# ilirlikalla/Smith-Waterman-FPGA-module

Hardware: AMD Instinct MI355X
Metric: GCUPS (higher is better)
Workload: dtype f16

## Files before the change

smith-waterman-fpga-module_amd/csrc/swbank_bank.h:

```cpp
#ifndef SWBANK_BANK_H
#define SWBANK_BANK_H

#include <dlfcn.h>
#include <hip/hip_runtime.h>
#include <rccl/rccl.h>

#include <algorithm>
#include <cmath>
#include <cstdarg>
#include <cstdio>
#include <cstdlib>
#include <cstring>
#include <atomic>
#include <condition_variable>
#include <functional>
#include <memory>
#include <mutex>
#include <numeric>
#include <thread>
#include <chrono>
#include <vector>
#if defined(__SSE2__)
#include <emmintrin.h>
#endif
#if defined(__x86_64__)
#include <immintrin.h>
#endif

#include "swbank.h"
#include "swbank_align.h"
#include "swbank_internal.h"
#include "swbank_pack.h"

extern "C" int swk_has_variant(int R, int RB, int col0, int prof, int gotoh, int f16);
extern "C" hipError_t swk_launch_wave(int K, int col0, int prof, int gotoh, int f16,
                                      const void* edge_in, void* edge_out, uint32_t ecols,
                                      int accum, const uint8_t* res,
                                      const uint64_t* offs, const uint32_t* lens, size_t n,
                                      const uint32_t* qtab, uint32_t nv, uint32_t S, uint32_t O,
                                      uint32_t E, uint32_t PS, uint32_t pad, int32_t* scores,
                                      int packed, const uint32_t* fb_qtab, uint32_t fb_nv,
                                      uint32_t fb_PS, int32_t fb_thresh,
                                      const SwkWaveSplit* split, uint32_t ulen,
                                      uint32_t ustride, int half, hipStream_t st);
extern "C" hipError_t swk_launch_score(int R, int RB, int col0, int prof, int gotoh, int f16,
                                       const uint8_t* res, const uint64_t* offs,
                                       const uint32_t* lens, size_t n, const uint32_t* qtab,
                                       uint32_t nv, uint32_t S, uint32_t O, uint32_t E,
                                       uint32_t PS, uint32_t pad, int W, int32_t* scores,
                                       const void* edge_in, void* edge_out, uint32_t ecols,
                                       int accum, int packed, const uint32_t* idx,
                                       const uint32_t* nidx, uint32_t idx_base,
                                       const uint32_t* ident, int pair, uint32_t pS1,
                                       uint32_t pS2, uint32_t ulen, uint32_t ustride, uint32_t nq,
                                       uint32_t qwords, size_t sstride, hipStream_t st);
extern "C" unsigned swk_bal_slots(int W, uint32_t PS, int trim);
extern "C" unsigned swk_wave_half_grid(int gotoh, uint32_t prof_bytes, int W);
extern "C" hipError_t swk_bal_plan_uniform(void* plan, uint32_t ntiles, uint32_t K, uint32_t G,
                                           hipStream_t st);
extern "C" hipError_t swk_launch_pair_bal(const uint8_t* res, const uint64_t* offs,
                                          const uint32_t* lens, size_t n, const uint32_t* qtab,
                                          uint32_t nv, uint32_t S, uint32_t O, uint32_t E,
                                          uint32_t PS, uint32_t pad, int W, int32_t* scores,
                                          uint32_t pS1, uint32_t pS2, uint32_t ulen,
                                          uint32_t ustride, uint32_t* flag, uint32_t* state,
                                          uint32_t gen, unsigned grid, const uint32_t* idx,
                                          const uint32_t* nidx, const uint32_t* ident,
                                          const void* plan, uint32_t* fault, uint32_t poll_limit,
                                          uint32_t stall, int trim, uint32_t packed,
                                          const uint32_t* sidx, hipStream_t st);
extern "C" hipError_t swk_best_hit(const int32_t* scores, const uint64_t* ids, size_t n,
                                   unsigned long long* key, uint64_t* out, uint64_t* out_index,
                                   hipStream_t st);
extern "C" hipError_t swk_best_part(const int32_t* scores, size_t n, size_t base,
                                    unsigned long long* key, hipStream_t st);
extern "C" hipError_t swk_best_finalize(const unsigned long long* key, const uint64_t* ids,
                                        uint64_t* out, uint64_t* out_index, hipStream_t st);
extern "C" hipError_t swk_sort_lens(const uint32_t* lens, size_t n, uint32_t max_len,
                                    uint32_t* perm, uint32_t* perm_n, uint32_t* ident,
                                    uint32_t* scratch, hipStream_t st, void* plan = nullptr,
                                    unsigned G = 0);
extern "C" size_t swk_sort_scratch_bytes(void);
extern "C" hipError_t swk_flag_high(const int32_t* scores, size_t n, int32_t thresh,
                                    uint32_t* idx, uint32_t* count, hipStream_t st);
extern "C" size_t swk_i32_waves(size_t n, uint32_t scols, size_t budget_bytes);
extern "C" hipError_t swk_launch_i32(int gotoh, const uint8_t* res, const uint64_t* offs,
                                     const uint32_t* lens, size_t n, int packed,
                                     const uint32_t* idx, const uint32_t* nidx, uint32_t idx_base,
                                     const void* prof, uint32_t nstrips, uint32_t qlen,
                                     uint32_t pad, uint32_t O, uint32_t E, int32_t* scores,
                                     void* scratch, uint32_t scols, size_t waves, hipStream_t st);

extern "C" size_t swk_top_state_words(void);
extern "C" hipError_t swk_top_hits(const int32_t* scores, const uint64_t* ids, size_t n, size_t nq,
                                   size_t k, int32_t min_score, unsigned long long* state,
                                   unsigned long long* keys, uint64_t* hits, int32_t* hit_scores,
                                   uint64_t* hit_ids, uint32_t* counts, hipStream_t st);

inline int env_int(const char* name, int dflt) {
  const char* v = std::getenv(name);
  return (v && *v) ? std::atoi(v) : dflt;
}

struct PhaseTrace {
  const char* path = std::getenv("SWBANK_TRACE_FILE");
  std::chrono::steady_clock::time_point t0 = std::chrono::steady_clock::now();
  std::vector<std::pair<const char*, double>> marks;
  std::mutex mu;
  void mark(const char* what) { mark_at(what, std::chrono::steady_clock::now()); }
  void mark_at(const char* what, std::chrono::steady_clock::time_point t) {
    if (!path) return;
    std::lock_guard<std::mutex> g(mu);
    marks.push_back({what, std::chrono::duration<double, std::micro>(t - t0).count()});
  }
  ~PhaseTrace() {
    if (!path || marks.empty()) return;
    if (FILE* f = std::fopen(path, "a")) {
      for (auto& m : marks) std::fprintf(f, "%s %.1f\n", m.first, m.second);
      std::fprintf(f, "--\n");
      std::fclose(f);
    }
  }
};
inline thread_local PhaseTrace* g_trace = nullptr;
inline void trace_mark(const char* what) {
  if (g_trace) g_trace->mark(what);
}

inline bool poison_buffers() {
  const char* v = std::getenv("SWBANK_POISON");
  return v && v[0] == '1';
}

template <typename T>
struct DevBuf {
  T* p = nullptr;
  size_t cap = 0;
  hipError_t reserve(size_t n) {
    if (n <= cap) return hipSuccess;
    if (p) (void)hipFree(p);
    p = nullptr;
    cap = 0;
    size_t want = std::max<size_t>(n, 64);
    hipError_t e = hipMalloc(reinterpret_cast<void**>(&p), want * sizeof(T));
    if (e == hipSuccess) cap = want;
    if (e == hipSuccess && poison_buffers()) {
      e = hipMemset(p, 0x3C, want * sizeof(T));
      if (e == hipSuccess) e = hipStreamSynchronize(nullptr);
    }
    return e;
  }
  void release() {
    if (p) (void)hipFree(p);
    p = nullptr;
    cap = 0;
  }
};

struct UcBuf {
  uint8_t* p = nullptr;
  size_t cap = 0;
  hipError_t reserve(size_t n) {
    if (n <= cap) return hipSuccess;
    if (p) (void)hipFree(p);
    p = nullptr;
    cap = 0;
    hipError_t e = hipExtMallocWithFlags(reinterpret_cast<void**>(&p), n, hipDeviceMallocUncached);
    if (e == hipSuccess) cap = n;
    return e;
  }
  void release() {
    if (p) (void)hipFree(p);
    p = nullptr;
    cap = 0;
  }
};

struct PinBuf {
  unsigned flags = hipHostMallocDefault;
  uint8_t* p = nullptr;
  size_t cap = 0;
  hipError_t reserve(size_t n) {
    if (n <= cap) return hipSuccess;
    if (p) (void)hipHostFree(p);
    p = nullptr;
    cap = 0;
    const size_t want = std::max<size_t>(n, 4096);
    hipError_t e = hipHostMalloc(reinterpret_cast<void**>(&p), want, flags);
    if (e == hipSuccess) cap = want;
    return e;
  }
  void release() {
    if (p) (void)hipHostFree(p);
    p = nullptr;
    cap = 0;
  }
};


class HostPool {
 public:
  explicit HostPool(unsigned n) : n_(std::max(1u, n)) {
    for (unsigned i = 1; i < n_; ++i) th_.emplace_back([this, i] { loop(i); });
  }
  ~HostPool() {
    {
      std::lock_guard<std::mutex> g(m_);
      stop_.store(true);
      gen_.fetch_add(1);
    }
    cv_.notify_all();
    for (auto& t : th_) t.join();
  }
  unsigned size() const { return n_; }
  void run(const std::function<void(unsigned)>& f) {
    if (n_ == 1) {
      f(0);
      return;
    }
    job_ = &f;
    pending_.store(n_ - 1, std::memory_order_relaxed);
    {
      std::lock_guard<std::mutex> g(m_);
      gen_.fetch_add(1, std::memory_order_release);
    }
    cv_.notify_all();
    f(0);
    for (unsigned it = 1; pending_.load(std::memory_order_acquire) != 0; ++it) relax(it);
    job_ = nullptr;
  }

 private:
  static void relax(unsigned) {
#if defined(__SSE2__)
    _mm_pause();
#endif
  }
  void loop(unsigned i) {
    uint64_t seen = 0;
    for (;;) {
      const auto t0 = std::chrono::steady_clock::now();
      for (unsigned it = 1; gen_.load(std::memory_order_acquire) == seen; ++it) {
        relax(it);
        if ((it & 255) == 0 &&
            std::chrono::steady_clock::now() - t0 > std::chrono::microseconds(200)) {
          std::unique_lock<std::mutex> l(m_);
          cv_.wait(l, [&] { return gen_.load() != seen; });
        }
      }
      seen = gen_.load(std::memory_order_acquire);
      if (stop_.load()) return;
      (*job_)(i);
      pending_.fetch_sub(1, std::memory_order_acq_rel);
    }
  }
  unsigned n_;
  std::vector<std::thread> th_;
  std::mutex m_;
  std::condition_variable cv_;
  const std::function<void(unsigned)>* job_ = nullptr;
  std::atomic<unsigned> pending_{0};
  std::atomic<uint64_t> gen_{0};
  std::atomic<bool> stop_{false};
};

class Launcher {
 public:
  explicit Launcher(int device) : th_([this, device] { loop(device); }) {}
  ~Launcher() {
    {
      std::lock_guard<std::mutex> g(m_);
      stop_ = true;
    }
    cv_.notify_one();
    th_.join();
  }
  void post(std::function<sw_status()> f) {
    {
      std::lock_guard<std::mutex> g(m_);
      q_.push_back(std::move(f));
      ++posted_;
    }
    cv_.notify_one();
  }
  sw_status wait(size_t k) {
    while (done_.load(std::memory_order_acquire) < k) {
#if defined(__SSE2__)
      _mm_pause();
#endif
    }
    return st_.load(std::memory_order_acquire);
  }
  sw_status wait_all() { return wait(posted_); }
  void reset() {
    wait_all();
    posted_ = 0;
    done_.store(0);
    st_.store(SW_OK);
  }

 private:
  void loop(int device) {
    (void)hipSetDevice(device);
    for (;;) {
      std::function<sw_status()> f;
      {
        std::unique_lock<std::mutex> l(m_);
        cv_.wait(l, [&] { return stop_ || !q_.empty(); });
        if (q_.empty()) return;
        f = std::move(q_.front());
        q_.erase(q_.begin());
      }
      if (st_.load(std::memory_order_relaxed) == SW_OK) {
        const sw_status s = f();
        if (s != SW_OK) st_.store(s, std::memory_order_release);
      }
      done_.fetch_add(1, std::memory_order_acq_rel);
    }
  }
  std::mutex m_;
  std::condition_variable cv_;
  std::vector<std::function<sw_status()>> q_;
  bool stop_ = false;
  size_t posted_ = 0;
  std::atomic<size_t> done_{0};
  std::atomic<sw_status> st_{SW_OK};
  std::thread th_;
};

struct sw_bank {
  sw_config cfg{};
  int device = 0;
  int cus = 0;
  hipStream_t stream = nullptr;
  char err[512] = {0};

  bool have_pen = false;
  int alpha = SW_DNA_ALPHA;
  std::vector<int8_t> matrix;
  int32_t gap_open = 0, gap_extend = 0;

  bool have_query = false;
  uint64_t qid = 0;
  std::vector<uint8_t> query;
  std::vector<std::vector<uint8_t>> qset;
  bool mq_ready = false;
  DevBuf<uint32_t> mqtab, mqtab16;
  size_t mq_words = 0;
  DevBuf<uint32_t> mqpair;
  size_t mq_pair_words = 0;
  int mq_pair_segs = 0, mq_pair_rows = 0;
  uint32_t mq_pS1 = 0, mq_pS2 = 0;

  bool dirty = true;
  int R = 32, RB = 4, W = 1, col0 = 0, prof = 0;
  uint32_t S = 0, O = 0, E = 0, nv = 0, PS = 0, pad = 4;
  int32_t smax = 0;
  DevBuf<uint32_t> qtab;
  bool f16 = false;
  uint32_t nv16 = 0, PS16 = 0;
  int32_t f16_neg = 0;
  DevBuf<uint32_t> qtab16;
  DevBuf<uint32_t> qpair;
  uint32_t pair_bytes = 0, pS1 = 0, pS2 = 0;
  DevBuf<uint32_t> fb_idx, fb_cnt;
  bool i32_ready = false;
  uint32_t i32_strips = 0;
  DevBuf<uint2> i32prof, i32scr;
  DevBuf<unsigned long long> best_key;
  bool al_ready = false;
  DevBuf<uint8_t> al_tab, al_res;
  DevBuf<uint2> al_scr;
  DevBuf<uint32_t> al_dirs, al_lens, al_cig, al_list;
  DevBuf<uint64_t> al_offs;
  DevBuf<sw_alignment> al_out;
  DevBuf<SwkAlignPlan> al_plan;
  DevBuf<unsigned long long> top_state, top_keys;
  DevBuf<int32_t> top_scores, top_hsc;
  DevBuf<uint64_t> top_hits;
  DevBuf<uint32_t> top_cnt;
  hipEvent_t ev_top = nullptr;
  struct Seg { int W; size_t off, off16; };
  std::vector<Seg> segs;
  DevBuf<uint2> edge[2];
  int wK = 0;
  int wsegs = 1;
  size_t wseg_words = 0, wseg_words16 = 0;
  uint32_t wPS = 0;
  DevBuf<uint32_t> wtab;
  DevBuf<uint32_t> wtab16;
  uint32_t wPS16 = 0;
  int sK[3] = {0, 0, 0};
  size_t sseg_words[3] = {0, 0, 0}, sseg_words16[3] = {0, 0, 0};
  uint32_t sPS[3] = {0, 0, 0}, sPS16[3] = {0, 0, 0};
  DevBuf<uint32_t> stab[3], stab16[3];
  DevBuf<uint2> sring;
  DevBuf<uint32_t> tprog;

  static constexpr int NSLOT = 3, NDSLOT = 6;
  hipStream_t copy_stream = nullptr;
  hipEvent_t h2d_done[NSLOT] = {}, kern_done[NDSLOT] = {};
  PinBuf hslot[NSLOT], hscores;
  std::vector<std::vector<uint32_t>> mlist;
  std::vector<std::vector<uint8_t>> mstage;
  std::vector<std::vector<uint32_t>> mbad;
  std::vector<hipEvent_t> out_ev;
  hipStream_t out_stream = nullptr;
  hipStream_t stream2 = nullptr;
  hipEvent_t ev_s2 = nullptr;
  double host_pack_ms = 0;
  int feed_dslots = NSLOT;
  DevBuf<uint8_t> dslot[NDSLOT];
  DevBuf<uint32_t> sortscr[NDSLOT];
  DevBuf<uint8_t> sbuf;
  UcBuf sflag;
  DevBuf<SwkStreamChunk> sdrec;
  DevBuf<uint32_t> sctr;
  hipStream_t kstream = nullptr;
  PinBuf srec, shflag{hipHostMallocCoherent};
  PinBuf shscores{hipHostMallocCoherent};
  std::vector<hipEvent_t> sev;
  std::unique_ptr<HostPool> pool;
  std::unique_ptr<Launcher> launcher;

  DevBuf<uint8_t> res;
  DevBuf<uint64_t> offs;
  DevBuf<uint32_t> lens;
  DevBuf<int32_t> scores;
  DevBuf<uint8_t> gres;
  DevBuf<uint64_t> goffs;
  DevBuf<uint32_t> glens;

  char last_kernel[160] = {0};

  int best_kind = 0;
  uint64_t best_id = 0, best_index = 0;
  int32_t best_score = 0;
  DevBuf<uint64_t> best_dev;
  hipEvent_t best_ev = nullptr;

  std::vector<sw_bank*> kids;
  std::unique_ptr<HostPool> dpool;
  std::vector<void*> comms;
  bool rccl_gather = false;
  unsigned pool_threads = 0;
  DevBuf<int32_t> grecv;
  PinBuf hrecv;
  DevBuf<uint32_t> bal_state, bal_flag;
  DevBuf<uint32_t> wbal_state, wbal_flag;
  uint32_t wbal_gen = 0;
  DevBuf<uint32_t> bal_plan;
  size_t bal_key[3] = {0, 0, 0};
  uint32_t bal_gen = 0;
  bool peer_ready = false;
  hipEvent_t ev_join = nullptr;
  std::vector<hipEvent_t> deal_ev;
  bool best_root = false;
  DevBuf<uint32_t> dperm, dsort;
  bool is_multi() const { return !kids.empty(); }
  bool gotoh() const { return cfg.gap_model == SW_GAP_GOTOH; }

  hipEvent_t ev_ready = nullptr, ev_used = nullptr;
  PinBuf stage;

  sw_counters ctr{};

  PinBuf faultw{hipHostMallocCoherent};
  bool host_call = false;
  bool no_handoff = false;

  bool timing = false;
  struct Ev { hipEvent_t a, b, c; };
  std::vector<Ev> events;
};

struct DevGuard {
  int prev = -1;
  DevGuard() {
    if (hipGetDevice(&prev) != hipSuccess) prev = -1;
  }
  explicit DevGuard(const sw_bank* b) : DevGuard() {
    if (b && b->device >= 0) (void)hipSetDevice(b->device);
  }
  ~DevGuard() {
    if (prev >= 0) (void)hipSetDevice(prev);
  }
  DevGuard(const DevGuard&) = delete;
  DevGuard& operator=(const DevGuard&) = delete;
};

inline uint16_t f16_score_bits(int v) {
  return __builtin_bit_cast(uint16_t, (_Float16)((float)v * (1.0f / 2048.0f)));
}


sw_status fail(sw_bank* b, sw_status st, const char* fmt, ...);

#define HIPOK(bank, expr)                                                                 \
  do {                                                                                    \
    hipError_t e_ = (expr);                                                               \
    if (e_ != hipSuccess)                                                                 \
      return fail((bank), SW_ERR_HIP, "%s: %s (%s:%d)", #expr, hipGetErrorString(e_),    \
                  __FILE__, __LINE__);                                                    \
  } while (0)

struct Timed {
  sw_bank* b;
  hipStream_t st;
  sw_bank::Ev ev{};
  sw_status begin() {
    if (!b->timing) return SW_OK;
    HIPOK(b, hipEventCreate(&ev.a));
    HIPOK(b, hipEventCreate(&ev.c));
    HIPOK(b, hipEventRecord(ev.a, st));
    ev.b = ev.a;
    return SW_OK;
  }
  sw_status end() {
    if (!b->timing) return SW_OK;
    HIPOK(b, hipEventRecord(ev.c, st));
    b->events.push_back(ev);
    return SW_OK;
  }
  void drop() {
    if (!b->timing) return;
    if (ev.a) (void)hipEventDestroy(ev.a);
    if (ev.c) (void)hipEventDestroy(ev.c);
    ev = {};
  }
};

struct Rccl {
  bool ok = false;
  char err[160] = {0};
  decltype(&ncclCommInitAll) commInitAll = nullptr;
  decltype(&ncclCommDestroy) commDestroy = nullptr;
  decltype(&ncclGather) gather = nullptr;
  decltype(&ncclGetErrorString) errorString = nullptr;
  decltype(&ncclCommAbort) commAbort = nullptr;
  decltype(&ncclCommGetAsyncError) asyncError = nullptr;
  decltype(&ncclGroupStart) groupStart = nullptr;
  decltype(&ncclGroupEnd) groupEnd = nullptr;
};
const Rccl& rccl();

template <class F>
sw_status each_kid(sw_bank* b, F&& f) {
  for (sw_bank* k : b->kids) {
    const sw_status st = f(k);
    if (st != SW_OK) return fail(b, st, "device %d: %s", k->device, k->err);
  }
  return SW_OK;
}

unsigned host_threads();

template <class F>
void parallel_for(HostPool& pool, size_t n, F&& f) {
  const unsigned T = pool.size();
  if (T <= 1 || n < 2048) {
    f((size_t)0, n);
    return;
  }
  const size_t step = (n + T - 1) / T;
  pool.run([&](unsigned p) {
    const size_t lo = std::min(n, p * step), hi = std::min(n, lo + step);
    if (lo < hi) f(lo, hi);
  });
}

inline size_t align16(size_t x) { return (x + 15) & ~(size_t)15; }
inline uint32_t record_len(const uint8_t* rec) {
  uint16_t l;
  std::memcpy(&l, rec + 4, 2);
  return l;
}

void copy_kernel_name(sw_bank* b, const char* gather);
uint32_t* fault_word(sw_bank* b);
sw_status take_fault(sw_bank* b, int which);
sw_status prepare(sw_bank* b);
sw_status prepare_multi(sw_bank* b);
sw_status prepare_i32(sw_bank* b);
void u16_gotoh_rows(const sw_bank* b, bool f16, int& R, int& W);
bool wave_preferred(const sw_bank* b, size_t n, uint32_t max_len, bool use_f16);
sw_status launch(sw_bank* b, const uint8_t* d_res, const uint64_t* d_offs,
                 const uint32_t* d_lens, size_t n, uint32_t max_len, int32_t* d_scores,
                 hipStream_t st, uint32_t packed = SWK_PACK_BYTES,
                 const uint32_t* perm = nullptr, const uint32_t* perm_n = nullptr,
                 bool dsort = false, bool wait_prev = true, uint32_t* sort_out = nullptr,
                 uint32_t* sort_scr = nullptr, uint32_t ulen = 0, uint32_t ustride = 0,
                 uint32_t min_len = 0);
bool chunk_perm(HostPool& pool, const uint32_t* len, size_t n, uint32_t* perm);
bool scratch_free(const sw_bank* b, uint32_t max_len);
struct MixedOrder {
  std::vector<uint32_t> pos;
  uint32_t hi = 0, shift = 0, nbin = 0;
};
bool mixed_pack(sw_bank* b, const uint8_t* residues, size_t nres, const uint64_t* offsets,
                const uint32_t* lens, size_t c0, size_t cnt, size_t step,
                const std::vector<uint64_t>& rbase, const std::vector<uint64_t>& rspan,
                const std::vector<size_t>& psz, const std::vector<size_t>& part4, uint32_t* so32,
                uint32_t* sl32, uint8_t* mcodes, uint32_t* order, MixedOrder* mo, size_t& end);
sw_status batch_feed(sw_bank* b, const uint8_t* residues, size_t nres, const uint64_t* offsets,
                     const uint32_t* lens, size_t n, int32_t* out);
sw_status records_feed(sw_bank* b, const uint8_t* recs, size_t n, int32_t* out);
sw_status stream_feed(sw_bank* b, const uint8_t* residues, size_t nres, const uint64_t* offsets,
                      size_t n, uint32_t L, int32_t* out, bool& used,
                      const uint8_t* recs = nullptr, const uint32_t* rlens = nullptr);
sw_status multi_batch(sw_bank* b, const uint8_t* residues, size_t nres, const uint64_t* offsets,
                      const uint32_t* lens, size_t n, int32_t* scores_out);
sw_status multi_records(sw_bank* b, const uint8_t* recs, size_t n, int32_t* scores_out);
sw_status multi_device(sw_bank* b, const uint8_t* d_res, const uint64_t* d_offs,
                       const uint32_t* d_lens, const uint64_t* d_ids, size_t n, uint32_t min_len,
                       uint32_t max_len, int32_t* d_scores, hipStream_t hs, bool records);
sw_status multi_resident(sw_bank* b, const sw_device_batch* per, int32_t* d_gathered,
                         hipStream_t hs);
sw_status launch_set(sw_bank* b, const uint8_t* d_res, const uint64_t* d_offs,
                     const uint32_t* d_lens, size_t n, uint32_t min_len, uint32_t max_len,
                     int32_t* d_scores, hipStream_t st, size_t sstride);
sw_status track_best_device(sw_bank* b, const int32_t* d_scores, const uint64_t* d_ids, size_t n,
                            hipStream_t st);

#endif
```

smith-waterman-fpga-module_amd/csrc/swbank_bank.hip:

```cpp
#include "swbank_bank.h"

sw_status fail(sw_bank* b, sw_status st, const char* fmt, ...) {
  if (b) {
    va_list ap;
    va_start(ap, fmt);
    vsnprintf(b->err, sizeof(b->err), fmt, ap);
    va_end(ap);
  }
  return st;
}

extern "C" int32_t sw_device_count(void) {
  int n = 0;
  if (hipGetDeviceCount(&n) != hipSuccess) return 0;
  return n;
}

static sw_status check_device(int dev) {
  int ndev = 0;
  if (hipGetDeviceCount(&ndev) != hipSuccess || ndev <= 0) return SW_ERR_NO_DEVICE;
  if (dev < 0 || dev >= ndev) return SW_ERR_NO_DEVICE;
  hipDeviceProp_t prop;
  if (hipGetDeviceProperties(&prop, dev) != hipSuccess) return SW_ERR_NO_DEVICE;
  if (std::strncmp(prop.gcnArchName, "gfx950", 6) != 0) return SW_ERR_NO_DEVICE;
  return SW_OK;
}


extern "C" sw_status sw_bank_create(sw_bank** out, const sw_config* cfg_in) {
  DevGuard dev_guard;
  if (!out) return SW_ERR_ARG;
  *out = nullptr;
  sw_config cfg;
  if (cfg_in)
    cfg = *cfg_in;
  else
    sw_config_default(&cfg);
  if (cfg.alphabet != SW_ALPHABET_DNA && cfg.alphabet != SW_ALPHABET_PROTEIN) return SW_ERR_ARG;
  if (cfg.gap_model != SW_GAP_MERGED && cfg.gap_model != SW_GAP_GOTOH) return SW_ERR_ARG;
  if (cfg.max_query_len > SWB_MAX_QUERY) return SW_ERR_UNSUPPORTED;
  if (cfg.n_devices < 0 || cfg.n_devices > SW_MAX_DEVICES) return SW_ERR_ARG;

  if (cfg.n_devices >= 1) {
    for (int d = 0; d < cfg.n_devices; ++d) {
      const sw_status st = check_device(cfg.devices[d]);
      if (st != SW_OK) return st;
    }
    sw_bank* b = new (std::nothrow) sw_bank();
    if (!b) return SW_ERR_NOMEM;
    b->cfg = cfg;
    b->device = cfg.devices[0];
    b->alpha = cfg.alphabet == SW_ALPHABET_DNA ? SW_DNA_ALPHA : SW_PROTEIN_ALPHA;
    for (int d = 0; d < cfg.n_devices; ++d) {
      sw_config kc = cfg;
      kc.n_devices = 0;
      kc.device = cfg.devices[d];
      sw_bank* k = nullptr;
      const sw_status st = sw_bank_create(&k, &kc);
      if (st != SW_OK) {
        sw_bank_destroy(b);
        return st;
      }
      k->pool_threads = std::max(2u, host_threads() / (unsigned)cfg.n_devices);
      b->kids.push_back(k);
    }
    b->dpool.reset(new (std::nothrow) HostPool((unsigned)cfg.n_devices));
    b->pool.reset(new (std::nothrow) HostPool(host_threads()));
    if (!b->dpool || !b->pool) {
      sw_bank_destroy(b);
      return SW_ERR_NOMEM;
    }
    const char* gm = std::getenv("SWBANK_GATHER");
    const bool force_copy = gm && std::strcmp(gm, "copy") == 0;
    const bool force_rccl = gm && std::strcmp(gm, "rccl") == 0;
    bool distinct = true;
    for (int i = 0; i < cfg.n_devices; ++i)
      for (int j = 0; j < i; ++j) distinct = distinct && cfg.devices[i] != cfg.devices[j];
    if (!force_copy && (distinct || force_rccl)) {
      const Rccl& r = rccl();
      ncclResult_t nr = ncclSuccess;
      if (r.ok) {
        std::vector<ncclComm_t> comms((size_t)cfg.n_devices);
        nr = r.commInitAll(comms.data(), cfg.n_devices, cfg.devices);
        if (nr == ncclSuccess) b->comms.assign(comms.begin(), comms.end());
      }
      b->rccl_gather = !b->comms.empty();
      if (b->comms.empty() && force_rccl) {
        sw_bank_destroy(b);
        return SW_ERR_UNSUPPORTED;
      }
      if (b->comms.empty())
        snprintf(b->err, sizeof(b->err), "RCCL unavailable (%s), gathering with device copies",
                 r.ok ? r.errorString(nr) : r.err);
    }
    (void)hipSetDevice(b->device);
    *out = b;
    return SW_OK;
  }

  int dev = cfg.device;
  if (dev < 0 && hipGetDevice(&dev) != hipSuccess) return SW_ERR_NO_DEVICE;
  const sw_status dst = check_device(dev);
  if (dst != SW_OK) return dst;

  sw_bank* b = new (std::nothrow) sw_bank();
  if (!b) return SW_ERR_NOMEM;
  b->cfg = cfg;
  b->device = dev;
  if (hipSetDevice(dev) != hipSuccess ||
      hipStreamCreateWithFlags(&b->stream, hipStreamNonBlocking) != hipSuccess ||
      hipStreamCreateWithFlags(&b->copy_stream, hipStreamNonBlocking) != hipSuccess ||
      hipStreamCreateWithFlags(&b->out_stream, hipStreamNonBlocking) != hipSuccess ||
      hipStreamCreateWithFlags(&b->stream2, hipStreamNonBlocking) != hipSuccess) {
    for (hipStream_t* x : {&b->stream, &b->copy_stream, &b->out_stream, &b->stream2})
      if (*x) (void)hipStreamDestroy(*x);
    delete b;
    return SW_ERR_HIP;
  }
  b->alpha = cfg.alphabet == SW_ALPHABET_DNA ? SW_DNA_ALPHA : SW_PROTEIN_ALPHA;
  if (hipDeviceGetAttribute(&b->cus, hipDeviceAttributeMultiprocessorCount, dev) != hipSuccess)
    b->cus = 0;
  if (cfg.alphabet == SW_ALPHABET_PROTEIN) {
    int8_t m[SW_PROTEIN_ALPHA * SW_PROTEIN_ALPHA];
    sw_fill_matrix(SW_ALPHABET_PROTEIN, 0, 0, m);
    b->matrix.assign(m, m + sizeof(m));
    b->gap_open = -11;
    b->gap_extend = -1;
    b->have_pen = true;
  }
  *out = b;
  return SW_OK;
}

extern "C" void sw_bank_destroy(sw_bank* b) {
  DevGuard dev_guard(b);
  if (!b) return;
  if (b->is_multi() || !b->comms.empty()) {
    const Rccl& r = rccl();
    for (void* c : b->comms) (void)r.commDestroy(static_cast<ncclComm_t>(c));
    (void)hipSetDevice(b->device);
    if (b->ev_used) (void)hipEventSynchronize(b->ev_used);
    if (b->ev_join) (void)hipEventDestroy(b->ev_join);
    if (b->ev_used) (void)hipEventDestroy(b->ev_used);
    for (sw_bank* k : b->kids) sw_bank_destroy(k);
    b->dpool.reset();
    b->pool.reset();
    (void)hipSetDevice(b->device);
    b->grecv.release();
    b->hrecv.release();
    b->res.release();
    b->offs.release();
    b->lens.release();
    b->dperm.release();
    b->dsort.release();
    delete b;
    return;
  }
  (void)hipSetDevice(b->device);
  if (b->stream) (void)hipStreamSynchronize(b->stream);
  if (b->ev_top) (void)hipEventSynchronize(b->ev_top);
  uint64_t nl;
  double pm, sm;
  (void)sw_bank_timing(b, &nl, &pm, &sm);
  b->faultw.release();
  b->qtab.release();
  b->qtab16.release();
  b->mqtab.release();
  b->mqtab16.release();
  b->mqpair.release();
  b->qpair.release();
  b->stage.release();
  if (b->ev_ready) (void)hipEventDestroy(b->ev_ready);
  if (b->ev_used) (void)hipEventDestroy(b->ev_used);
  if (b->best_ev) (void)hipEventDestroy(b->best_ev);
  if (b->ev_top) (void)hipEventDestroy(b->ev_top);
  if (b->ev_join) (void)hipEventDestroy(b->ev_join);
  for (hipEvent_t e : b->deal_ev) (void)hipEventDestroy(e);
  b->fb_idx.release();
  b->fb_cnt.release();
  b->best_key.release();
  b->best_dev.release();
  b->i32prof.release();
  b->i32scr.release();
  b->al_tab.release();
  b->al_res.release();
  b->al_scr.release();
  b->al_dirs.release();
  b->al_lens.release();
  b->al_cig.release();
  b->al_list.release();
  b->al_offs.release();
  b->al_out.release();
  b->al_plan.release();
  b->top_state.release();
  b->top_keys.release();
  b->top_scores.release();
  b->top_hsc.release();
  b->top_hits.release();
  b->top_cnt.release();
  b->dperm.release();
  b->dsort.release();
  b->bal_state.release();
  b->bal_flag.release();
  b->wbal_state.release();
  b->wbal_flag.release();
  b->bal_plan.release();
  b->wtab.release();
  b->wtab16.release();
  b->tprog.release();
  for (int i = 0; i < 3; ++i) {
    b->stab[i].release();
    b->stab16[i].release();
  }
  b->sring.release();
  b->edge[0].release();
  b->edge[1].release();
  if (b->copy_stream) (void)hipStreamSynchronize(b->copy_stream);
  if (b->out_stream) (void)hipStreamSynchronize(b->out_stream);
  if (b->stream2) (void)hipStreamSynchronize(b->stream2);
  for (hipEvent_t e : b->out_ev) (void)hipEventDestroy(e);
  for (int i = 0; i < sw_bank::NSLOT; ++i) b->hslot[i].release();
  for (int i = 0; i < sw_bank::NDSLOT; ++i) {
    b->dslot[i].release();
    b->sortscr[i].release();
  }
  b->sbuf.release();
  b->sflag.release();
  b->sdrec.release();
  b->sctr.release();
  b->srec.release();
  b->shflag.release();
  b->shscores.release();
  for (hipEvent_t e : b->sev) (void)hipEventDestroy(e);
  for (int i = 0; i < sw_bank::NSLOT; ++i)
    if (b->h2d_done[i]) (void)hipEventDestroy(b->h2d_done[i]);
  for (int i = 0; i < sw_bank::NDSLOT; ++i)
    if (b->kern_done[i]) (void)hipEventDestroy(b->kern_done[i]);
  b->hscores.release();
  b->launcher.reset();
  b->pool.reset();
  if (b->copy_stream) (void)hipStreamDestroy(b->copy_stream);
  if (b->out_stream) (void)hipStreamDestroy(b->out_stream);
  if (b->stream2) (void)hipStreamDestroy(b->stream2);
  if (b->kstream) (void)hipStreamDestroy(b->kstream);
  if (b->ev_s2) (void)hipEventDestroy(b->ev_s2);
  b->res.release();
  b->offs.release();
  b->lens.release();
  b->scores.release();
  b->gres.release();
  b->goffs.release();
  b->glens.release();
  if (b->stream) (void)hipStreamDestroy(b->stream);
  delete b;
}

extern "C" int32_t sw_bank_devices(const sw_bank* b, int32_t* devices, int32_t cap) {
  if (!b) return 0;
  const int32_t n = b->is_multi() ? (int32_t)b->kids.size() : 1;
  for (int32_t i = 0; devices && i < std::min(n, cap); ++i)
    devices[i] = b->is_multi() ? b->kids[(size_t)i]->device : b->device;
  return n;
}

extern "C" const char* sw_last_error(const sw_bank* b) { return b ? b->err : "null bank"; }

extern "C" const char* sw_last_kernel(const sw_bank* b) { return b ? b->last_kernel : ""; }

uint32_t* fault_word(sw_bank* b) {
  if (!b->faultw.p) {
    if (b->faultw.reserve(64) != hipSuccess) return nullptr;
    std::memset(b->faultw.p, 0, b->faultw.cap);
  }
  return reinterpret_cast<uint32_t*>(b->faultw.p);
}

sw_status take_fault(sw_bank* b, int which) {
  if (b->is_multi()) {
    sw_status st = SW_OK;
    for (sw_bank* k : b->kids) {
      const sw_status ks = take_fault(k, which);
      if (ks != SW_OK && st == SW_OK) st = fail(b, ks, "device %d: %s", k->device, k->err);
    }
    return st;
  }
  if (!b->faultw.p) return SW_OK;
  volatile uint32_t* w = reinterpret_cast<volatile uint32_t*>(b->faultw.p) + which * SWK_FAULT_WORDS;
  uint32_t f = 0;
  for (int i = 0; i < SWK_FAULT_WORDS; ++i) {
    f |= w[i];
    w[i] = 0;
  }
  if (f == 0) return SW_OK;
  if (f & SWK_FAULT_BAL) ++b->ctr.balanced_timeouts;
  if (f & SWK_FAULT_TAIL) ++b->ctr.tail_timeouts;
  if (f & SWK_FAULT_WBAL) ++b->ctr.wave_balanced_timeouts;
  char kinds[96] = "";
  const char* names[3] = {"balanced ranges", "protein tail", "wave balanced ranges"};
  for (int i = 0; i < 3; ++i)
    if (f & (1u << i)) {
      if (kinds[0]) strncat(kinds, ", ", sizeof(kinds) - strlen(kinds) - 1);
      strncat(kinds, names[i], sizeof(kinds) - strlen(kinds) - 1);
    }
  return fail(b, SW_ERR_TIMEOUT,
              "a cross-workgroup hand-off wait ran out (%s) in a %s call: its scores are invalid",
              kinds, which ? "host-buffer" : "device");
}

extern "C" sw_status sw_bank_sync(sw_bank* b) {
  DevGuard dev_guard(b);
  if (!b) return SW_ERR_ARG;
  if (b->is_multi()) {
    for (sw_bank* k : b->kids) {
      const sw_status st = sw_bank_sync(k);
      if (st != SW_OK) {
        (void)take_fault(b, 0);
        return fail(b, st, "device %d: %s", k->device, k->err);
      }
    }
    if (b->ev_used) {
      int cur = -1;
      HIPOK(b, hipGetDevice(&cur));
      hipError_t e = hipSetDevice(b->device);
      if (e == hipSuccess) e = hipEventSynchronize(b->ev_used);
      (void)hipSetDevice(cur);
      HIPOK(b, e);
    }
    return SW_OK;
  }
  int cur = -1;
  HIPOK(b, hipGetDevice(&cur));
  hipError_t e = hipSetDevice(b->device);
  if (e == hipSuccess && b->ev_used) e = hipEventSynchronize(b->ev_used);
  if (e == hipSuccess && b->ev_top) e = hipEventSynchronize(b->ev_top);
  if (e == hipSuccess) e = hipStreamSynchronize(b->stream);
  (void)hipSetDevice(cur);
  HIPOK(b, e);
  return take_fault(b, 0);
}

static void sum_counters(sw_counters& c, const sw_bank* b) {
  c.stream_calls += b->ctr.stream_calls;
  c.stream_reruns += b->ctr.stream_reruns;
  c.stream_declined += b->ctr.stream_declined;
  c.chunked_calls += b->ctr.chunked_calls;
  c.device_sorts += b->ctr.device_sorts;
  c.gather_timeouts += b->ctr.gather_timeouts;
  c.mixed_chunks += b->ctr.mixed_chunks;
  c.mixed_runs += b->ctr.mixed_runs;
  c.balanced_calls += b->ctr.balanced_calls;
  c.balanced_timeouts += b->ctr.balanced_timeouts;
  c.tail_timeouts += b->ctr.tail_timeouts;
  c.handoff_reruns += b->ctr.handoff_reruns;
  c.wave_balanced_timeouts += b->ctr.wave_balanced_timeouts;
  c.h2d_bytes += __atomic_load_n(&b->ctr.h2d_bytes, __ATOMIC_RELAXED);
}

extern "C" sw_status sw_bank_counters_ex(const sw_bank* b, sw_counters* out, size_t out_size) {
  if (!b || !out) return SW_ERR_ARG;
  if (out_size != 64 && out_size != 80 && out_size != 96 && out_size != sizeof(sw_counters))
    return SW_ERR_ARG;
  sw_counters c{};
  sum_counters(c, b);
  for (const sw_bank* k : b->kids) sum_counters(c, k);
  std::memcpy(out, &c, out_size);
  return SW_OK;
}

extern "C" sw_status sw_bank_counters(const sw_bank* b, sw_counters* out) {
  return sw_bank_counters_ex(b, out, 64);
}

void copy_kernel_name(sw_bank* b, const char* gather) {
  snprintf(b->last_kernel, sizeof(b->last_kernel), "multi[%zu] gather=%s: %s", b->kids.size(),
           gather, b->kids[0]->last_kernel);
}

static sw_status set_matrix_impl(sw_bank* b, const int8_t* m, int alpha, int32_t go,
                                 int32_t ge) {
  if (go > 0 || ge > 0 || go < -32767 || ge < -32767)
    return fail(b, SW_ERR_ARG, "gap penalties must be <= 0 (got open %d, extend %d)", go, ge);
  b->matrix.assign(m, m + (size_t)alpha * alpha);
  b->alpha = alpha;
  b->gap_open = go;
  b->gap_extend = ge;
  b->have_pen = true;
  b->dirty = true;
  return SW_OK;
}


extern "C" sw_status sw_set_penalties(sw_bank* b, int32_t match, int32_t mismatch,
                                      int32_t gap_open, int32_t gap_extend) {
  DevGuard dev_guard(b);
  if (!b) return SW_ERR_ARG;
  if (b->is_multi())
    return each_kid(b, [&](sw_bank* k) {
      return sw_set_penalties(k, match, mismatch, gap_open, gap_extend);
    });
  if (b->cfg.alphabet != SW_ALPHABET_DNA)
    return fail(b, SW_ERR_ARG, "sw_set_penalties needs a DNA bank; use sw_set_matrix");
  int8_t m[SW_DNA_ALPHA * SW_DNA_ALPHA];
  if (sw_fill_matrix(SW_ALPHABET_DNA, match, mismatch, m) != SW_OK)
    return fail(b, SW_ERR_ARG, "match/mismatch outside int8 (%d, %d)", match, mismatch);
  return set_matrix_impl(b, m, SW_DNA_ALPHA, gap_open, gap_extend);
}

extern "C" sw_status sw_set_matrix(sw_bank* b, const int8_t* m, int32_t alpha, int32_t gap_open,
                                   int32_t gap_extend) {
  DevGuard dev_guard(b);
  if (!b || !m) return SW_ERR_ARG;
  if (b->is_multi())
    return each_kid(b, [&](sw_bank* k) { return sw_set_matrix(k, m, alpha, gap_open, gap_extend); });
  const int want = b->cfg.alphabet == SW_ALPHABET_DNA ? SW_DNA_ALPHA : SW_PROTEIN_ALPHA;
  if (alpha != want) return fail(b, SW_ERR_ARG, "matrix alphabet %d, bank expects %d", alpha, want);
  return set_matrix_impl(b, m, alpha, gap_open, gap_extend);
}

extern "C" sw_status sw_load_query(sw_bank* b, uint64_t id, const uint8_t* codes, uint32_t len) {
  DevGuard dev_guard(b);
  if (!b || (!codes && len)) return SW_ERR_ARG;
  if (b->is_multi()) {
    const sw_status st = each_kid(b, [&](sw_bank* k) { return sw_load_query(k, id, codes, len); });
    b->qset.clear();
    b->have_query = st == SW_OK;
    return st;
  }
  const uint32_t cap = b->cfg.max_query_len ? b->cfg.max_query_len : SWB_MAX_QUERY;
  if (len > cap)
    return fail(b, SW_ERR_UNSUPPORTED, "query length %u exceeds the bank maximum %u", len, cap);
  for (uint32_t i = 0; i < len; ++i)
    if (codes[i] >= (uint32_t)b->alpha)
      return fail(b, SW_ERR_ARG, "query code %u at %u outside alphabet %d", codes[i], i, b->alpha);
  b->query.assign(codes, codes + len);
  b->qid = id;
  b->qset.clear();
  b->have_query = true;
  b->dirty = true;
  return SW_OK;
}

extern "C" sw_status sw_load_queries(sw_bank* b, size_t nq, const uint64_t* ids,
                                     const uint8_t* codes, const uint64_t* offsets,
                                     const uint32_t* lens) {
  DevGuard dev_guard(b);
  if (!b || nq == 0 || !offsets || !lens) return SW_ERR_ARG;
  if (b->is_multi()) {
    const sw_status st = each_kid(
        b, [&](sw_bank* k) { return sw_load_queries(k, nq, ids, codes, offsets, lens); });
    b->qset = b->kids[0]->qset;
    b->have_query = st == SW_OK;
    return st;
  }
  if (nq > 65536) return fail(b, SW_ERR_UNSUPPORTED, "more than 65536 queries in one set");
  if (nq == 1) return sw_load_query(b, ids ? ids[0] : 0, codes + offsets[0], lens[0]);
  const uint32_t cap = b->cfg.max_query_len ? b->cfg.max_query_len : SWB_MAX_QUERY;
  size_t longest = 0;
  for (size_t i = 0; i < nq; ++i) {
    if (lens[i] > cap)
      return fail(b, SW_ERR_UNSUPPORTED, "query %zu length %u exceeds the bank maximum %u", i,
                  lens[i], cap);
    if (lens[i] && !codes) return fail(b, SW_ERR_ARG, "null query codes");
    for (uint32_t j = 0; j < lens[i]; ++j)
      if (codes[offsets[i] + j] >= (uint32_t)b->alpha)
        return fail(b, SW_ERR_ARG, "query %zu code %u at %u outside alphabet %d", i,
                    codes[offsets[i] + j], j, b->alpha);
    if (lens[i] > lens[longest]) longest = i;
  }
  b->qset.assign(nq, {});
  for (size_t i = 0; i < nq; ++i)
    b->qset[i].assign(codes + offsets[i], codes + offsets[i] + lens[i]);
  b->query = b->qset[longest];
  b->qid = ids ? ids[longest] : 0;
  b->have_query = true;
  b->dirty = true;
  b->mq_ready = false;
  return SW_OK;
}

extern "C" size_t sw_query_count(const sw_bank* b) {
  return !b || !b->have_query ? 0 : b->qset.size() > 1 ? b->qset.size() : 1;
}

static void pair_strides(uint32_t NR, uint32_t& pS1, uint32_t& pS2) {
  const uint32_t B = 4 * NR;
  pS2 = (B + 15) / 16 * 16;
  while ((pS2 / 16) % 16 != 1) pS2 += 16;
  pS1 = (4 * pS2 + B + 15) / 16 * 16;
  while ((pS1 / 16) % 16 != 4) pS1 += 16;
}

static std::vector<uint32_t> pair_table(const uint8_t* q, int qlen, int r0, uint32_t NR,
                                        const int8_t* m, int A, uint32_t pS1, uint32_t pS2) {
  const uint32_t bytes = 16 + 4 * pS1 + 4 * pS2 + 4 * NR;
  std::vector<uint32_t> t(bytes / 4, 0xBC00BC00u);
  auto word = [&](int r, int x, int y) -> uint32_t {
    if (r0 + r >= qlen) return 0xBC00BC00u;
    const int c = q[r0 + r];
    return (uint32_t)f16_score_bits(m[c * A + x]) | (uint32_t)f16_score_bits(m[c * A + y]) << 16;
  };
  for (int x = 0; x < A; ++x)
    for (int y = 0; y < A; ++y) {
      const uint32_t base = (16 + x * pS1 + y * pS2) / 4;
      for (uint32_t k = 0; k + 1 < NR; ++k) t[base + k] = word((int)k + 1, x, y);
    }
  for (int x = 0; x < A; ++x)
    for (int y = 0; y < A; ++y) t[(16 + x * pS1 + y * pS2) / 4 - 1] = word(0, x, y);
  return t;
}

sw_status prepare(sw_bank* b) {
  if (!b->have_pen || !b->have_query)
    return fail(b, SW_ERR_STATE, "load penalties (ld_penalties) and a query (ld_sequence) first");
  if (!b->dirty) return SW_OK;
  const int A = b->alpha;
  const int8_t* m = b->matrix.data();
  int smax = -128, smin = 127;
  for (int i = 0; i < A * A; ++i) {
    smax = std::max<int>(smax, m[i]);
    smin = std::min<int>(smin, m[i]);
  }
  const int S = std::max(0, smax);
  if (S - smin > 254)
    return fail(b, SW_ERR_RANGE, "substitution range [%d, %d] exceeds 254", smin, smax);
  const int o = -b->gap_open, e = -b->gap_extend;
  const bool gotoh = b->cfg.gap_model == SW_GAP_GOTOH;
  if (gotoh && o + e + S > 65535) return fail(b, SW_ERR_RANGE, "gap penalties too large");

  bool lut = A == SW_DNA_ALPHA;
  const int sN = m[4];
  for (int i = 0; lut && i < A; ++i) lut = m[i * A + 4] == sN;
  lut = lut && sN <= 0;
  bool lut_f16 = true;
  for (int i = 0; i < A * A; ++i) {
    const uint16_t bits = f16_score_bits(m[i]);
    lut_f16 = lut_f16 && (bits & 0xFFu) == 0;
  }
  const bool f16_range = -(o + 2 * e + (std::max(0, smax) - smin)) >= -2048;
  const int prof =
      (env_int("SWBANK_PROFILE", 0) || !lut || (!lut_f16 && f16_range)) ? 1 : 0;

  const int qlen = (int)b->query.size();
  const int col0 = (!gotoh && smax > o + e) ? 1 : 0;
  const bool u16_only = gotoh && (!f16_range || env_int("SWBANK_F16", 1) == 0);
  int R = (qlen <= 16 || prof || col0 || u16_only) ? 16 : 32, RB = 4;
  R = env_int("SWBANK_R", R);
  RB = env_int("SWBANK_RB", RB);
  const int max_rows = (R >= 64 ? 8 : 16) * R;
  int seg_rows = qlen > max_rows ? env_int("SWBANK_SEG", max_rows)
                                 : std::max(qlen, 1);
  if (seg_rows % R != 0 && seg_rows < qlen)
    return fail(b, SW_ERR_ARG, "segment rows %d not a multiple of R=%d", seg_rows, R);
  if (!swk_has_variant(R, RB, col0, prof, gotoh ? 1 : 0, 0))
    return fail(b, SW_ERR_UNSUPPORTED, "no kernel variant R=%d RB=%d col0=%d prof=%d gotoh=%d", R,
                RB, col0, prof, (int)gotoh);
  const int Wseg = std::max(1, (seg_rows + R - 1) / R);
  if (Wseg * 64 > (R >= 64 ? 512 : 1024))
    return fail(b, SW_ERR_UNSUPPORTED, "segment of %d rows too tall for one workgroup", seg_rows);

  std::vector<uint32_t> tab;
  std::vector<sw_bank::Seg> segs;
  uint32_t PS = prof ? (uint32_t)((Wseg * R + 15) / 16 * 16) : 0;
  if (prof) PS += (16u + 256u - PS % 256u) % 256u;
  const uint32_t pad = prof ? (uint32_t)A : 4u;
  const uint32_t nv = prof ? 0u : (uint32_t)(uint8_t)(S - sN) * 0x01010101u;
  for (int r0 = 0; r0 < std::max(qlen, 1); r0 += seg_rows) {
    const int rows = std::min(seg_rows, std::max(qlen, 1) - r0);
    const int W = std::max(1, (rows + R - 1) / R);
    segs.push_back({W, tab.size(), 0});
    if (!prof) {
      const size_t base = tab.size();
      tab.resize(base + (size_t)W * R, 0xFFFFFFFFu);
      for (int i = 0; i < rows && r0 + i < qlen; ++i) {
        uint32_t w = 0;
        for (int c = 0; c < 4; ++c)
          w |= (uint32_t)(uint8_t)(S - m[b->query[r0 + i] * A + c]) << (8 * c);
        tab[base + i] = w;
      }
    } else {
      std::vector<uint8_t> qp((size_t)(A + 1) * PS, 0xFF);
      for (int c = 0; c < A; ++c)
        for (int i = 0; i < rows && r0 + i < qlen; ++i)
          qp[(size_t)c * PS + i] = (uint8_t)(S - m[b->query[r0 + i] * A + c]);
      const size_t base = tab.size();
      tab.resize(base + qp.size() / 4);
      std::memcpy(tab.data() + base, qp.data(), qp.size());
    }
  }
  auto f16_hi = [](int v, uint8_t* out) {
    const uint16_t bits = f16_score_bits(v);
    *out = (uint8_t)(bits >> 8);
    return (bits & 0xFFu) == 0 &&
           (int)((float)__builtin_bit_cast(_Float16, bits) * 2048.0f) == v;
  };
  bool f16 = swk_has_variant(R, RB, col0, prof, gotoh ? 1 : 0, 1) != 0;
  std::vector<uint32_t> tab16;
  uint8_t hN = 0;
  uint32_t PS16 = 0;
  if (!prof) {
    f16 = f16 && f16_hi(sN, &hN);
    for (int i = 0; f16 && i < A * A; ++i) {
      uint8_t h;
      f16 = f16_hi(m[i], &h);
    }
  }
  if (f16 && !prof) {
    tab16.assign(tab.size(), 0xBCBCBCBCu);
    for (sw_bank::Seg& sg : segs) {
      const int r0 = (int)(&sg - segs.data()) * seg_rows;
      sg.off16 = sg.off;
      for (int i = 0; i < sg.W * R && r0 + i < qlen && i < seg_rows; ++i) {
        uint32_t w = 0;
        for (int c = 0; c < 4; ++c) {
          uint8_t h;
          f16_hi(m[b->query[r0 + i] * A + c], &h);
          w |= (uint32_t)h << (8 * c);
        }
        tab16[sg.off + i] = w;
      }
    }
  } else if (f16) {
    PS16 = (uint32_t)((2 * Wseg * R + 15) / 16 * 16);
    PS16 += (16u + 256u - PS16 % 256u) % 256u;
    const uint16_t padv = 0xBC00u;
    for (sw_bank::Seg& sg : segs) {
      const int r0 = (int)(&sg - segs.data()) * seg_rows;
      std::vector<uint16_t> qp((size_t)(A + 1) * PS16 / 2, padv);
      for (int c = 0; c < A; ++c)
        for (int i = 0; i < sg.W * R && r0 + i < qlen && i < seg_rows; ++i)
          qp[(size_t)c * PS16 / 2 + i] =
              f16_score_bits(m[b->query[r0 + i] * A + c]);
      sg.off16 = tab16.size();
      tab16.resize(sg.off16 + qp.size() / 2);
      std::memcpy(tab16.data() + sg.off16, qp.data(), qp.size() * 2);
    }
  }
  std::vector<uint32_t> tpair;
  uint32_t pS1 = 0, pS2 = 0, pair_words = 0;
  if (f16 && !prof && !col0 && A == SW_DNA_ALPHA &&
      (gotoh ? R == 16 || R == 32 : R == 32 && segs.size() == 1 && segs[0].W <= 4)) {
    const uint32_t NR = (uint32_t)segs[0].W * R;
    pair_strides(NR, pS1, pS2);
    for (size_t sg = 0; sg < segs.size(); ++sg) {
      const std::vector<uint32_t> t =
          pair_table(b->query.data(), qlen, (int)sg * seg_rows, NR, m, A, pS1, pS2);
      pair_words = (uint32_t)t.size();
      tpair.insert(tpair.end(), t.begin(), t.end());
    }
  }
  const auto wave_tables = [&](int wrows, int nsegs, std::vector<uint32_t>& wt,
                               std::vector<uint32_t>& wt16) {
    for (int sg = 0; sg < nsegs; ++sg) {
      const int r0 = sg * wrows, nr = std::min(wrows, std::max(0, qlen - r0));
      if (!prof) {
        const size_t base = wt.size();
        wt.resize(base + wrows, 0xFFFFFFFFu);
        for (int i = 0; i < nr; ++i) {
          uint32_t w = 0;
          for (int c = 0; c < 4; ++c)
            w |= (uint32_t)(uint8_t)(S - m[b->query[r0 + i] * A + c]) << (8 * c);
          wt[base + i] = w;
        }
        if (f16) {
          const size_t b16 = wt16.size();
          wt16.resize(b16 + wrows, 0xBCBCBCBCu);
          for (int i = 0; i < nr; ++i) {
            uint32_t w = 0;
            for (int c = 0; c < 4; ++c) {
              uint8_t h;
              f16_hi(m[b->query[r0 + i] * A + c], &h);
              w |= (uint32_t)h << (8 * c);
            }
            wt16[b16 + i] = w;
          }
        }
      } else {
        std::vector<uint8_t> qp((size_t)(A + 1) * wrows, 0xFF);
        for (int c = 0; c < A; ++c)
          for (int i = 0; i < nr; ++i)
            qp[(size_t)c * wrows + i] = (uint8_t)(S - m[b->query[r0 + i] * A + c]);
        const size_t base = wt.size();
        wt.resize(base + qp.size() / 4);
        std::memcpy(wt.data() + base, qp.data(), qp.size());
        if (f16) {
          std::vector<uint16_t> q16((size_t)(A + 1) * wrows, 0xBC00u);
          for (int c = 0; c < A; ++c)
            for (int i = 0; i < nr; ++i)
              q16[(size_t)c * wrows + i] = f16_score_bits(m[b->query[r0 + i] * A + c]);
          const size_t b16 = wt16.size();
          wt16.resize(b16 + q16.size() / 2);
          std::memcpy(wt16.data() + b16, q16.data(), q16.size() * 2);
        }
      }
    }
  };
  std::vector<uint32_t> wt, wt16;
  const int wK = qlen <= 256 ? 4 : qlen <= 512 ? 8 : 16;
  const int wrows = 64 * wK;
  const int wsegs = std::max(1, (qlen + wrows - 1) / wrows);
  const uint32_t wPS = prof ? (uint32_t)wrows : 0, wPS16 = prof ? (uint32_t)wrows * 2 : 0;
  wave_tables(wrows, wsegs, wt, wt16);
  std::vector<uint32_t> st[3], st16[3];
  int sK[3] = {0, 0, 0};
  for (int i = 0; i < 3; ++i) {
    sK[i] = (wsegs == 1 && wK >= 8) ? wK / (2 << i) : 0;
    if (sK[i]) wave_tables(64 * sK[i], 2 << i, st[i], st16[i]);
  }
  HIPOK(b, hipSetDevice(b->device));
  if (!b->ev_ready) {
    HIPOK(b, hipEventCreateWithFlags(&b->ev_ready, hipEventDisableTiming));
    HIPOK(b, hipEventCreateWithFlags(&b->ev_used, hipEventDisableTiming));
    HIPOK(b, hipEventRecord(b->ev_ready, b->stream));
    HIPOK(b, hipEventRecord(b->ev_used, b->stream));
  }
  HIPOK(b, hipEventSynchronize(b->ev_ready));
  const size_t nbytes =
      (wt16.size() + wt.size() + st16[0].size() + st[0].size() + st16[1].size() +
       st[1].size() + st16[2].size() + st[2].size() + tab.size() + tab16.size() + tpair.size()) *
      4;
  HIPOK(b, b->stage.reserve(nbytes));
  HIPOK(b, hipStreamWaitEvent(b->stream, b->ev_used, 0));
  size_t at = 0;
  auto upload = [&](DevBuf<uint32_t>& dst, const std::vector<uint32_t>& src) -> hipError_t {
    hipError_t e = dst.reserve(src.size());
    if (e != hipSuccess || src.empty()) return e;
    std::memcpy(b->stage.p + at, src.data(), src.size() * 4);
    e = hipMemcpyAsync(dst.p, b->stage.p + at, src.size() * 4, hipMemcpyHostToDevice, b->stream);
    at += src.size() * 4;
    return e;
  };
  if (!wt16.empty()) HIPOK(b, upload(b->wtab16, wt16));
  HIPOK(b, upload(b->wtab, wt));
  b->wPS16 = wPS16;
  b->wK = wK;
  b->wPS = wPS;
  b->wsegs = wsegs;
  b->wseg_words = wt.size() / wsegs;
  b->wseg_words16 = wt16.empty() ? 0 : wt16.size() / wsegs;
  for (int i = 0; i < 3; ++i) {
    if (!st16[i].empty()) HIPOK(b, upload(b->stab16[i], st16[i]));
    HIPOK(b, upload(b->stab[i], st[i]));
    b->sK[i] = sK[i];
    b->sseg_words[i] = st[i].size() / (2 << i);
    b->sseg_words16[i] = st16[i].size() / (2 << i);
    b->sPS[i] = prof ? (uint32_t)(64 * sK[i]) : 0;
    b->sPS16[i] = prof ? (uint32_t)(128 * sK[i]) : 0;
  }
  HIPOK(b, upload(b->qtab, tab));
  if (f16) HIPOK(b, upload(b->qtab16, tab16));
  if (!tpair.empty()) HIPOK(b, upload(b->qpair, tpair));
  b->pair_bytes = pair_words * 4;
  b->pS1 = pS1;
  b->pS2 = pS2;
  HIPOK(b, hipEventRecord(b->ev_ready, b->stream));
  b->f16 = f16;
  b->nv16 = (uint32_t)hN * 0x01010101u;
  b->PS16 = PS16;
  b->f16_neg = -(o + 2 * e + (S - smin));
  b->R = R;
  b->RB = RB;
  b->W = segs[0].W;
  b->segs = segs;
  b->S = (uint32_t)S;
  b->O = (uint32_t)o;
  b->E = (uint32_t)e;
  b->nv = nv;
  b->PS = PS;
  b->pad = pad;
  b->prof = prof;
  b->smax = smax;
  b->col0 = col0;
  b->i32_ready = false;
  b->al_ready = false;
  b->mq_ready = false;
  b->dirty = false;
  return SW_OK;
}

sw_status prepare_multi(sw_bank* b) {
  if (b->mq_ready) return SW_OK;
  const int A = b->alpha;
  const int8_t* m = b->matrix.data();
  const int R = b->R, S = (int)b->S;
  const size_t words = b->segs.back().off + (size_t)b->segs.back().W * R;
  const int seg_rows = b->segs[0].W * R;
  const size_t nq = b->qset.size();
  std::vector<uint32_t> t16, t8(nq * words, 0xFFFFFFFFu);
  if (b->f16) t16.assign(nq * words, 0xBCBCBCBCu);
  for (size_t i = 0; i < nq; ++i) {
    const std::vector<uint8_t>& qi = b->qset[i];
    for (size_t sg = 0; sg < b->segs.size(); ++sg) {
      const size_t base = i * words + b->segs[sg].off;
      const int r0 = (int)sg * seg_rows;
      for (int j = 0; j < b->segs[sg].W * R && r0 + j < (int)qi.size(); ++j) {
        uint32_t w = 0, h = 0;
        for (int c = 0; c < 4; ++c) {
          const int v = m[qi[r0 + j] * A + c];
          w |= (uint32_t)(uint8_t)(S - v) << (8 * c);
          h |= (uint32_t)(f16_score_bits(v) >> 8) << (8 * c);
        }
        t8[base + j] = w;
        if (b->f16) t16[base + j] = h;
      }
    }
  }
  std::vector<uint32_t> tp;
  b->mq_pair_segs = 0;
  if (b->f16 && !b->prof && !b->gotoh() && !b->col0 && A == SW_DNA_ALPHA &&
      env_int("SWBANK_MQ_PAIR", 1) != 0) {
    const int want = env_int("SWBANK_MQ_PAIR_ROWS", 128);
    const uint32_t NR = want == 128 ? 128 : want == 256 ? 256 : 512;
    b->mq_pair_rows = (int)NR;
    pair_strides(NR, b->mq_pS1, b->mq_pS2);
    const int qmax = (int)b->query.size();
    b->mq_pair_segs = std::max(1, (qmax + (int)NR - 1) / (int)NR);
    for (int sg = 0; sg < b->mq_pair_segs; ++sg)
      for (size_t i = 0; i < nq; ++i) {
        const std::vector<uint32_t> t = pair_table(b->qset[i].data(), (int)b->qset[i].size(),
                                                   sg * (int)NR, NR, m, A, b->mq_pS1, b->mq_pS2);
        b->mq_pair_words = t.size();
        tp.insert(tp.end(), t.begin(), t.end());
      }
  }
  HIPOK(b, hipSetDevice(b->device));
  HIPOK(b, hipEventSynchronize(b->ev_ready));
  HIPOK(b, b->stage.reserve((t8.size() + t16.size() + tp.size()) * 4));
  HIPOK(b, b->mqtab.reserve(t8.size()));
  if (!t16.empty()) HIPOK(b, b->mqtab16.reserve(t16.size()));
  HIPOK(b, hipStreamWaitEvent(b->stream, b->ev_used, 0));
  std::memcpy(b->stage.p, t8.data(), t8.size() * 4);
  HIPOK(b, hipMemcpyAsync(b->mqtab.p, b->stage.p, t8.size() * 4, hipMemcpyHostToDevice,
                          b->stream));
  if (!t16.empty()) {
    std::memcpy(b->stage.p + t8.size() * 4, t16.data(), t16.size() * 4);
    HIPOK(b, hipMemcpyAsync(b->mqtab16.p, b->stage.p + t8.size() * 4, t16.size() * 4,
                            hipMemcpyHostToDevice, b->stream));
  }
  if (!tp.empty()) {
    const size_t at = (t8.size() + t16.size()) * 4;
    HIPOK(b, b->mqpair.reserve(tp.size()));
    std::memcpy(b->stage.p + at, tp.data(), tp.size() * 4);
    HIPOK(b, hipMemcpyAsync(b->mqpair.p, b->stage.p + at, tp.size() * 4, hipMemcpyHostToDevice,
                            b->stream));
  }
  HIPOK(b, hipEventRecord(b->ev_ready, b->stream));
  b->mq_words = words;
  b->mq_ready = true;
  return SW_OK;
}

sw_status prepare_i32(sw_bank* b) {
  if (b->i32_ready) return SW_OK;
  const int A = b->alpha;
  const int8_t* m = b->matrix.data();
  const uint32_t qlen = (uint32_t)b->query.size();
  const uint32_t strips = std::max(1u, (qlen + 255) / 256), pad = b->pad;
  if (pad + 1 > 25) return fail(b, SW_ERR_UNSUPPORTED, "int32 kernel: alphabet %d too large", A);
  std::vector<int16_t> h((size_t)strips * (pad + 1) * 64 * 4, 0);
  for (uint32_t s = 0; s < strips; ++s)
    for (uint32_t c = 0; c <= pad; ++c)
      for (uint32_t l = 0; l < 64; ++l)
        for (uint32_t k = 0; k < 4; ++k) {
          const uint32_t r = s * 256 + 4 * l + k;
          int v = 0;
          if (r < qlen) v = c < (uint32_t)A ? m[b->query[r] * A + c] : (int)b->S - 255;
          h[(((size_t)s * (pad + 1) + c) * 64 + l) * 4 + k] = (int16_t)v;
        }
  HIPOK(b, hipSetDevice(b->device));
  HIPOK(b, hipEventSynchronize(b->ev_ready));
  HIPOK(b, b->stage.reserve(h.size() * 2));
  HIPOK(b, b->i32prof.reserve(h.size() / 4));
  HIPOK(b, hipStreamWaitEvent(b->stream, b->ev_used, 0));
  std::memcpy(b->stage.p, h.data(), h.size() * 2);
  HIPOK(b, hipMemcpyAsync(b->i32prof.p, b->stage.p, h.size() * 2, hipMemcpyHostToDevice,
                          b->stream));
  HIPOK(b, hipEventRecord(b->ev_ready, b->stream));
  b->i32_strips = strips;
  b->i32_ready = true;
  return SW_OK;
}

extern "C" sw_status sw_bank_set_timing(sw_bank* b, int32_t enable) {
  DevGuard dev_guard(b);
  if (!b) return SW_ERR_ARG;
  if (b->is_multi()) return each_kid(b, [&](sw_bank* k) { return sw_bank_set_timing(k, enable); });
  b->timing = enable != 0;
  return SW_OK;
}

extern "C" sw_status sw_bank_timing(sw_bank* b, uint64_t* launches, double* pack_ms,
                                    double* score_ms) {
  DevGuard dev_guard(b);
  if (!b) return SW_ERR_ARG;
  double p = 0, s = 0;
  uint64_t n = 0;
  sw_status st = SW_OK;
  if (b->is_multi()) {
    for (sw_bank* k : b->kids) {
      uint64_t kn = 0;
      double kp = 0, ks = 0;
      if ((st = sw_bank_timing(k, &kn, &kp, &ks)) != SW_OK)
        return fail(b, st, "device %d: %s", k->device, k->err);
      n += kn;
      p += kp;
      s += ks;
    }
    if (launches) *launches = n;
    if (pack_ms) *pack_ms = p;
    if (score_ms) *score_ms = s;
    return SW_OK;
  }
  for (auto& ev : b->events) {
    float t1 = 0, t2 = 0;
    if (st == SW_OK && hipEventSynchronize(ev.c) == hipSuccess &&
        (ev.b == ev.a || hipEventElapsedTime(&t1, ev.a, ev.b) == hipSuccess) &&
        hipEventElapsedTime(&t2, ev.b, ev.c) == hipSuccess) {
      p += t1;
      s += t2;
      ++n;
    } else {
      st = fail(b, SW_ERR_HIP, "event timing failed");
    }
    (void)hipEventDestroy(ev.a);
    if (ev.b != ev.a) (void)hipEventDestroy(ev.b);
    (void)hipEventDestroy(ev.c);
  }
  b->events.clear();
  p += b->host_pack_ms;
  b->host_pack_ms = 0;
  if (launches) *launches = n;
  if (pack_ms) *pack_ms = p;
  if (score_ms) *score_ms = s;
  if (st == SW_OK && n > 0) st = take_fault(b, 0);
  return st;
}

extern "C" sw_status sw_best_hit_device(sw_bank* b, const int32_t* d_scores, const uint64_t* d_ids,
                                        size_t n, uint64_t* d_out, void* stream) {
  DevGuard dev_guard(b);
  if (!b) return SW_ERR_ARG;
  if (b->is_multi())
    return sw_best_hit_device(b->kids[0], d_scores, d_ids, n, d_out,
                              stream ? stream : b->kids[0]->stream);
  if (!d_scores || !d_out || n == 0 || n > 0xFFFFFFFFull)
    return fail(b, SW_ERR_ARG, "sw_best_hit_device: empty, null or > 2^32 scores");
  HIPOK(b, hipSetDevice(b->device));
  HIPOK(b, b->best_key.reserve(1));
  HIPOK(b, swk_best_hit(d_scores, d_ids, n, b->best_key.p, d_out, nullptr,
                        stream ? reinterpret_cast<hipStream_t>(stream) : b->stream));
  return SW_OK;
}

extern "C" sw_status sw_best_hit(sw_bank* b, const int32_t* scores, const uint64_t* ids, size_t n,
                                 uint64_t* best_id, int32_t* best_score) {
  DevGuard dev_guard(b);
  if (!scores || !best_id || !best_score || n == 0)
    return b ? fail(b, SW_ERR_ARG, "sw_best_hit: empty or null input") : SW_ERR_ARG;
  size_t bi = 0;
  for (size_t k = 1; k < n; ++k)
    if (scores[k] > scores[bi]) bi = k;
  *best_id = ids ? ids[bi] : (uint64_t)bi;
  *best_score = scores[bi];
  return SW_OK;
}
```

smith-waterman-fpga-module_amd/csrc/swbank_kcommon.h:

```cpp
#ifndef SWBANK_KCOMMON_H
#define SWBANK_KCOMMON_H
#include <hip/hip_runtime.h>
#include <stdint.h>

#include <algorithm>
#include <cstdlib>
#include <mutex>
#include <type_traits>
#include <vector>

#include "swbank_internal.h"

#ifndef SWK_TAIL_TOP
#define SWK_TAIL_TOP 1
#endif
#ifndef SWK_PRIO_ROT
#define SWK_PRIO_ROT 1
#endif
#ifndef SWK_PRIO_SHIFT
#define SWK_PRIO_SHIFT 18
#endif

#ifndef SWK_PRIO_END
#define SWK_PRIO_END 3
#endif
#ifndef SWK_PRIO_END_FRAC
#define SWK_PRIO_END_FRAC 4
#endif

#ifndef SWK_STAMPS
#define SWK_STAMPS 0
#endif

namespace swk {

#if SWK_PRIO_ROT
__device__ __forceinline__ void prio_rotate(uint32_t q, uint32_t& prio, uint32_t shift) {
  const uint32_t pr = ((uint32_t)(__builtin_amdgcn_s_memtime() >> shift) + q) & 3u;
  if (pr != prio) {
    prio = pr;
    if (pr == 0) __builtin_amdgcn_s_setprio(0);
    else if (pr == 1) __builtin_amdgcn_s_setprio(1);
    else if (pr == 2) __builtin_amdgcn_s_setprio(2);
    else __builtin_amdgcn_s_setprio(3);
  }
}
#endif

#if SWK_STAMPS
inline uint64_t* g_stamps_host = nullptr;
#endif
typedef unsigned short u16x2 __attribute__((ext_vector_type(2)));

__device__ __forceinline__ u16x2 as_u16x2(uint32_t x) { return __builtin_bit_cast(u16x2, x); }
__device__ __forceinline__ uint32_t as_u32(u16x2 x) { return __builtin_bit_cast(uint32_t, x); }
__device__ __forceinline__ u16x2 vmax(u16x2 a, u16x2 b) { return __builtin_elementwise_max(a, b); }
__device__ __forceinline__ u16x2 vsubs(u16x2 a, u16x2 b) {
  return __builtin_elementwise_sub_sat(a, b);
}



template <int R>
struct LutLookup {
  const uint32_t (&tab)[R];
  uint32_t nv, selw;
  __device__ __forceinline__ u16x2 operator()(int r) const {
    return as_u16x2(__builtin_amdgcn_perm(nv, tab[r], selw));
  }
};
template <int R>
struct ProfLookup {
  uint32_t lo[R / 4], hi[R / 4];
  __device__ __forceinline__ u16x2 operator()(int r) const {
    const uint32_t sel = (uint32_t)(r & 3) | ((uint32_t)(4 + (r & 3)) << 16) | 0x0C000C00u;
    return as_u16x2(__builtin_amdgcn_perm(hi[r >> 2], lo[r >> 2], sel));
  }
};

template <int R>
struct ProfLookup16 {
  uint32_t lo[R / 2], hi[R / 2];
  __device__ __forceinline__ u16x2 operator()(int r) const {
    const uint32_t k = (uint32_t)(r & 1) * 2;
    const uint32_t sel = k | ((k + 1) << 8) | ((k + 4) << 16) | ((k + 5) << 24);
    return as_u16x2(__builtin_amdgcn_perm(hi[r >> 1], lo[r >> 1], sel));
  }
};

template <int R, int RB, bool ZDOWN, class LK>
__device__ __forceinline__ void column_merged(const LK& lk, u16x2& diag, u16x2& upG,
                                              u16x2 (&Hl)[R], u16x2 (&Gl)[R], u16x2& best,
                                              u16x2 S2, u16x2 O2, u16x2 E2) {
#pragma unroll
  for (int r = 0; r < R; ++r) {
    const u16x2 p = lk(r);
    const u16x2 M = vsubs(diag, p);
    const u16x2 I = vsubs(vmax(upG, Gl[r]), E2);
    const u16x2 Hn = vmax(M, I) + S2;
    const u16x2 Gn = vmax(vsubs(M, O2), I);
    best = vmax(best, M);
    diag = Hl[r];
    Hl[r] = Hn;
    Gl[r] = Gn;
    upG = ZDOWN ? (u16x2){0, 0} : Gn;
    if ((r % RB) == RB - 1) __builtin_amdgcn_sched_barrier(0);
  }
}

typedef _Float16 f16x2 __attribute__((ext_vector_type(2)));
__device__ __forceinline__ f16x2 as_f16x2(u16x2 x) { return __builtin_bit_cast(f16x2, x); }
__device__ __forceinline__ u16x2 as_u16x2(f16x2 x) { return __builtin_bit_cast(u16x2, x); }
__device__ __forceinline__ f16x2 fmax2(f16x2 a, f16x2 b) {
  return __builtin_elementwise_maximum(a, b);
}
__host__ __device__ inline uint32_t f16_pair(int x) {
  const uint16_t h = __builtin_bit_cast(uint16_t, (_Float16)((float)x * (1.0f / 2048.0f)));
  return (uint32_t)h * 0x10001u;
}
__device__ __forceinline__ int32_t f16_unscore(uint32_t bits) {
  return (int32_t)((float)__builtin_bit_cast(_Float16, (unsigned short)bits) * 2048.0f);
}
template <int R, int RB, bool ZDOWN, class LK>
__device__ __forceinline__ void column_merged_f16(const LK& lk, u16x2& diag_, u16x2& upT_,
                                                  u16x2 (&Hl)[R], u16x2 (&Tl)[R], u16x2& best_,
                                                  f16x2 NOE2, f16x2 NE2) {
  f16x2 diag = as_f16x2(diag_), upT = as_f16x2(upT_), best = as_f16x2(best_);
  const f16x2 Z = {(_Float16)0, (_Float16)0};
#pragma unroll
  for (int r = 0; r < R; ++r) {
    const f16x2 sc = as_f16x2(lk(r));
    const f16x2 D = diag + sc;
    const f16x2 I = fmax2(upT, as_f16x2(Tl[r]));
    const f16x2 H = fmax2(fmax2(D, Z), I);
    const f16x2 T = fmax2(fmax2(D + NOE2, NOE2), I + NE2);
    best = fmax2(best, H);
    diag = as_f16x2(Hl[r]);
    Hl[r] = as_u16x2(H);
    Tl[r] = as_u16x2(T);
    upT = ZDOWN ? NOE2 : T;
    if ((r % RB) == RB - 1) __builtin_amdgcn_sched_barrier(0);
  }
  diag_ = as_u16x2(diag);
  upT_ = as_u16x2(upT);
  best_ = as_u16x2(best);
}

template <int R, int RB, class LK>
__device__ __forceinline__ void column_gotoh_f16(const LK& lk, u16x2& diag_, u16x2& upF_,
                                                 u16x2 (&Hl)[R], u16x2 (&El)[R], u16x2& best_,
                                                 f16x2 NOE2, f16x2 NE2) {
  f16x2 diag = as_f16x2(diag_), F = as_f16x2(upF_), best = as_f16x2(best_);
  const f16x2 Z = {(_Float16)0, (_Float16)0};
#pragma unroll
  for (int r = 0; r < R; ++r) {
    const f16x2 D = diag + as_f16x2(lk(r));
    const f16x2 E = as_f16x2(El[r]);
    const f16x2 H = fmax2(fmax2(D, E), F);
    const f16x2 HN = H + NOE2;
    best = fmax2(best, H);
    diag = as_f16x2(Hl[r]);
    Hl[r] = as_u16x2(H);
    El[r] = as_u16x2(fmax2(fmax2(HN, Z), E + NE2));
    F = fmax2(fmax2(HN, Z), F + NE2);
    if ((r % RB) == RB - 1) __builtin_amdgcn_sched_barrier(0);
  }
  upF_ = as_u16x2(F);
  best_ = as_u16x2(best);
}

#ifndef SWK_F16_ASM
#define SWK_F16_ASM 1
#endif
#ifndef SWK_F16_COLBLOCK
#define SWK_F16_COLBLOCK 1
#endif
#include "swbank_f16_rows.inc"
#define SWK_F16_HT(B)                                                                         \
  [h0] "+v"(Hl[B]), [h1] "+v"(Hl[B + 1]), [h2] "+v"(Hl[B + 2]), [h3] "+v"(Hl[B + 3]),          \
      [h4] "+v"(Hl[B + 4]), [h5] "+v"(Hl[B + 5]), [h6] "+v"(Hl[B + 6]), [h7] "+v"(Hl[B + 7]),  \
      [t0] "+v"(Xl[B]), [t1] "+v"(Xl[B + 1]), [t2] "+v"(Xl[B + 2]), [t3] "+v"(Xl[B + 3]),      \
      [t4] "+v"(Xl[B + 4]), [t5] "+v"(Xl[B + 5]), [t6] "+v"(Xl[B + 6]), [t7] "+v"(Xl[B + 7]),  \
      [Da] "+v"(Da), [Db] "=&v"(Db), [S1] "=&v"(S1), [best] "+v"(best)
#define SWK_F16_OUT_M(B) SWK_F16_HT(B), [X] "=&v"(X), [DN] "=&v"(DN), [IN] "=&v"(IN)
#define SWK_F16_OUT_G(B) SWK_F16_HT(B), [EN] "=&v"(X), [HN] "=&v"(DN), [FN] "=&v"(IN), [F] "+v"(up)
#define SWK_F16_IN_L(B)                                                                       \
  [nv] "v"(lk.nv), [sel] "v"(lk.selw), [noe] "s"(noe), [ne] "s"(ne), [no] "s"(no), [up] "v"(up),            \
      [tb0] "s"(lk.tab[B + 1]), [tb1] "s"(lk.tab[B + 2]), [tb2] "s"(lk.tab[B + 3]),           \
      [tb3] "s"(lk.tab[B + 4]), [tb4] "s"(lk.tab[B + 5]), [tb5] "s"(lk.tab[B + 6]),           \
      [tb6] "s"(lk.tab[B + 7]), [tb7] "s"(lk.tab[(B + 8) < R ? B + 8 : R - 1])
#define SWK_F16_IN_P(B)                                                                       \
  [noe] "s"(noe), [ne] "s"(ne), [no] "s"(no), [up] "v"(up), [selA] "s"(0x05040100u), [selB] "s"(0x07060302u), \
      [lo0] "v"(lk.lo[B / 2]), [lo1] "v"(lk.lo[B / 2 + 1]), [lo2] "v"(lk.lo[B / 2 + 2]),       \
      [lo3] "v"(lk.lo[B / 2 + 3]), [lo4] "v"(lk.lo[(B + 8) < R ? B / 2 + 4 : B / 2 + 3]),      \
      [hi0] "v"(lk.hi[B / 2]), [hi1] "v"(lk.hi[B / 2 + 1]), [hi2] "v"(lk.hi[B / 2 + 2]),       \
      [hi3] "v"(lk.hi[B / 2 + 3]), [hi4] "v"(lk.hi[(B + 8) < R ? B / 2 + 4 : B / 2 + 3])
#define SWK_F16_IN_LG(B)                                                                      \
  [nv] "v"(lk.nv), [sel] "v"(lk.selw), [noe] "s"(noe), [ne] "s"(ne),                          \
      [tb0] "s"(lk.tab[B + 1]), [tb1] "s"(lk.tab[B + 2]), [tb2] "s"(lk.tab[B + 3]),           \
      [tb3] "s"(lk.tab[B + 4]), [tb4] "s"(lk.tab[B + 5]), [tb5] "s"(lk.tab[B + 6]),           \
      [tb6] "s"(lk.tab[B + 7]), [tb7] "s"(lk.tab[(B + 8) < R ? B + 8 : R - 1])
#define SWK_F16_IN_PG(B)                                                                      \
  [noe] "s"(noe), [ne] "s"(ne), [selA] "s"(0x05040100u), [selB] "s"(0x07060302u),            \
      [lo0] "v"(lk.lo[B / 2]), [lo1] "v"(lk.lo[B / 2 + 1]), [lo2] "v"(lk.lo[B / 2 + 2]),       \
      [lo3] "v"(lk.lo[B / 2 + 3]), [lo4] "v"(lk.lo[(B + 8) < R ? B / 2 + 4 : B / 2 + 3]),      \
      [hi0] "v"(lk.hi[B / 2]), [hi1] "v"(lk.hi[B / 2 + 1]), [hi2] "v"(lk.hi[B / 2 + 2]),       \
      [hi3] "v"(lk.hi[B / 2 + 3]), [hi4] "v"(lk.hi[(B + 8) < R ? B / 2 + 4 : B / 2 + 3])

template <int R, bool GOTOH, bool ZDOWN, class LK>
__device__ __forceinline__ void column_f16_asm(const LK& lk, u16x2& diag_, u16x2& upX_,
                                               u16x2 (&Hl)[R], u16x2 (&Xl)[R], u16x2& best_,
                                               uint32_t noe, uint32_t ne, uint32_t no) {
  static_assert(R % 8 == 0, "rows come in blocks of 8");
  constexpr bool PROF = !std::is_same<LK, LutLookup<R>>::value;
  uint32_t Da, Db, S1, X, DN, IN;
  u16x2 best = best_, up = upX_;
#if SWK_F16_COLBLOCK
  if constexpr ((R == 32 || R == 16) && !GOTOH && !PROF && !ZDOWN) {
#define SWK_F16_COLASM(RR)                                                                    \
    asm volatile(                                                                             \
        "v_perm_b32 %[Da], %[nv], %[tz], %[sel]\n\t"                                          \
        "v_pk_add_f16 %[Da], %[dg], %[Da] clamp\n\t" SWK_F16M_L_Z0_COL##RR                          \
        : SWK_F16_COL##RR##_HT, [Da] "=&v"(Da), [Db] "=&v"(Db), [S1] "=&v"(S1), [X] "=&v"(X), \
          [DN] "=&v"(DN), [IN] "=&v"(IN), [best] "+v"(best)                                  \
        : [nv] "v"(lk.nv), [sel] "v"(lk.selw), [noe] "s"(noe), [ne] "s"(ne), [no] "s"(no), [up] "v"(up),     \
          [tz] "s"(lk.tab[0]), [dg] "v"(diag_), SWK_F16_COL##RR##_TB)
    if constexpr (R == 32) SWK_F16_COLASM(32);
    else SWK_F16_COLASM(16);
#undef SWK_F16_COLASM
    (void)Db; (void)S1; (void)X; (void)DN; (void)IN;
    upX_ = Xl[R - 1];
    best_ = best;
    return;
  }
#endif
  if constexpr (PROF)
    asm volatile(
        "v_perm_b32 %[Da], %[h0], %[l0], %[sA]\n\t"
        "v_pk_add_f16 %[Da], %[dg], %[Da] clamp"
        : [Da] "=&v"(Da)
        : [h0] "v"(lk.hi[0]), [l0] "v"(lk.lo[0]), [sA] "s"(0x05040100u), [dg] "v"(diag_));
  else
    asm volatile(
        "v_perm_b32 %[Da], %[nv], %[t0], %[sel]\n\t"
        "v_pk_add_f16 %[Da], %[dg], %[Da] clamp"
        : [Da] "=&v"(Da)
        : [nv] "v"(lk.nv), [t0] "s"(lk.tab[0]), [sel] "v"(lk.selw), [dg] "v"(diag_));
#pragma unroll
  for (int b = 0; b < R; b += 8) {
    const bool last = b + 8 >= R;
    if constexpr (GOTOH) {
      if constexpr (PROF) {
        if (last) asm volatile(SWK_F16G_P_L1 : SWK_F16_OUT_G(b) : SWK_F16_IN_PG(b));
        else      asm volatile(SWK_F16G_P_L0 : SWK_F16_OUT_G(b) : SWK_F16_IN_PG(b));
      } else {
        if (last) asm volatile(SWK_F16G_L_L1 : SWK_F16_OUT_G(b) : SWK_F16_IN_LG(b));
        else      asm volatile(SWK_F16G_L_L0 : SWK_F16_OUT_G(b) : SWK_F16_IN_LG(b));
      }
    } else {
      if constexpr (PROF) {
        if constexpr (ZDOWN) {
          if (last) asm volatile(SWK_F16M_P_Z1_L1 : SWK_F16_OUT_M(b) : SWK_F16_IN_P(b));
          else      asm volatile(SWK_F16M_P_Z1_L0 : SWK_F16_OUT_M(b) : SWK_F16_IN_P(b));
        } else {
          if (last) asm volatile(SWK_F16M_P_Z0_L1 : SWK_F16_OUT_M(b) : SWK_F16_IN_P(b));
          else      asm volatile(SWK_F16M_P_Z0_L0 : SWK_F16_OUT_M(b) : SWK_F16_IN_P(b));
        }
      } else {
        if constexpr (ZDOWN) {
          if (last) asm volatile(SWK_F16M_L_Z1_L1 : SWK_F16_OUT_M(b) : SWK_F16_IN_L(b));
          else      asm volatile(SWK_F16M_L_Z1_L0 : SWK_F16_OUT_M(b) : SWK_F16_IN_L(b));
        } else {
          if (last) asm volatile(SWK_F16M_L_Z0_L1 : SWK_F16_OUT_M(b) : SWK_F16_IN_L(b));
          else      asm volatile(SWK_F16M_L_Z0_L0 : SWK_F16_OUT_M(b) : SWK_F16_IN_L(b));
        }
      }
      up = ZDOWN ? as_u16x2(noe) : Xl[b + 7];
    }
  }
  (void)Db; (void)S1; (void)X; (void)DN; (void)IN;
  upX_ = up;
  best_ = best;
}

template <int R, int RB, bool GOTOH, bool ZDOWN, class LK>
__device__ __forceinline__ void column_f16(const LK& lk, u16x2& diag, u16x2& upX,
                                           u16x2 (&Hl)[R], u16x2 (&Xl)[R], u16x2& best,
                                           f16x2 NOE2, f16x2 NE2, f16x2 NO2) {
#if SWK_F16_ASM
  column_f16_asm<R, GOTOH, ZDOWN>(lk, diag, upX, Hl, Xl, best, as_u32(as_u16x2(NOE2)),
                                  as_u32(as_u16x2(NE2)), as_u32(as_u16x2(NO2)));
#else
  (void)NO2;
  if constexpr (GOTOH)
    column_gotoh_f16<R, RB>(lk, diag, upX, Hl, Xl, best, NOE2, NE2);
  else
    column_merged_f16<R, RB, ZDOWN>(lk, diag, upX, Hl, Xl, best, NOE2, NE2);
#endif
}

template <int R, int RB, class LK>
__device__ __forceinline__ void column_gotoh(const LK& lk, u16x2& diag, u16x2& upH, u16x2& upF,
                                             u16x2 (&Hl)[R], u16x2 (&El)[R], u16x2& best,
                                             u16x2 S2, u16x2 OES2, u16x2 E2) {
#pragma unroll
  for (int r = 0; r < R; ++r) {
    const u16x2 p = lk(r);
    const u16x2 M = vsubs(diag, p);
    const u16x2 Ei = vmax(vsubs(Hl[r], OES2), vsubs(El[r], E2));
    const u16x2 Fi = vmax(vsubs(upH, OES2), vsubs(upF, E2));
    const u16x2 Hn = vmax(vmax(M, Ei), Fi) + S2;
    best = vmax(best, M);
    diag = Hl[r];
    Hl[r] = Hn;
    El[r] = Ei;
    upH = Hn;
    upF = Fi;
    if ((r % RB) == RB - 1) __builtin_amdgcn_sched_barrier(0);
  }
}

struct Lane2 {
  const uint8_t* plo;
  const uint8_t* phi;
  uint32_t llo, lhi;
};

__device__ __forceinline__ uint2 unpack8(uint32_t b) {
  return make_uint2((b & 3u) | ((b << 6) & 0x300u) | ((b << 12) & 0x30000u) |
                        ((b << 18) & 0x3000000u),
                    ((b >> 8) & 3u) | ((b >> 2) & 0x300u) | ((b << 4) & 0x30000u) |
                        ((b << 10) & 0x3000000u));
}
__device__ __forceinline__ uint2 unpack8n(uint32_t x) {
  const uint32_t lo = x & 0x0F0F0F0Fu, hi = (x >> 4) & 0x0F0F0F0Fu;
  return make_uint2(__builtin_amdgcn_perm(hi, lo, 0x05010400u),
                    __builtin_amdgcn_perm(hi, lo, 0x07030602u));
}
__device__ __forceinline__ uint2 pad_tail(uint2 w, uint32_t j0, uint32_t len, uint32_t pad) {
  const uint32_t n = len > j0 ? min(len - j0, 8u) : 0u;
  const uint64_t keep = n >= 8 ? ~0ull : ((1ull << (8 * n)) - 1);
  const uint64_t v = ((uint64_t)w.y << 32 | w.x) & keep;
  const uint64_t p = (pad * 0x0101010101010101ull) & ~keep;
  return make_uint2((uint32_t)(v | p), (uint32_t)((v | p) >> 32));
}

template <class T>
__device__ __forceinline__ T load_u(const uint8_t* p) {
  T v;
  __builtin_memcpy(&v, p, sizeof(T));
  return v;
}
__device__ __forceinline__ uint32_t record_len(const uint8_t* rec) {
  return min((uint32_t)load_u<uint16_t>(rec + 4), SWB_RECORD_MAX);
}

constexpr uint64_t SWK_MIX_NIB = 1ull << 63;
constexpr uint64_t SWK_MIX_ADDR = (1ull << 61) - 1;
__device__ __forceinline__ const uint8_t* mixed_ptr(const uint8_t* res, uint32_t o) {
  const uint64_t p = reinterpret_cast<uint64_t>(res);
  return reinterpret_cast<const uint8_t*>(
      (o & 1u) ? (p + (o >> 1)) | SWK_MIX_NIB : (p + (o >> 3)) | (uint64_t)((o >> 1) & 3u) << 61);
}
template <int C>
__device__ __forceinline__ uint32_t mixed_word(const uint8_t* tp, uint32_t cl, bool& nib) {
  const uint64_t v = reinterpret_cast<uint64_t>(tp);
  nib = (v & SWK_MIX_NIB) != 0;
  const uint8_t* p = reinterpret_cast<const uint8_t*>(v & SWK_MIX_ADDR);
  if (nib) return C == 4 ? (uint32_t)load_u<uint16_t>(p + 2 * cl) : load_u<uint32_t>(p + 4 * cl);
  const uint32_t w = C == 4 ? (uint32_t)load_u<uint16_t>(p + cl) : load_u<uint32_t>(p + 2 * cl);
  return w >> (2u * (uint32_t)(v >> 61 & 3u));
}

__device__ __forceinline__ uint32_t pad_tail4(uint32_t w, uint32_t j0, uint32_t len, uint32_t pad) {
  const uint32_t n = len > j0 ? min(len - j0, 4u) : 0u;
  const uint32_t keep = n >= 4 ? ~0u : ((1u << (8 * n)) - 1);
  return (w & keep) | ((pad * 0x01010101u) & ~keep);
}

template <int C = 8, bool MIX = true>
__device__ __forceinline__ void load_raw(const Lane2& t, int c, bool full, uint32_t pad,
                                         uint32_t packed, uint2& lo, uint2& hi) {
  static_assert(C == 8 || C == 4, "chunks of 8 or 4 columns");
  if constexpr (C == 4) {
    const uint32_t j0 = (uint32_t)c * 4;
    uint32_t x, y;
    if (packed == SWK_PACK_NIBBLE) {
      const uint32_t cl = min((uint32_t)c, max((t.llo + 3) / 4, 1u) - 1);
      const uint32_t ch = min((uint32_t)c, max((t.lhi + 3) / 4, 1u) - 1);
      x = unpack8n(load_u<uint16_t>(t.plo + 2 * cl)).x;
      y = unpack8n(load_u<uint16_t>(t.phi + 2 * ch)).x;
    } else if (MIX && packed == SWK_PACK_MIXED) {
      const uint32_t cl = min((uint32_t)c, max((t.llo + 3) / 4, 1u) - 1);
      const uint32_t ch = min((uint32_t)c, max((t.lhi + 3) / 4, 1u) - 1);
      bool nl, nh;
      const uint32_t wl = mixed_word<4>(t.plo, cl, nl);
      const uint32_t wh = mixed_word<4>(t.phi, ch, nh);
      x = nl ? unpack8n(wl).x : unpack8(wl).x;
      y = nh ? unpack8n(wh).x : unpack8(wh).x;
    } else if (packed) {
      uint32_t cl = (uint32_t)c, ch = (uint32_t)c;
      if (packed == SWK_PACK_STREAM) {
        cl = min(cl, max((t.llo + 3) / 4, 1u) - 1);
        ch = min(ch, max((t.lhi + 3) / 4, 1u) - 1);
      }
      x = unpack8(t.plo[cl]).x;
      y = unpack8(t.phi[ch]).x;
    } else if (full) {
      x = load_u<uint32_t>(t.plo + j0);
      y = load_u<uint32_t>(t.phi + j0);
    } else {
      uint32_t b[2][4];
#pragma unroll
      for (int k = 0; k < 4; ++k) {
        const uint32_t j = j0 + k;
        const uint32_t av = t.plo[j < t.llo ? j : 0];
        const uint32_t hv = t.phi[j < t.lhi ? j : 0];
        b[0][k] = j < t.llo ? av : pad;
        b[1][k] = j < t.lhi ? hv : pad;
      }
      x = b[0][0] | b[0][1] << 8 | b[0][2] << 16 | b[0][3] << 24;
      y = b[1][0] | b[1][1] << 8 | b[1][2] << 16 | b[1][3] << 24;
    }
    if (packed && !full) {
      x = pad_tail4(x, j0, t.llo, pad);
      y = pad_tail4(y, j0, t.lhi, pad);
    }
    lo = make_uint2(x, 0u);
    hi = make_uint2(y, 0u);
    return;
  }
  const uint32_t j0 = (uint32_t)c * 8;
  if (MIX && packed == SWK_PACK_MIXED) {
    const uint32_t cl = min((uint32_t)c, max((t.llo + 7) / 8, 1u) - 1);
    const uint32_t ch = min((uint32_t)c, max((t.lhi + 7) / 8, 1u) - 1);
    bool nl, nh;
    const uint32_t wl = mixed_word<8>(t.plo, cl, nl);
    const uint32_t wh = mixed_word<8>(t.phi, ch, nh);
    lo = nl ? unpack8n(wl) : unpack8(wl);
    hi = nh ? unpack8n(wh) : unpack8(wh);
    if (!full) {
      lo = pad_tail(lo, j0, t.llo, pad);
      hi = pad_tail(hi, j0, t.lhi, pad);
    }
  } else if (packed == SWK_PACK_NIBBLE) {
    const uint32_t cl = min((uint32_t)c, max((t.llo + 7) / 8, 1u) - 1);
    const uint32_t ch = min((uint32_t)c, max((t.lhi + 7) / 8, 1u) - 1);
    lo = unpack8n(load_u<uint32_t>(t.plo + 4 * cl));
    hi = unpack8n(load_u<uint32_t>(t.phi + 4 * ch));
    if (!full) {
      lo = pad_tail(lo, j0, t.llo, pad);
      hi = pad_tail(hi, j0, t.lhi, pad);
    }
  } else if (packed) {
    uint32_t cl = (uint32_t)c, ch = (uint32_t)c;
    if (packed == SWK_PACK_STREAM) {
      cl = min(cl, max((t.llo + 7) / 8, 1u) - 1);
      ch = min(ch, max((t.lhi + 7) / 8, 1u) - 1);
    }
    const uint32_t x = load_u<uint16_t>(t.plo + 2 * cl);
    const uint32_t y = load_u<uint16_t>(t.phi + 2 * ch);
    lo = unpack8(x);
    hi = unpack8(y);
    if (!full) {
      lo = pad_tail(lo, j0, t.llo, pad);
      hi = pad_tail(hi, j0, t.lhi, pad);
    }
  } else if (full) {
    lo = load_u<uint2>(t.plo + j0);
    hi = load_u<uint2>(t.phi + j0);
  } else {
    uint32_t b[2][8];
#pragma unroll
    for (int k = 0; k < 8; ++k) {
      const uint32_t j = j0 + k;
      const uint32_t a = t.plo[j < t.llo ? j : 0];
      const uint32_t h = t.phi[j < t.lhi ? j : 0];
      b[0][k] = j < t.llo ? a : pad;
      b[1][k] = j < t.lhi ? h : pad;
    }
    lo.x = b[0][0] | b[0][1] << 8 | b[0][2] << 16 | b[0][3] << 24;
    lo.y = b[0][4] | b[0][5] << 8 | b[0][6] << 16 | b[0][7] << 24;
    hi.x = b[1][0] | b[1][1] << 8 | b[1][2] << 16 | b[1][3] << 24;
    hi.y = b[1][4] | b[1][5] << 8 | b[1][6] << 16 | b[1][7] << 24;
  }
}

template <bool MIX = true>
__device__ __forceinline__ Lane2 lane_targets(const uint8_t* res, const uint64_t* offs,
                                              const uint32_t* lens, size_t n, int tile, int lane,
                                              uint32_t packed, const uint32_t* idx,
                                              uint32_t ulen, uint32_t ustride) {
  Lane2 t;
  size_t a = (size_t)tile * SWB_TILE + lane, b = a + 64;
  const bool va = a < n, vb = b < n;
  const size_t p0 = (size_t)tile * SWB_TILE;
  if (p0 >= n) {
    t.llo = t.lhi = 0u;
    t.plo = t.phi = packed == SWK_PACK_RECORDS || ustride ? res + (packed ? 6 : 0)
                                                          : reinterpret_cast<const uint8_t*>(lens);
    return t;
  }
  if (!va) a = p0;
  if (!vb) b = p0;
  if (idx) {
    a = idx[a];
    b = idx[b];
  }
  if (packed == SWK_PACK_RECORDS) {
    t.llo = va ? record_len(res + a * SWB_RECORD) : 0u;
    t.lhi = vb ? record_len(res + b * SWB_RECORD) : 0u;
    t.plo = res + a * SWB_RECORD + 6;
    t.phi = res + b * SWB_RECORD + 6;
    return t;
  }
  if (ustride) {
    t.llo = va ? ulen : 0u;
    t.lhi = vb ? ulen : 0u;
    t.plo = res + a * ustride;
    t.phi = res + b * ustride;
    return t;
  }
  const uint32_t la = lens[a], lb = lens[b];
  t.llo = va ? la : 0u;
  t.lhi = vb ? lb : 0u;
  if constexpr (MIX) {
    if (packed == SWK_PACK_MIXED) {
      const uint32_t* o32 = reinterpret_cast<const uint32_t*>(offs);
      t.plo = la ? mixed_ptr(res, o32[a]) : reinterpret_cast<const uint8_t*>(lens);
      t.phi = lb ? mixed_ptr(res, o32[b]) : reinterpret_cast<const uint8_t*>(lens);
      return t;
    }
  }
  t.plo = la ? res + offs[a] : reinterpret_cast<const uint8_t*>(lens);
  t.phi = lb ? res + offs[b] : reinterpret_cast<const uint8_t*>(lens);
  return t;
}

template <int C = 8>
__device__ __forceinline__ void tile_chunks(const Lane2& t, size_t tlo, size_t thi, size_t n,
                                            int& nch, int& nfull, int& ncl) {
  uint32_t Lmax = max(t.llo, t.lhi);
  uint32_t Lmin = min(tlo < n ? t.llo : ~0u, thi < n ? t.lhi : ~0u);
#pragma unroll
  for (int off = 32; off >= 1; off >>= 1) {
    Lmax = max(Lmax, (uint32_t)__shfl_xor((int)Lmax, off));
    Lmin = min(Lmin, (uint32_t)__shfl_xor((int)Lmin, off));
  }
  const int lx = (int)__builtin_amdgcn_readfirstlane(Lmax);
  nch = max(1, (lx + C - 1) / C);
  ncl = lx == 0 ? C : lx - C * (nch - 1);
  const uint32_t lm = __builtin_amdgcn_readfirstlane(Lmin);
  nfull = lm == ~0u ? 0 : (int)(lm / C);
}

struct ScoreArgs {
  const uint8_t* res;
  const uint64_t* offs;
  const uint32_t* lens;
  size_t n;
  const uint32_t* qtab;
  uint32_t nv;
  uint32_t S, O, E;
  uint32_t PS;
  uint32_t pad;
  int32_t* scores;
  const uint2* edge_in;
  uint2* edge_out;
  uint32_t ecols;
  uint32_t accum;
  uint32_t packed;
  const uint32_t* idx;
  const uint32_t* nidx;
  uint32_t idx_base;
  const uint32_t* ident;
  uint32_t pS1, pS2;
  uint32_t f16_noe, f16_ne, f16_no;
  const uint32_t* fb_qtab;
  uint32_t fb_nv, fb_PS;
  int32_t fb_thresh;
  uint32_t split_blocks;
  uint32_t split_P;
  uint32_t main_pairs;
  const uint32_t* split_qtab;
  const uint32_t* split_fb_qtab;
  uint32_t split_words, split_fb_words, split_PS, split_fb_PS;
  uint2* split_ring;
  uint32_t ulen, ustride;
  uint32_t nq, qwords;
  size_t sstride;
  const SwkStreamChunk* sc;
  const uint32_t* hflag;
  uint32_t* dflag;
  uint32_t* tctr;
  uint32_t nsc;
  uint32_t* bal_flag;
  uint32_t* bal_state;
  const uint4* bal_plan;
  uint32_t bal_gen;
  uint32_t* tail_prog;
  uint32_t tail_pairs, tail_cols;
  uint32_t* fault;
  uint32_t poll_limit, stall;
  uint32_t wbal_blocks, wbal_grid;
  const uint32_t* sidx;
};
static_assert(sizeof(ScoreArgs) == 376, "ScoreArgs layout (kernel argument block) changed");

__device__ __forceinline__ void report_fault(uint32_t* fault, uint32_t bit) {
  if (fault) __hip_atomic_store(fault + __builtin_ctz(bit), bit, __ATOMIC_RELAXED,
                                __HIP_MEMORY_SCOPE_SYSTEM);
}

typedef __attribute__((address_space(3))) void* lds_void_ptr;
typedef __attribute__((address_space(1))) void* glob_void_ptr;

#define SWK_RING_ROW 65

template <int C = 8>
__device__ __forceinline__ void dma_edge_chunk(const uint2* src, uint2* dst, int lane) {
  const uint32_t* s = reinterpret_cast<const uint32_t*>(src) + lane;
#pragma unroll
  for (int q = 0; q < 2 * C; ++q)
    __builtin_amdgcn_global_load_lds(
        (glob_void_ptr)(s + q * 64),
        (lds_void_ptr)(reinterpret_cast<uint32_t*>(dst + (q >> 1) * SWK_RING_ROW) + (q & 1) * 64),
        4, 0, 0);
}

template <int C = 8>
__device__ __forceinline__ int tile_nch(const uint8_t* res, const uint32_t* lens, size_t n,
                                        int tile, int lane, uint32_t packed, const uint32_t* idx,
                                        uint32_t ulen, uint32_t ustride) {
  const size_t a = (size_t)tile * SWB_TILE + lane, b = a + 64;
  auto len = [&](size_t k) -> uint32_t {
    if (k >= n) return 0u;
    if (ustride) return ulen;
    if (idx) k = idx[k];
    return packed == SWK_PACK_RECORDS ? record_len(res + k * SWB_RECORD) : lens[k];
  };
  uint32_t L = max(len(a), len(b));
#pragma unroll
  for (int off = 32; off >= 1; off >>= 1) L = max(L, (uint32_t)__shfl_xor((int)L, off));
  return max(1, (int)((__builtin_amdgcn_readfirstlane(L) + C - 1) / C));
}

#ifndef SWK_STREAM_POLL
#define SWK_STREAM_POLL 64
#endif
#ifndef SWK_STREAM_POLL_ALL
#define SWK_STREAM_POLL_ALL 0
#endif
__device__ __forceinline__ uint32_t stream_mode(const uint32_t* hflag, uint32_t* dflag, int c,
                                                int nsc, int lane) {
  for (int it = 0; it < (1 << 20); ++it) {
    uint32_t v = __builtin_amdgcn_readfirstlane(
        __hip_atomic_load(dflag + c, __ATOMIC_ACQUIRE, __HIP_MEMORY_SCOPE_AGENT));
    if (v) {
      __builtin_amdgcn_fence(__ATOMIC_ACQUIRE, "");
      return v;
    }
    if ((SWK_STREAM_POLL_ALL || threadIdx.x < 64) &&
        (it == 0 || ((it + (int)blockIdx.x) % SWK_STREAM_POLL) == 0)) {
      v = __builtin_amdgcn_readfirstlane(
          __hip_atomic_load(hflag + c, __ATOMIC_ACQUIRE, __HIP_MEMORY_SCOPE_SYSTEM));
      if (v) {
        if (lane == 0) __hip_atomic_store(dflag + c, v, __ATOMIC_RELEASE, __HIP_MEMORY_SCOPE_AGENT);
        return v;
      }
    }
    __builtin_amdgcn_s_sleep(16);
  }
  if (lane == 0) {
    __hip_atomic_store(dflag + c, SWK_STREAM_ABORT, __ATOMIC_RELAXED, __HIP_MEMORY_SCOPE_AGENT);
    __hip_atomic_store(const_cast<uint32_t*>(hflag) + nsc + c, SWK_STREAM_ABORT,
                       __ATOMIC_RELAXED, __HIP_MEMORY_SCOPE_SYSTEM);
  }
  return SWK_STREAM_ABORT;
}


inline int cached_occupancy(const void* fn, int threads, size_t lds, int dev, int* cus) {
  struct Entry { const void* fn; int threads; size_t lds; int dev, occ, cus; };
  static std::mutex m;
  static std::vector<Entry> cache;
  std::lock_guard<std::mutex> g(m);
  for (const Entry& e : cache)
    if (e.fn == fn && e.threads == threads && e.lds == lds && e.dev == dev) {
      *cus = e.cus;
      return e.occ;
    }
  int occ = 0, c = 0;
  if (hipDeviceGetAttribute(&c, hipDeviceAttributeMultiprocessorCount, dev) != hipSuccess ||
      hipOccupancyMaxActiveBlocksPerMultiprocessor(&occ, fn, threads, lds) != hipSuccess)
    return 0;
  cache.push_back({fn, threads, lds, dev, occ, c});
  *cus = c;
  return occ;
}

inline unsigned persistent_grid(const void* fn, size_t ntiles, int threads, size_t lds) {
  int dev = 0, cus = 0;
  if (hipGetDevice(&dev) != hipSuccess) return (unsigned)ntiles;
  const int occ = cached_occupancy(fn, threads, lds, dev, &cus);
  if (cus <= 0 || occ <= 0) return (unsigned)ntiles;
  const size_t slots = (size_t)cus * occ;
  const size_t rounds = (ntiles + slots - 1) / slots;
  return (unsigned)((ntiles + rounds - 1) / rounds);
}

}
#endif
```

smith-waterman-fpga-module_amd/csrc/swbank_ktile.hip:

```cpp
#include "swbank_kcommon.h"

namespace swk {

#ifndef SWK_TRIM_BREAK
#define SWK_TRIM_BREAK 1
#endif
template <int R, int RB, bool COL0, bool PROF, bool GOTOH, bool F16, bool PAIR = false,
          bool MQ = false, bool STREAM = false, int C = 8, bool BAL = false, bool TRIM = false>
__global__ void __launch_bounds__(R >= 64 ? 512 : 1024) score_kernel(const ScoreArgs a) {
  static_assert(!BAL || (!MQ && !STREAM && !COL0), "balanced ranges: one query, resident batch");
  static_assert(!TRIM || (BAL && PAIR), "trimmed last chunks: the balanced pair kernel");
  static_assert(!MQ || !PROF, "several queries: row-LUT or pair-table variants");
  static_assert(!STREAM || (!MQ && !PROF), "streamed batches: single-query LUT / pair variants");
  static_assert(C == 8 || (C == 4 && PAIR && !STREAM), "4-column chunks: pair tables only");
  static_assert(!PAIR || ((R == 32 || (R == 16 && GOTOH)) && F16 && !PROF && !COL0 &&
                          (!GOTOH || !MQ)),
                "PAIR: f16, merged R = 32 or Gotoh R = 16 / 32 (one query)");
  extern __shared__ __attribute__((aligned(16))) uint32_t smem[];
  const int lane = threadIdx.x & 63;
  const int wave = __builtin_amdgcn_readfirstlane(threadIdx.x >> 6);
  const int W = __builtin_amdgcn_readfirstlane(blockDim.x >> 6);
  const bool seg_in = a.edge_in != nullptr, seg_out = a.edge_out != nullptr;
  uint32_t* bestsh = smem + (PAIR ? a.PS / 4 : 0);
  constexpr int RS = SWK_RING_ROW;
  uint2* ein = reinterpret_cast<uint2*>(bestsh + W * SWB_TILE);
  uint2* ring = ein + (seg_in ? 2 * C * RS : 0);
  uint8_t* prof = reinterpret_cast<uint8_t*>(ring + (size_t)(W > 1 ? 2 * (W - 1) : 1) * C * RS);

  size_t n = a.n;
  const uint32_t* idx = a.idx;
  if (idx && a.ident && __builtin_amdgcn_readfirstlane(*a.ident)) idx = nullptr;
  const uint32_t* sidx = TRIM ? a.sidx : nullptr;
  if (TRIM && sidx && a.ident && __builtin_amdgcn_readfirstlane(*a.ident)) sidx = nullptr;
  if (idx) {
    const uint32_t cnt = __builtin_amdgcn_readfirstlane(*a.nidx);
    n = cnt > a.idx_base ? min(a.n, (size_t)(cnt - a.idx_base)) : 0;
  }
  const int ntiles = (int)((n + SWB_TILE - 1) / SWB_TILE);
  const int G = (int)gridDim.x;
  const int nunits = MQ ? ntiles * (int)a.nq : ntiles;
  int total = 0;
  uint32_t packed = a.packed;
  int* sq = reinterpret_cast<int*>(prof);
  int bs = 0, bo = 0, be = 0, bf = 0;
  if constexpr (BAL) {
    const uint4 p0 = a.bal_plan[blockIdx.x], p1 = a.bal_plan[blockIdx.x + 1];
    bs = (int)__builtin_amdgcn_readfirstlane(p0.x), bo = (int)__builtin_amdgcn_readfirstlane(p0.y);
    be = (int)__builtin_amdgcn_readfirstlane(p1.x), bf = (int)__builtin_amdgcn_readfirstlane(p1.y);
    total = (int)__builtin_amdgcn_readfirstlane(p1.z - p0.z);
  }
  const auto bal_visit = [&](int v, int& t, int& c0, int& c1) {
    const int bK = -1;
    const int bfirst = bo ? bs + 1 : bs;
    const int hh = bf > 0 ? 1 : 0;
    if (v < hh) {
      t = be, c0 = 0, c1 = bf;
    } else if (v - hh < be - bfirst) {
      t = bfirst + v - hh, c0 = 0, c1 = bK;
    } else if (v - hh == be - bfirst && bo > 0) {
      t = bs, c0 = bo, c1 = bK;
    } else {
      t = nunits, c0 = 0, c1 = 1;
    }
    t = __builtin_amdgcn_readfirstlane(t);
    c0 = __builtin_amdgcn_readfirstlane(c0);
    c1 = __builtin_amdgcn_readfirstlane(c1);
  };
  if constexpr (BAL) {
  } else if constexpr (STREAM) {
    total = (int)blockIdx.x < ntiles ? (1 << 30) : 0;
  } else {
    for (int u = blockIdx.x; u < nunits; u += G)
      total += tile_nch<C>(a.res, a.lens, n, !MQ ? u : PAIR ? u / (int)a.nq : u % ntiles, lane,
                        packed, idx, a.ulen, a.ustride);
  }
  const SwkStreamChunk* const ssc = a.sc;
  const int snc = (int)a.nsc;
  int scur = -1, st0 = 0;
  uint32_t scn = 0, sro_lo = 0, sro_hi = 0, smode = SWK_PACK_STREAM;
  const uint32_t* cperm = nullptr;
  const uint32_t* wperm = nullptr;
  int wst0 = 0;
  const auto stream_tile = [&](int t, uint32_t& pk) -> Lane2 {
    if (t >= ntiles) {
      pk = SWK_PACK_STREAM;
      Lane2 e;
      e.llo = e.lhi = 0u;
      e.plo = e.phi = a.res;
      return e;
    }
    int c = scur < 0 ? 0 : scur;
    while (c + 1 < snc && t >= (int)ssc[c + 1].tile0) ++c;
    if (c != scur) {
      scur = __builtin_amdgcn_readfirstlane(c);
      st0 = __builtin_amdgcn_readfirstlane((int)ssc[c].tile0);
      scn = __builtin_amdgcn_readfirstlane(
          (uint32_t)((c + 1 < snc ? (size_t)ssc[c + 1].tile0 * SWB_TILE : n) -
                     (size_t)st0 * SWB_TILE));
      sro_lo = __builtin_amdgcn_readfirstlane(ssc[c].res_off_lo);
      sro_hi = __builtin_amdgcn_readfirstlane(ssc[c].res_off_hi);
      const uint32_t md = stream_mode(a.hflag, a.dflag, c, snc, lane);
      smode = a.ulen == 0 ? SWK_PACK_MIXED
                          : md == SWK_PACK_NIBBLE ? SWK_PACK_NIBBLE : SWK_PACK_STREAM;
      if (md == SWK_STREAM_ABORT && a.ulen == 0) {
        const uint64_t z = (uint64_t)__builtin_amdgcn_readfirstlane(ssc[c].zero_off256) * 256u;
        sro_lo = (uint32_t)z;
        sro_hi = (uint32_t)(z >> 32);
      }
    }
    pk = smode;
    const uint8_t* base = a.res + ((size_t)sro_hi << 32 | sro_lo);
    if (a.ulen == 0) {
      const uint32_t* co = reinterpret_cast<const uint32_t*>(base);
      const uint32_t* cl = co + scn;
      cperm = cl + scn;
      return lane_targets<true>(base + (((size_t)scn * 12 + 15) & ~(size_t)15),
                                reinterpret_cast<const uint64_t*>(co), cl, scn, t - st0, lane, pk,
                                cperm, 0u, 0u);
    }
    return lane_targets<true>(base, nullptr, nullptr, scn, t - st0, lane, pk, nullptr, a.ulen,
                               pk == SWK_PACK_NIBBLE ? (a.ulen + 1) / 2 : (a.ulen + 3) / 4);
  };

  int unit = blockIdx.x, q = 0;
  int tile = unit;
  int vc0 = 0, vend = 0;
  if constexpr (BAL) {
    bal_visit(0, tile, vc0, vend);
    unit = tile;
  }
  if constexpr (MQ) {
    if (unit < nunits) {
      q = PAIR ? unit % (int)a.nq : unit / ntiles;
      tile = PAIR ? unit / (int)a.nq : unit - q * ntiles;
    }
  }
  Lane2 cur;
  if constexpr (STREAM) {
    cur = stream_tile(tile, packed);
    wperm = cperm;
    wst0 = st0;
  } else {
    cur = lane_targets<!MQ>(a.res, a.offs, a.lens, n, tile, lane, packed, idx, a.ulen,
                            a.ustride);
  }
  int nch, nfull, ncl;
  tile_chunks<C>(cur, (size_t)tile * SWB_TILE + lane, (size_t)tile * SWB_TILE + lane + 64, n, nch,
              nfull, ncl);
  (void)ncl;
  if constexpr (BAL) {
    if (vend >= 0 && vend < nch) ncl = C;
    nch = vend < 0 ? nch : vend;
  }
  const uint32_t S = a.S;

  for (int i = threadIdx.x; i < W * SWB_TILE; i += blockDim.x) bestsh[i] = 0;
  const f16x2 NOE2 = as_f16x2(as_u16x2(a.f16_noe)), NE2 = as_f16x2(as_u16x2(a.f16_ne)),
              NO2 = as_f16x2(as_u16x2(a.f16_no));
  if (wave == 0) {
    if (lane < C)
      ring[lane * RS + 64] = F16 ? make_uint2(0u, GOTOH ? 0u : as_u32(as_u16x2(NOE2)))
                                 : make_uint2(S | (S << 16), 0u);
    if (seg_in)
      dma_edge_chunk<C>(a.edge_in + (size_t)(MQ ? unit : tile) * a.ecols * 64, ein, lane);
  }
  uint32_t nv = a.nv;
  uint32_t tab[PROF || PAIR ? 1 : R];
  if constexpr (PAIR) {
    const uint4* src = reinterpret_cast<const uint4*>(a.qtab + (MQ ? (size_t)q * a.qwords : 0));
    for (uint32_t i = threadIdx.x; i < a.PS / 16; i += blockDim.x)
      reinterpret_cast<uint4*>(smem)[i] = src[i];
  } else if constexpr (PROF) {
    const uint32_t words = (a.pad + 1) * a.PS / 16;
    const uint4* src = reinterpret_cast<const uint4*>(a.qtab);
    for (uint32_t i = threadIdx.x; i < words; i += blockDim.x)
      reinterpret_cast<uint4*>(prof)[i] = src[i];
  } else {
    asm volatile("" : "+v"(nv));
#pragma unroll
    for (int r = 0; r < R; ++r)
      tab[r] = __builtin_amdgcn_readfirstlane(a.qtab[(MQ ? (size_t)q * a.qwords : 0) + wave * R + r]);
  }
  const u16x2 S2 = {(unsigned short)S, (unsigned short)S};
  const u16x2 O2 = {(unsigned short)a.O, (unsigned short)a.O};
  const u16x2 E2 = {(unsigned short)a.E, (unsigned short)a.E};
  const uint32_t oes = a.O + a.E + S;
  const u16x2 OES2 = {(unsigned short)oes, (unsigned short)oes};
  const u16x2 H0 = F16 ? (u16x2){0, 0} : S2;
  const u16x2 X0 = (F16 && !GOTOH) ? as_u16x2(NOE2) : (u16x2){0, 0};

  u16x2 Hl[R], Xl[R];
#pragma unroll
  for (int r = 0; r < R; ++r) {
    Hl[r] = H0;
    Xl[r] = X0;
  }
  u16x2 best = {0, 0};
  u16x2 prevUpH = H0;
  uint2 rlo, rhi;
  load_raw<C, !MQ>(cur, vc0, vc0 < nfull, a.pad, packed, rlo, rhi);
  if (STREAM && threadIdx.x == 0) sq[W] = total;
  __syncthreads();

  typedef unsigned int u32x4 __attribute__((ext_vector_type(4)));
  typedef __attribute__((address_space(3))) const u32x4 lds_u4;
  typedef __attribute__((address_space(3))) const uint32_t lds_u32;
  const auto ld4 = [](uint32_t addr) { return __builtin_bit_cast(uint4, *(lds_u4*)(size_t)addr); };
  const auto ld1 = [](uint32_t addr) {
    return __atomic_load_n((lds_u32*)(size_t)addr, __ATOMIC_RELAXED);
  };
  const uint32_t wofs = (uint32_t)wave * R * 4 + (uint32_t)(size_t)(lds_void_ptr)smem;
  const u16x2 pS12 = {(unsigned short)a.pS1, (unsigned short)a.pS2};
  const auto pair_addr = [&](uint32_t wl, uint32_t wh, int sh) {
    const uint32_t sel = (uint32_t)(sh >> 3) | 0x0C00u | ((uint32_t)(4 + (sh >> 3)) << 16) |
                         0x0C000000u;
    const u16x2 ab = __builtin_elementwise_min(as_u16x2(__builtin_amdgcn_perm(wh, wl, sel)),
                                               (u16x2){4, 4});
    return __builtin_amdgcn_udot2(ab, pS12, wofs, false);
  };
  uint32_t acur = 0, pw = 0;
  uint4 pA0 = {0, 0, 0, 0}, pA1 = {0, 0, 0, 0};
  if constexpr (PAIR) {
    acur = pair_addr(rlo.x, rhi.x, 0);
    pA0 = ld4(acur + 16);
    pA1 = ld4(acur + 32);
    pw = ld1(acur + 12);
  }
  (void)pA0; (void)pA1; (void)pw; (void)acur; (void)wofs;

  const uint32_t pbase = (uint32_t)wave * R;
  const uint32_t padc = a.pad;
  int bal_pend = 0;
  const auto bal_store = [&](int g_to) {
    uint32_t ol = (uint32_t)lane;
    asm volatile("" : "+v"(ol));
    uint32_t* sp = a.bal_state + ((size_t)g_to * W + wave) * (2 * R + 2) * 64 + ol;
#pragma unroll
    for (int r = 0; r < R; ++r) {
      __hip_atomic_store(sp + r * 64, as_u32(Hl[r]), __ATOMIC_RELAXED, __HIP_MEMORY_SCOPE_AGENT);
      __hip_atomic_store(sp + (R + r) * 64, as_u32(Xl[r]), __ATOMIC_RELAXED,
                         __HIP_MEMORY_SCOPE_AGENT);
    }
    __hip_atomic_store(sp + 2 * R * 64, as_u32(prevUpH), __ATOMIC_RELAXED, __HIP_MEMORY_SCOPE_AGENT);
    __hip_atomic_store(sp + (2 * R + 1) * 64, as_u32(best), __ATOMIC_RELAXED,
                       __HIP_MEMORY_SCOPE_AGENT);
    bal_pend = 2;
  };
  const auto bal_flag_out = [&]() {
    asm volatile("s_waitcnt vmcnt(0)" ::: "memory");
    if (lane == 0 && blockIdx.x + 1 != a.stall)
      __hip_atomic_store(a.bal_flag + ((size_t)blockIdx.x + 1) * W + wave, a.bal_gen,
                         __ATOMIC_RELAXED, __HIP_MEMORY_SCOPE_AGENT);
  };
#if SWK_STAMPS
  uint64_t st_bload = 0;
#endif
  const auto bal_load = [&]() {
#if SWK_STAMPS
    const uint64_t sb0 = __builtin_amdgcn_s_memtime();
#endif
    const uint32_t* fl = a.bal_flag + (size_t)blockIdx.x * W + wave;
    uint32_t it = 0;
    for (; it < a.poll_limit; ++it) {
      if (__builtin_amdgcn_readfirstlane(
              __hip_atomic_load(fl, __ATOMIC_RELAXED, __HIP_MEMORY_SCOPE_AGENT)) == a.bal_gen)
        break;
      __builtin_amdgcn_s_sleep(8);
    }
    if (it == a.poll_limit && lane == 0) report_fault(a.fault, SWK_FAULT_BAL);
    asm volatile("s_waitcnt vmcnt(0)" ::: "memory");
    uint32_t ol = (uint32_t)lane;
    asm volatile("" : "+v"(ol));
    const uint32_t* sp = a.bal_state + ((size_t)blockIdx.x * W + wave) * (2 * R + 2) * 64 + ol;
#pragma unroll
    for (int r = 0; r < R; ++r) {
      Hl[r] = as_u16x2(__hip_atomic_load(sp + r * 64, __ATOMIC_RELAXED, __HIP_MEMORY_SCOPE_AGENT));
      Xl[r] = as_u16x2(
          __hip_atomic_load(sp + (R + r) * 64, __ATOMIC_RELAXED, __HIP_MEMORY_SCOPE_AGENT));
    }
    prevUpH = as_u16x2(
        __hip_atomic_load(sp + 2 * R * 64, __ATOMIC_RELAXED, __HIP_MEMORY_SCOPE_AGENT));
    best = as_u16x2(
        __hip_atomic_load(sp + (2 * R + 1) * 64, __ATOMIC_RELAXED, __HIP_MEMORY_SCOPE_AGENT));
#if SWK_STAMPS
    asm volatile("s_waitcnt vmcnt(0)" ::: "memory");
    st_bload += __builtin_amdgcn_s_memtime() - sb0;
#endif
  };
  (void)bal_store; (void)bal_load; (void)bal_flag_out;
  int c = vc0, k = 0;
  int nch_n = 1, nfull_n = 0, ncl_n = C;
  uint32_t packed_n = packed;
#if SWK_PRIO_ROT
  const uint32_t prq = (uint32_t)((blockIdx.x * 4ull) / gridDim.x);
  uint32_t prio = 4;
#endif
#if SWK_STAMPS
  uint64_t st_t0 = __builtin_amdgcn_s_memtime(), st_act = 0, st_idle = 0, st_bar = 0;
  uint64_t st_p = st_t0;
#endif
  for (int ph = 0;; ++ph) {
    if constexpr (STREAM) total = __builtin_amdgcn_readfirstlane(sq[W]);
    if (ph >= total + W - 1) break;
#if SWK_PRIO_ROT
    if (W <= 8)
      prio_rotate(prq, prio,
                  SWK_PRIO_END && ph >= total - (total >> SWK_PRIO_END_FRAC)
                      ? SWK_PRIO_SHIFT - SWK_PRIO_END : SWK_PRIO_SHIFT);

#endif
    const int g = ph - wave;
    if (g >= 0 && g < total) {
      const uint2 clo = rlo, chi = rhi;
      const bool last = c + 1 == nch;
      int nunit = (MQ ? unit : tile) + G;
      int nc0 = 0, nvend = 0;
      if constexpr (BAL) {
        if (last) bal_visit(k + 1, nunit, nc0, nvend);
      }
      if constexpr (STREAM) {
        if (last) {
          if (wave == 0) {
            int nt = 0;
            if (lane == 0) nt = G + (int)atomicAdd(a.tctr, 1u);
            nt = min(__builtin_amdgcn_readfirstlane(nt), ntiles);
            if (lane == 0) {
              sq[(k + 1) % W] = nt;
              if (nt >= ntiles) sq[W] = g + 1;
            }
            nunit = nt;
          } else {
            nunit = __builtin_amdgcn_readfirstlane(sq[(k + 1) % W]);
          }
        }
      }
      int ntile = nunit, nqq = q;
      if constexpr (MQ) {
        if (nunit < nunits) {
          if constexpr (PAIR) {
            ntile = nunit / (int)a.nq;
          } else {
            ntile = tile + G;
            while (ntile >= ntiles) {
              ntile -= ntiles;
              ++nqq;
            }
          }
        }
      }
      if (!last) {
        load_raw<C, !MQ>(cur, c + 1, c + 1 < nfull, a.pad, packed, rlo, rhi);
      } else if (nunit < nunits) {
        if constexpr (STREAM) cur = stream_tile(ntile, packed_n);
        else
          cur = lane_targets<!MQ>(a.res, a.offs, a.lens, n, ntile, lane, packed, idx, a.ulen,
                                  a.ustride);
        tile_chunks<C>(cur, (size_t)ntile * SWB_TILE + lane, (size_t)ntile * SWB_TILE + lane + 64,
                    n, nch_n, nfull_n, ncl_n);
        if (BAL && nvend >= 0 && nvend < nch_n) ncl_n = C;
        if (BAL && nvend < 0) nvend = nch_n;
        load_raw<C, !MQ>(cur, nc0, nc0 < nfull_n, a.pad, STREAM ? packed_n : packed, rlo, rhi);
      }
      const int slot = g & 1;
      if (seg_in && wave == 0 && (last ? nunit < nunits : (MQ ? unit : tile) < nunits))
        dma_edge_chunk<C>(a.edge_in + ((size_t)(last ? nunit : MQ ? unit : tile) * a.ecols +
                                    (size_t)(last ? 0 : c + 1) * C) * 64,
                       ein + (size_t)((g + 1) & 1) * C * RS, lane);
      uint2* rin = wave > 0 ? ring + ((size_t)((wave - 1) * 2 + slot) * C) * RS + lane
                   : seg_in ? ein + (size_t)slot * C * RS + lane
                            : ring + 64;
      uint2* rout = wave < W - 1 ? ring + ((size_t)(wave * 2 + slot) * C) * RS + lane
                    : W > 1      ? rin
                                 : ring + lane;
      uint2 rv = rin[0];
      ProfLookup16<PROF && F16 ? R : 2> lkq;
      (void)lkq;
      const int ncols = TRIM && c + 1 == nch ? ncl : C;
      bool trimmed = false;
      (void)ncols;
#pragma unroll
      for (int jj = 0; jj < C; ++jj) {
        if (TRIM && jj > 0 && __builtin_expect(jj >= ncols, 0)) {
          trimmed = true;
#if SWK_TRIM_BREAK
          break;
#else
          continue;
#endif
        }
        const u16x2 upH = as_u16x2(rv.x);
        u16x2 upX = as_u16x2(rv.y);
        if (jj + 1 < C) rv = rin[(jj + 1) * RS];
        u16x2 diag = prevUpH;
        prevUpH = upH;
        const uint32_t wlo = jj < 4 ? clo.x : clo.y, whi = jj < 4 ? chi.x : chi.y;
        if constexpr (PROF && F16) {
          const auto load16 = [&](int j, ProfLookup16<R>& out) {
            const uint32_t wl = j < 4 ? clo.x : clo.y, wh = j < 4 ? chi.x : chi.y;
            const uint32_t blo = min((wl >> (8 * (j & 3))) & 0xFFu, padc);
            const uint32_t bhi = min((wh >> (8 * (j & 3))) & 0xFFu, padc);
            const uint4* plo = reinterpret_cast<const uint4*>(prof + __umul24(blo, a.PS) + 2 * pbase);
            const uint4* phi = reinterpret_cast<const uint4*>(prof + __umul24(bhi, a.PS) + 2 * pbase);
#pragma unroll
            for (int q = 0; q < R / 8; ++q) {
              const uint4 x = plo[q], y = phi[q];
              out.lo[4 * q] = x.x; out.lo[4 * q + 1] = x.y; out.lo[4 * q + 2] = x.z;
              out.lo[4 * q + 3] = x.w;
              out.hi[4 * q] = y.x; out.hi[4 * q + 1] = y.y; out.hi[4 * q + 2] = y.z;
              out.hi[4 * q + 3] = y.w;
            }
          };
          ProfLookup16<R> lk;
          if (jj == 0) load16(0, lk);
          else lk = lkq;
          if (jj + 1 < C) load16(jj + 1, lkq);
          __builtin_amdgcn_sched_barrier(0);
          if (COL0 && jj == 0 && c == 0)
            column_f16<R, RB, GOTOH, true>(lk, diag, upX, Hl, Xl, best, NOE2, NE2, NO2);
          else
            column_f16<R, RB, GOTOH, false>(lk, diag, upX, Hl, Xl, best, NOE2, NE2, NO2);
        } else if constexpr (PROF) {
          ProfLookup<R> lk;
          const uint32_t blo = min((wlo >> (8 * (jj & 3))) & 0xFFu, padc);
          const uint32_t bhi = min((whi >> (8 * (jj & 3))) & 0xFFu, padc);
          const uint4* plo = reinterpret_cast<const uint4*>(prof + __umul24(blo, a.PS) + pbase);
          const uint4* phi = reinterpret_cast<const uint4*>(prof + __umul24(bhi, a.PS) + pbase);
#pragma unroll
          for (int q = 0; q < R / 16; ++q) {
            const uint4 x = plo[q], y = phi[q];
            lk.lo[4 * q] = x.x; lk.lo[4 * q + 1] = x.y; lk.lo[4 * q + 2] = x.z;
            lk.lo[4 * q + 3] = x.w;
            lk.hi[4 * q] = y.x; lk.hi[4 * q + 1] = y.y; lk.hi[4 * q + 2] = y.z;
            lk.hi[4 * q + 3] = y.w;
          }
          __builtin_amdgcn_sched_barrier(0);
          if constexpr (GOTOH) {
            u16x2 uH = upH;
            column_gotoh<R, RB>(lk, diag, uH, upX, Hl, Xl, best, S2, OES2, E2);
          } else if (COL0 && jj == 0 && c == 0) {
            column_merged<R, RB, true>(lk, diag, upX, Hl, Xl, best, S2, O2, E2);
          } else {
            column_merged<R, RB, false>(lk, diag, upX, Hl, Xl, best, S2, O2, E2);
          }
        } else if constexpr (PAIR) {
          const uint32_t nwl = jj + 1 < C ? (jj + 1 < 4 ? clo.x : clo.y) : rlo.x;
          const uint32_t nwh = jj + 1 < C ? (jj + 1 < 4 ? chi.x : chi.y) : rhi.x;
          const int nsh = jj + 1 < C ? 8 * ((jj + 1) & 3) : 0;
          uint32_t Da, Db, X, DN, IN;
          const uint32_t noe = as_u32(as_u16x2(NOE2)), ne = as_u32(as_u16x2(NE2)),
                 no = as_u32(as_u16x2(NO2));
          u16x2 bst = best;
          u16x2 F = upX;
#define SWK_PAIR_HT(B)                                                                        \
  [h0] "+v"(Hl[B]), [h1] "+v"(Hl[B + 1]), [h2] "+v"(Hl[B + 2]), [h3] "+v"(Hl[B + 3]),          \
      [h4] "+v"(Hl[B + 4]), [h5] "+v"(Hl[B + 5]), [h6] "+v"(Hl[B + 6]), [h7] "+v"(Hl[B + 7]),  \
      [t0] "+v"(Xl[B]), [t1] "+v"(Xl[B + 1]), [t2] "+v"(Xl[B + 2]), [t3] "+v"(Xl[B + 3]),      \
      [t4] "+v"(Xl[B + 4]), [t5] "+v"(Xl[B + 5]), [t6] "+v"(Xl[B + 6]), [t7] "+v"(Xl[B + 7]),  \
      [Db] "=&v"(Db), [best] "+v"(bst)
#define SWK_PAIR_OUT(B, DA) SWK_PAIR_HT(B), [Da] DA(Da), [X] "=&v"(X), [DN] "=&v"(DN), [IN] "=&v"(IN)
#define SWK_PAIR_OUTG(B, DA)                                                                  \
  SWK_PAIR_HT(B), [Da] DA(Da), [EN] "=&v"(X), [HN] "=&v"(DN), [FN] "=&v"(IN), [F] "+v"(F)
#define SWK_PAIR_IN(P0, P1)                                                                   \
  [p0] "v"(P0.x), [p1] "v"(P0.y), [p2] "v"(P0.z), [p3] "v"(P0.w), [p4] "v"(P1.x),             \
      [p5] "v"(P1.y), [p6] "v"(P1.z), [p7] "v"(P1.w), [noe] "s"(noe), [ne] "s"(ne), [no] "s"(no)
#define SWK_PAIR_BLOCK(KIND, B, P0, P1)                                                       \
  if constexpr (GOTOH) {                                                                      \
    if constexpr (KIND == 0)                                                                  \
      asm volatile(SWK_F16PAIRG_F : SWK_PAIR_OUTG(B, "=&v")                                   \
                   : SWK_PAIR_IN(P0, P1), [dg] "v"(diag), [pw] "v"(pw));                   \
    else if constexpr (KIND == 1)                                                             \
      asm volatile(SWK_F16PAIRG_M : SWK_PAIR_OUTG(B, "+v") : SWK_PAIR_IN(P0, P1));         \
    else                                                                                      \
      asm volatile(SWK_F16PAIRG_L : SWK_PAIR_OUTG(B, "+v") : SWK_PAIR_IN(P0, P1));         \
  } else {                                                                                    \
    if constexpr (KIND == 0)                                                                  \
      asm volatile(SWK_F16PAIR_F : SWK_PAIR_OUT(B, "=&v")                                     \
                   : SWK_PAIR_IN(P0, P1), [up] "v"(upX), [dg] "v"(diag), [pw] "v"(pw));                 \
    else if constexpr (KIND == 1)                                                             \
      asm volatile(SWK_F16PAIR_M : SWK_PAIR_OUT(B, "+v") : SWK_PAIR_IN(P0, P1), [up] "v"(Xl[B - 1]));   \
    else                                                                                      \
      asm volatile(SWK_F16PAIR_L : SWK_PAIR_OUT(B, "+v") : SWK_PAIR_IN(P0, P1), [up] "v"(Xl[B - 1]));   \
  }
          uint4 pB0 = ld4(acur + 48), pB1 = ld4(acur + 64);
          __builtin_amdgcn_sched_barrier(0);
          SWK_PAIR_BLOCK(0, 0, pA0, pA1)
          if constexpr (R == 32) {
            pA0 = ld4(acur + 80);
            pA1 = ld4(acur + 96);
            __builtin_amdgcn_sched_barrier(0);
            SWK_PAIR_BLOCK(1, 8, pB0, pB1)
            pB0 = ld4(acur + 112);
            pB1 = ld4(acur + 128);
            __builtin_amdgcn_sched_barrier(0);
            SWK_PAIR_BLOCK(1, 16, pA0, pA1)
          }
          acur = pair_addr(nwl, nwh, nsh);
          pA0 = ld4(acur + 16);
          pA1 = ld4(acur + 32);
          pw = ld1(acur + 12);
          __builtin_amdgcn_sched_barrier(0);
          SWK_PAIR_BLOCK(2, R - 8, pB0, pB1)
#undef SWK_PAIR_BLOCK
#undef SWK_PAIR_HT
#undef SWK_PAIR_OUT
#undef SWK_PAIR_OUTG
#undef SWK_PAIR_IN
          (void)Db; (void)X; (void)DN; (void)IN;
          best = bst;
          upX = GOTOH ? F : Xl[R - 1];
        } else if constexpr (F16) {
          const uint32_t sel16 = 0x0Cu | ((uint32_t)(jj & 3) << 8) | (0x0Cu << 16) |
                                 ((uint32_t)(4 + (jj & 3)) << 24);
          const LutLookup<R> lk{tab, nv, __builtin_amdgcn_perm(whi, wlo, sel16) | 0x000C000Cu};
          __builtin_amdgcn_sched_barrier(0);
          if (COL0 && jj == 0 && c == 0)
            column_f16<R, RB, GOTOH, true>(lk, diag, upX, Hl, Xl, best, NOE2, NE2, NO2);
          else
            column_f16<R, RB, GOTOH, false>(lk, diag, upX, Hl, Xl, best, NOE2, NE2, NO2);
        } else {
          const uint32_t sel =
              (uint32_t)(jj & 3) | ((uint32_t)(4 + (jj & 3)) << 16) | 0x0C000C00u;
          const LutLookup<R> lk{tab, nv, __builtin_amdgcn_perm(whi, wlo, sel) | 0x0C000C00u};
          __builtin_amdgcn_sched_barrier(0);
          if constexpr (GOTOH) {
            u16x2 uH = upH;
            column_gotoh<R, RB>(lk, diag, uH, upX, Hl, Xl, best, S2, OES2, E2);
          } else if (COL0 && jj == 0 && c == 0) {
            column_merged<R, RB, true>(lk, diag, upX, Hl, Xl, best, S2, O2, E2);
          } else {
            column_merged<R, RB, false>(lk, diag, upX, Hl, Xl, best, S2, O2, E2);
          }
        }
        asm volatile("" : "+v"(best));
        rout[jj * RS] = make_uint2(as_u32(Hl[R - 1]), as_u32(upX));
      }
      if constexpr (PAIR && TRIM) {
        if (trimmed) {
          acur = pair_addr(rlo.x, rhi.x, 0);
          pA0 = ld4(acur + 16);
          pA1 = ld4(acur + 32);
          pw = ld1(acur + 12);
        }
      }
      (void)trimmed;
      if (seg_out && wave == W - 1) {
        uint2* dst = a.edge_out + ((size_t)(MQ ? unit : tile) * a.ecols + (size_t)c * C) * 64 + lane;
#pragma unroll
        for (int jj = 0; jj < C; ++jj) dst[jj * 64] = rout[jj * RS];
      }
      if (last) {
        if (BAL && k == 0 && bf > 0) {
          bal_store((int)blockIdx.x + 1);
        } else {
        uint32_t* bs = bestsh + (k % W) * SWB_TILE;
        atomicMax(&bs[lane], (uint32_t)best.x);
        atomicMax(&bs[lane + 64], (uint32_t)best.y);
        if (wave == W - 1) {
          const size_t tlo = (size_t)tile * SWB_TILE + lane, thi = tlo + 64;
          int32_t blo = (int32_t)bs[lane], bhi = (int32_t)bs[lane + 64];
          bs[lane] = 0;
          bs[lane + 64] = 0;
          if constexpr (F16) {
            blo = f16_unscore((uint32_t)blo);
            bhi = f16_unscore((uint32_t)bhi);
          }
          const uint32_t* sx = TRIM && sidx ? sidx : idx;
          size_t slo = sx && tlo < n ? sx[tlo] : tlo;
          size_t shi = sx && thi < n ? sx[thi] : thi;
          if constexpr (STREAM) {
            if (wperm) {
              const size_t b0 = (size_t)wst0 * SWB_TILE;
              if (tlo < n) slo = b0 + wperm[tlo - b0];
              if (thi < n) shi = b0 + wperm[thi - b0];
            }
          }
          int32_t* qsc = MQ ? a.scores + (size_t)q * a.sstride : a.scores;
          if (a.accum) {
            if (tlo < n) blo = max(blo, qsc[slo]);
            if (thi < n) bhi = max(bhi, qsc[shi]);
          }
          if (tlo < n) qsc[slo] = blo;
          if (thi < n) qsc[shi] = bhi;
        }
        }
#pragma unroll
        for (int r = 0; r < R; ++r) {
          Hl[r] = H0;
          Xl[r] = X0;
        }
        best = (u16x2){0, 0};
        prevUpH = H0;
        tile = ntile;
        if constexpr (STREAM) {
          packed = packed_n;
          wperm = cperm;
          wst0 = st0;
        }
        if constexpr (MQ && PAIR) unit = nunit;
        if constexpr (MQ && !PAIR) {
          unit = nunit;
          if (nqq != q) {
            q = nqq;
#pragma unroll
            for (int r = 0; r < R; ++r)
              tab[r] = __builtin_amdgcn_readfirstlane(a.qtab[(size_t)q * a.qwords + wave * R + r]);
          }
        }
        nch = nch_n;
        nfull = nfull_n;
        ncl = ncl_n;
        c = 0;
        if constexpr (BAL) {
          c = nc0;
          nch = nvend;
          if (nc0 > 0) bal_load();
        }
        ++k;
      } else {
        ++c;
      }
    }
    if constexpr (BAL) {
      if (bal_pend > 0 && --bal_pend == 0) bal_flag_out();
    }
#if SWK_STAMPS
    const bool st_own = g >= 0 && g < total;
    const uint64_t st_b = __builtin_amdgcn_s_memtime();
    (st_own ? st_act : st_idle) += st_b - st_p;
#endif
    __syncthreads();
#if SWK_STAMPS
    st_p = __builtin_amdgcn_s_memtime();
    (st_own ? st_bar : st_idle) += st_p - st_b;
#endif
  }
  if constexpr (BAL) {
    if (bal_pend > 0) bal_flag_out();
  }
#if SWK_STAMPS
  uint64_t* const g_stamps = STREAM ? nullptr : reinterpret_cast<uint64_t*>(a.tctr);
  if (lane == 0 && g_stamps) {
    uint64_t* o = g_stamps + ((size_t)blockIdx.x * 16 + wave) * 16;
    unsigned hw = 0;
    asm volatile("s_getreg_b32 %0, hwreg(HW_REG_HW_ID)" : "=s"(hw));
    o[0] = st_t0;
    o[1] = __builtin_amdgcn_s_memtime();
    o[2] = st_act;
    o[3] = st_idle;
    o[4] = st_bar;
    o[5] = hw;
    unsigned xcc = 0;
    asm volatile("s_getreg_b32 %0, hwreg(HW_REG_XCC_ID)" : "=s"(xcc));
    o[6] = (uint64_t)total;
    o[7] = (uint64_t)(xcc & 15);
    o[8] = st_bload;
  }
#endif
}

static size_t tile_ring_entries(int W, int C, bool seg_in) {
  return (size_t)((W > 1 ? 2 * (W - 1) : 1) + (seg_in ? 2 : 0)) * C * SWK_RING_ROW;
}

template <int R, int RB, bool COL0, bool PROF, bool GOTOH, bool F16, bool PAIR = false,
          bool MQ = false, bool STREAM = false, int C = 8, bool BAL = false, bool TRIM = false>
static hipError_t launch_score(const ScoreArgs& a, int W, uint32_t prof_bytes, hipStream_t st,
                               unsigned bal_grid = 0) {
  const size_t ntiles = (a.n + SWB_TILE - 1) / SWB_TILE * (MQ ? a.nq : 1);
  const size_t lds = (size_t)W * SWB_TILE * 4 + tile_ring_entries(W, C, a.edge_in != nullptr) * 8 +
                     (PROF ? prof_bytes : 0) + (PAIR ? a.PS : 0) + (STREAM ? 256 : 0);
  auto fn = &score_kernel<R, RB, COL0, PROF, GOTOH, F16, PAIR, MQ, STREAM, C, BAL, TRIM>;
  static bool attr_set = false;
  if (!attr_set) {
    hipError_t e = hipFuncSetAttribute(reinterpret_cast<const void*>(fn),
                                       hipFuncAttributeMaxDynamicSharedMemorySize, 160 * 1024);
    if (e != hipSuccess) return e;
    attr_set = true;
  }
  if (lds > 160 * 1024) return hipErrorInvalidConfiguration;
  unsigned grid = BAL ? bal_grid
                      : persistent_grid(reinterpret_cast<const void*>(fn), ntiles, 64 * W, lds);
#if SWK_STAMPS
  if (!STREAM && g_stamps_host) {
    ScoreArgs b = a;
    b.tctr = reinterpret_cast<uint32_t*>(g_stamps_host);
    hipLaunchKernelGGL(fn, dim3(grid), dim3(64 * W), (unsigned)lds, st, b);
    return hipGetLastError();
  }
#endif
  if (MQ && PAIR) grid = std::max(a.nq, grid / a.nq * a.nq);
  if (BAL && (grid == 0 || ntiles < 2 * (size_t)grid)) return hipErrorInvalidConfiguration;
  hipLaunchKernelGGL(fn, dim3(grid), dim3(64 * W), (unsigned)lds, st, a);
  return hipGetLastError();
}

}

#define SWK_VARIANTS(X)                                                                       \
  X(16, 4, 0, 0, 0, 0) X(16, 4, 1, 0, 0, 0) X(32, 4, 0, 0, 0, 0) X(32, 4, 1, 0, 0, 0)         \
  X(32, 8, 0, 0, 0, 0) X(64, 4, 0, 0, 0, 0) X(64, 4, 1, 0, 0, 0)                              \
  X(16, 4, 0, 0, 1, 0) X(32, 4, 0, 0, 1, 0) X(64, 4, 0, 0, 1, 0)                              \
  X(16, 4, 0, 1, 0, 0) X(16, 4, 1, 1, 0, 0) X(32, 4, 0, 1, 0, 0) X(32, 4, 1, 1, 0, 0)         \
  X(64, 4, 0, 1, 0, 0) X(64, 4, 1, 1, 0, 0)                                                   \
  X(16, 4, 0, 1, 1, 0) X(32, 4, 0, 1, 1, 0) X(64, 4, 0, 1, 1, 0)                              \
  X(16, 4, 0, 0, 0, 1) X(16, 4, 1, 0, 0, 1) X(32, 4, 0, 0, 0, 1) X(64, 4, 0, 0, 0, 1)         \
  X(16, 4, 0, 0, 1, 1)                                                                        \
  X(16, 4, 0, 1, 0, 1) X(16, 4, 1, 1, 0, 1) X(16, 4, 0, 1, 1, 1) X(32, 4, 0, 0, 1, 1)


extern "C" int swk_has_variant(int R, int RB, int col0, int prof, int gotoh, int f16) {
#define SWK_HAS(RR, BB, C0, PF, GT, FH) \
  if (R == RR && RB == BB && col0 == C0 && prof == PF && gotoh == GT && f16 == FH) return 1;
  SWK_VARIANTS(SWK_HAS)
#undef SWK_HAS
  return 0;
}

extern "C" hipError_t swk_launch_score(int R, int RB, int col0, int prof, int gotoh, int f16,
                                       const uint8_t* res, const uint64_t* offs,
                                       const uint32_t* lens, size_t n, const uint32_t* qtab,
                                       uint32_t nv, uint32_t S, uint32_t O, uint32_t E,
                                       uint32_t PS, uint32_t pad, int W, int32_t* scores,
                                       const void* edge_in, void* edge_out, uint32_t ecols,
                                       int accum, int packed, const uint32_t* idx,
                                       const uint32_t* nidx, uint32_t idx_base,
                                       const uint32_t* ident, int pair, uint32_t pS1,
                                       uint32_t pS2, uint32_t ulen, uint32_t ustride,
                                       uint32_t nq, uint32_t qwords, size_t sstride,
                                       hipStream_t st) {
  if (n == 0) return hipSuccess;
  swk::ScoreArgs a{res,  offs, lens, n,  qtab, nv, S,
                   O,    E,    PS,   pad, scores, static_cast<const uint2*>(edge_in),
                   static_cast<uint2*>(edge_out), ecols, (uint32_t)accum, (uint32_t)packed,
                   idx, nidx, idx_base, ident, pS1, pS2,
                   swk::f16_pair(-(int)(O + E)), swk::f16_pair(-(int)E),
                   swk::f16_pair(-(int)O), nullptr, 0u, 0u, 0};
  a.ulen = ulen;
  a.ustride = ustride;
  a.nq = nq;
  a.qwords = qwords;
  a.sstride = sstride;
  const uint32_t prof_bytes = (pad + 1) * PS;
  if (nq > 1 && pair) {
    if (R == 32 && f16 && !prof && !gotoh && !col0 && (W > 4 || a.edge_in || a.edge_out))
      return swk::launch_score<32, 4, false, false, false, true, true, true, false, 4>(a, W, 0, st);
    if (R == 32 && f16 && !prof && !gotoh && !col0)
      return swk::launch_score<32, 4, false, false, false, true, true, true>(a, W, 0, st);
    return hipErrorInvalidValue;
  }
  if (nq > 1) {
#define SWK_MQ_CASE(RR, GT, FH)                                                                  \
  if (R == RR && RB == 4 && !col0 && !prof && !pair && gotoh == GT && f16 == FH)                 \
    return swk::launch_score<RR, 4, false, false, (GT != 0), (FH != 0), false, true>(a, W, 0, st);
    SWK_MQ_CASE(32, 0, 1) SWK_MQ_CASE(32, 0, 0) SWK_MQ_CASE(16, 0, 1) SWK_MQ_CASE(16, 0, 0)
    SWK_MQ_CASE(16, 1, 1) SWK_MQ_CASE(16, 1, 0) SWK_MQ_CASE(32, 1, 1) SWK_MQ_CASE(32, 1, 0)
#undef SWK_MQ_CASE
    return hipErrorInvalidValue;
  }
  if (pair) {
    if (R == 32 && f16 && !prof && !gotoh && !col0)
      return swk::launch_score<32, 4, false, false, false, true, true>(a, W, 0, st);
#define SWK_GPAIR(RR)                                                                         \
    if (R == RR && f16 && !prof && gotoh && !col0) {                                          \
      const hipError_t e = a.edge_in || a.edge_out                                            \
          ? hipErrorInvalidConfiguration                                                      \
          : swk::launch_score<RR, 4, false, false, true, true, true>(a, W, 0, st);            \
      if (e != hipErrorInvalidConfiguration) return e;                                        \
      return swk::launch_score<RR, 4, false, false, true, true, true, false, false, 4>(a, W, 0, \
                                                                                         st); \
    }
    SWK_GPAIR(32) SWK_GPAIR(16)
#undef SWK_GPAIR
    return hipErrorInvalidValue;
  }
#define SWK_CASE(RR, BB, C0, PF, GT, FH)                                                      \
  if (R == RR && RB == BB && col0 == C0 && prof == PF && gotoh == GT && f16 == FH)            \
    return swk::launch_score<RR, BB, (C0 != 0), (PF != 0), (GT != 0), (FH != 0)>(a, W,        \
                                                                               prof_bytes, st);
  SWK_VARIANTS(SWK_CASE)
#undef SWK_CASE
  return hipErrorInvalidValue;
}

#if SWK_STAMPS
extern "C" void swk_set_stamps(void* p) { swk::g_stamps_host = static_cast<uint64_t*>(p); }
#endif

namespace swk {
__global__ void __launch_bounds__(256) bal_plan_uniform(uint4* plan, uint32_t ntiles, uint32_t K,
                                                        uint32_t G) {
  for (uint32_t g = threadIdx.x; g <= G; g += blockDim.x) {
    const uint64_t A = (uint64_t)ntiles * K * g / G;
    plan[g] = make_uint4((uint32_t)(A / K), (uint32_t)(A % K), (uint32_t)A, 0u);
  }
}
}

extern "C" hipError_t swk_bal_plan_uniform(void* plan, uint32_t ntiles, uint32_t K, uint32_t G,
                                           hipStream_t st) {
  if (!plan || K == 0 || G == 0 || (uint64_t)ntiles * K >= (1ull << 31)) return hipErrorInvalidValue;
  hipLaunchKernelGGL(swk::bal_plan_uniform, dim3(1), dim3(256), 0, st, static_cast<uint4*>(plan),
                     ntiles, K, G);
  return hipGetLastError();
}

extern "C" unsigned swk_bal_slots(int W, uint32_t PS, int trim) {
  const void* fn =
      trim ? reinterpret_cast<const void*>(
                 &swk::score_kernel<32, 4, false, false, false, true, true, false, false, 8, true,
                                    true>)
           : reinterpret_cast<const void*>(
                 &swk::score_kernel<32, 4, false, false, false, true, true, false, false, 8, true>);
  if (hipFuncSetAttribute(fn, hipFuncAttributeMaxDynamicSharedMemorySize, 160 * 1024) !=
      hipSuccess)
    return 0;
  const size_t lds = (size_t)W * SWB_TILE * 4 + swk::tile_ring_entries(W, 8, false) * 8 + PS;
  int dev = 0, cus = 0;
  if (hipGetDevice(&dev) != hipSuccess) return 0;
  const int occ = swk::cached_occupancy(fn, 64 * W, lds, dev, &cus);
  return occ > 0 && cus > 0 ? (unsigned)(occ * cus) : 0u;
}

extern "C" hipError_t swk_launch_pair_bal(const uint8_t* res, const uint64_t* offs,
                                          const uint32_t* lens, size_t n, const uint32_t* qtab,
                                          uint32_t nv, uint32_t S, uint32_t O, uint32_t E,
                                          uint32_t PS, uint32_t pad, int W, int32_t* scores,
                                          uint32_t pS1, uint32_t pS2, uint32_t ulen,
                                          uint32_t ustride, uint32_t* flag, uint32_t* state,
                                          uint32_t gen, unsigned grid, const uint32_t* idx,
                                          const uint32_t* nidx, const uint32_t* ident,
                                          const void* plan, uint32_t* fault, uint32_t poll_limit,
                                          uint32_t stall, int trim, uint32_t packed,
                                          const uint32_t* sidx, hipStream_t st) {
  if (n == 0) return hipSuccess;
  if (W > 4 || !flag || !state || !plan || !fault || poll_limit == 0 || (idx && !nidx) ||
      (packed != SWK_PACK_BYTES && packed != SWK_PACK_NIBBLE) || (sidx && (!trim || idx)))
    return hipErrorInvalidValue;
  swk::ScoreArgs a{res,  offs, lens, n,  qtab, nv, S,
                   O,    E,    PS,   pad, scores, nullptr, nullptr, 0u, 0u, packed,
                   idx, nidx, 0u, ident, pS1, pS2,
                   swk::f16_pair(-(int)(O + E)), swk::f16_pair(-(int)E),
                   swk::f16_pair(-(int)O), nullptr, 0u, 0u, 0};
  a.ulen = ulen;
  a.ustride = ustride;
  a.nq = 1;
  a.bal_flag = flag;
  a.bal_state = state;
  a.bal_gen = gen;
  a.bal_plan = static_cast<const uint4*>(plan);
  a.fault = fault;
  a.poll_limit = poll_limit;
  a.stall = stall;
  a.sidx = sidx;
  if (trim)
    return swk::launch_score<32, 4, false, false, false, true, true, false, false, 8, true, true>(
        a, W, 0, st, grid);
  return swk::launch_score<32, 4, false, false, false, true, true, false, false, 8, true>(
      a, W, 0, st, grid);
}

extern "C" hipError_t swk_launch_stream(int R, int gotoh, int f16, int pair, const uint8_t* res,
                                        size_t n, uint32_t ulen, const SwkStreamChunk* sc,
                                        const uint32_t* hflag, uint32_t* dflag, uint32_t nsc,
                                        uint32_t* tctr, const uint32_t* qtab, uint32_t nv,
                                        uint32_t S, uint32_t O, uint32_t E, uint32_t PS,
                                        uint32_t pad, int W, int32_t* scores, uint32_t pS1,
                                        uint32_t pS2, hipStream_t st) {
  if (n == 0) return hipSuccess;
  if (!sc || !hflag || !dflag || !tctr || nsc == 0) return hipErrorInvalidValue;
  swk::ScoreArgs a{res,  nullptr, nullptr, n, qtab, nv, S, O, E, PS, pad, scores, nullptr, nullptr,
                   0u, 0u, (uint32_t)SWK_PACK_STREAM, nullptr, nullptr, 0u, nullptr, pS1, pS2,
                   swk::f16_pair(-(int)(O + E)), swk::f16_pair(-(int)E),
                   swk::f16_pair(-(int)O), nullptr, 0u, 0u, 0};
  a.ulen = ulen;
  a.sc = sc;
  a.hflag = hflag;
  a.dflag = dflag;
  a.tctr = tctr;
  a.nsc = nsc;
  if (pair) {
    if (R == 32 && f16 && !gotoh)
      return swk::launch_score<32, 4, false, false, false, true, true, false, true>(a, W, 0, st);
    if (R == 32 && f16 && gotoh)
      return swk::launch_score<32, 4, false, false, true, true, true, false, true>(a, W, 0, st);
    if (R == 16 && f16 && gotoh)
      return swk::launch_score<16, 4, false, false, true, true, true, false, true>(a, W, 0, st);
    return hipErrorInvalidValue;
  }
#define SWK_ST_CASE(RR, GT, FH)                                                                  \
  if (R == RR && gotoh == GT && f16 == FH)                                                       \
    return swk::launch_score<RR, 4, false, false, (GT != 0), (FH != 0), false, false, true>(     \
        a, W, 0, st);
  SWK_ST_CASE(32, 0, 1) SWK_ST_CASE(32, 0, 0) SWK_ST_CASE(16, 0, 1) SWK_ST_CASE(16, 0, 0)
  SWK_ST_CASE(16, 1, 1) SWK_ST_CASE(16, 1, 0) SWK_ST_CASE(32, 1, 1) SWK_ST_CASE(32, 1, 0)
#undef SWK_ST_CASE
  return hipErrorInvalidValue;
}
```

smith-waterman-fpga-module_amd/csrc/swbank_launch.hip:

```cpp
#include "swbank_bank.h"

static bool one_len_bin(uint32_t min_len, uint32_t max_len) {
  if (min_len > max_len) return false;
  uint32_t shift = 0;
  while ((max_len >> shift) >= 2048u) ++shift;
  return ((max_len - min_len) >> shift) == 0;
}

void u16_gotoh_rows(const sw_bank* b, bool f16, int& R, int& W) {
  if (f16 || !b->gotoh() || b->prof || R != 32 || b->segs.size() != 1 || b->query.size() > 256)
    return;
  R = 16;
  W = std::max(1, (int)((b->query.size() + 15) / 16));
}

bool wave_preferred(const sw_bank* b, size_t n, uint32_t max_len, bool use_f16) {
  const size_t nseg = b->segs.size();
  const size_t ntiles = (n + SWB_TILE - 1) / SWB_TILE;
  const bool gotoh = b->cfg.gap_model == SW_GAP_GOTOH;
  const double tiles = (double)ntiles, W = b->segs[0].W;
  const double cu_frac = std::min(1.0, tiles / 256.0);
  const double wps = std::min(4.0, std::max(1.0, std::ceil(tiles / 256.0)) * W / 4.0);
  const bool pair_tab = use_f16 && b->pair_bytes != 0 && env_int("SWBANK_PAIR", 1) != 0;
  const double tile_base = use_f16 ? (gotoh ? (b->prof ? 7100 : pair_tab ? 8500 : 7500)
                                            : (b->prof ? 8000 : 9000))
                                   : (gotoh ? (b->prof ? 5600 : 5800) : (b->prof ? 6500 : 7400));
  const double tile_est = tile_base * cu_frac * std::min(1.0, 0.45 + 0.15 * wps) *
                          (nseg > 1 ? 0.85 : 1.0);
  double wave_est = 0;
  if (b->wK > 0) {
    const double rowfill = (double)b->query.size() / (64.0 * b->wK * b->wsegs);
    const double colfill = max_len / (max_len + 63.0);
    const double wave_base = use_f16 ? (gotoh ? (b->prof ? 6800 : 7800) : (b->prof ? 7700 : 8600))
                                     : (gotoh ? (b->prof ? 5200 : 6100) : (b->prof ? 6600 : 7600));
    wave_est = wave_base * rowfill * colfill *
               (b->wsegs > 1 ? 0.9 : 1.0);
  }
  const char* kforce = std::getenv("SWBANK_KERNEL");
  bool use_wave = b->wK > 0 && wave_est > tile_est;
  if (kforce && std::strcmp(kforce, "tile") == 0) use_wave = false;
  if (kforce && std::strcmp(kforce, "wave") == 0 && b->wK > 0) use_wave = true;
  return use_wave;
}

static uint32_t poll_limit(uint32_t dflt) {
  const int v = env_int("SWBANK_POLL_LIMIT", 0);
  return v > 0 ? (uint32_t)v : dflt;
}

static int ragged_trim() { return env_int("SWBANK_TRIM", 1) != 0 ? 1 : 0; }

sw_status launch(sw_bank* b, const uint8_t* d_res, const uint64_t* d_offs,
                 const uint32_t* d_lens, size_t n, uint32_t max_len, int32_t* d_scores,
                 hipStream_t st, uint32_t packed, const uint32_t* perm, const uint32_t* perm_n,
                 bool dsort, bool wait_prev, uint32_t* sort_out, uint32_t* sort_scr, uint32_t ulen,
                 uint32_t ustride, uint32_t min_len) {
  const uint64_t bound = std::min<uint64_t>(b->query.size(), max_len) *
                             (uint64_t)std::max(0, b->smax) + (uint64_t)std::max(0, b->smax);
  const bool need32 = bound > 65535u || env_int("SWBANK_I32", 0) != 0;
  if (need32 && ustride) return fail(b, SW_ERR_ARG, "uniform batch past the 16-bit bound");
  if (need32) {
    if (n > 0xFFFFFFFFull)
      return fail(b, SW_ERR_RANGE, "batches past the 16-bit score bound hold < 2^32 targets");
    const sw_status ps = prepare_i32(b);
    if (ps != SW_OK) return ps;
  }
  sw_bank::Ev ev{};
  if (b->timing) {
    HIPOK(b, hipEventCreate(&ev.a));
    HIPOK(b, hipEventCreate(&ev.c));
    HIPOK(b, hipEventRecord(ev.a, st));
    ev.b = ev.a;
  }
  HIPOK(b, hipStreamWaitEvent(st, b->ev_ready, 0));
  if (wait_prev) HIPOK(b, hipStreamWaitEvent(st, b->ev_used, 0));
  const size_t nseg = b->segs.size();
  const bool rec = packed == SWK_PACK_RECORDS;
  const uint32_t ecols = (max_len + 7) / 8 * 8;
  const size_t ntiles = (n + SWB_TILE - 1) / SWB_TILE;
  const bool gotoh = b->cfg.gap_model == SW_GAP_GOTOH;
  const uint64_t top = std::min<uint64_t>(b->query.size(), max_len) * (uint64_t)std::max(0, b->smax) +
                       (uint64_t)std::max(0, b->smax);
  const bool f16_ok = b->f16 && b->f16_neg >= -2048 && env_int("SWBANK_F16", 1) != 0;
  const bool exact16 = f16_ok && top <= 2048u;
  const bool opt16 = f16_ok && !exact16 && n <= 0xFFFFFFFFull;
  const bool use_f16 = exact16 || opt16;
  bool use_wave = wave_preferred(b, n, max_len, use_f16);
  if (packed == SWK_PACK_MIXED) use_wave = false;
  if (use_f16 && b->prof && (size_t)(b->alpha + 1) * b->wPS16 > 65536) use_wave = false;
  const char* arith = opt16 ? "f16+u16-rescore" : use_f16 ? "f16" : "u16";
  const bool use_pair = use_f16 && b->pair_bytes != 0 && env_int("SWBANK_PAIR", 1) != 0;
  bool wave_fb = false;
  if (use_wave) {
    const bool half = use_f16 && b->prof && !b->col0 && b->wK == 8 && b->wsegs == 1 &&
                      env_int("SWBANK_WAVE_HALF", 1) != 0;
    snprintf(b->last_kernel, sizeof(b->last_kernel), "wave %s%s K=%d segs=%d%s", arith,
             b->prof ? "-profile" : "", b->wK, b->wsegs, half ? " pairs/wave=2" : "");
    size_t wspan = n;
    if (b->wsegs > 1) {
      const size_t budget = (size_t)std::max(1, env_int("SWBANK_EDGE_MB", 2048)) << 20;
      wspan = std::min(n, std::max<size_t>(1, budget / ((size_t)ecols * sizeof(uint2))) * 2);
      const size_t words = std::max<size_t>(1, (wspan + 1) / 2 * ecols);
      HIPOK(b, b->edge[0].reserve(words));
      HIPOK(b, b->edge[1].reserve(words));
    }
    wave_fb = opt16 && b->wsegs == 1;
    SwkWaveSplit sp{};
    const size_t pairs = (n + 1) / 2;
    const int sforce = env_int("SWBANK_WAVE_SPLIT", -1);
    bool wbal = false;
    if (half && b->wsegs == 1 && n == wspan && !b->no_handoff && (ustride || min_len == max_len) &&
        sforce < 0 && pairs <= 0xFFFFFFFFull && env_int("SWBANK_WAVE_BAL", 1) != 0) {
      const size_t U = (pairs + 1) / 2, B = (max_len + 31 + 31) / 32;
      const int wforce = env_int("SWBANK_WAVE_W", 0);
      int W = wforce == 4 ? 4 : 8;
      unsigned grid = swk_wave_half_grid(gotoh ? 1 : 0, (b->pad + 1) * b->wPS16, W);
      bool ok = W == 8 && swk_wbal_admissible(U, B, 8, grid) &&
                (wforce == 8 || U >= (size_t)8 * grid);
      if (!ok) {
        W = 4;
        grid = swk_wave_half_grid(gotoh ? 1 : 0, (b->pad + 1) * b->wPS16, W);
        const size_t G4 = (size_t)4 * grid;
        ok = swk_wbal_admissible(U, B, 4, grid) && U >= G4 && U % G4;
      }
      const size_t G = (size_t)W * grid;
      uint32_t* fw = ok ? fault_word(b) : nullptr;
      if (ok && fw) {
        const size_t sw = (G + 1) * 36 * 64;
        HIPOK(b, b->wbal_state.reserve(sw));
        if (b->wbal_flag.cap < G + 1) {
          HIPOK(b, b->wbal_flag.reserve(G + 1));
          HIPOK(b, hipMemsetAsync(b->wbal_flag.p, 0, b->wbal_flag.cap * 4, st));
        }
        sp.wbal_blocks = (uint32_t)B;
        sp.wbal_grid = grid;
        sp.wbal_waves = (unsigned)W;
        sp.wbal_gen = ++b->wbal_gen;
        sp.wbal_flag = b->wbal_flag.p;
        sp.wbal_state = b->wbal_state.p;
        sp.fault = fw + (b->host_call ? SWK_FAULT_WORDS : 0);
        sp.poll_limit = poll_limit(1u << 23);
        sp.stall = (unsigned)std::max(0, env_int("SWBANK_STALL", 0));
        wbal = true;
        const size_t L = strlen(b->last_kernel);
        snprintf(b->last_kernel + L, sizeof(b->last_kernel) - L, " balanced grid=%ux%d", grid, W);
      }
    }
    if (!wbal && b->sK[0] && b->wsegs == 1 && n == wspan && pairs <= 0xFFFFFFFFull) {
      const size_t simds = 4 * (size_t)std::max(b->cus, 1);
      const size_t units = half ? 2 * simds : simds;
      size_t T = 0;
      if (sforce >= 0) T = std::min(pairs, (size_t)sforce);
      else if (pairs >= units && pairs % units <= units / 2) T = pairs % units;
      const int pforce = env_int("SWBANK_WAVE_SPLIT_P", 0);
      const bool seg8 = half && b->sK[2] == 1 && T && !b->no_handoff &&
                        (pforce == 8 || (!pforce && 8 * T <= simds));
      const int i = pforce == 2 ? 0 : pforce == 4 ? 1 : (4 * T <= simds ? 1 : 0);
      uint32_t* fw = seg8 ? fault_word(b) : nullptr;
      if (seg8 && !fw) return fail(b, SW_ERR_NOMEM, "fault word allocation failed");
      if (seg8) {
        HIPOK(b, b->sring.reserve(std::max<size_t>(1, T * 7 * (size_t)ecols)));
        const size_t pw = T * 8 * 3;
        HIPOK(b, b->tprog.reserve(pw));
        HIPOK(b, hipMemsetAsync(b->tprog.p, 0, pw * 4, st));
        sp.pairs = (unsigned)T;
        sp.P = 8;
        sp.qtab = b->stab16[2].p;
        sp.words = (unsigned)b->sseg_words16[2];
        sp.PS = b->sPS16[2];
        sp.ring = b->sring.p;
        sp.cols = ecols;
        sp.prog = b->tprog.p;
        sp.fault = fw + (b->host_call ? SWK_FAULT_WORDS : 0);
        sp.poll_limit = poll_limit(1u << 24);
        sp.stall = (unsigned)std::max(0, env_int("SWBANK_STALL", 0));
        const size_t L = strlen(b->last_kernel);
        snprintf(b->last_kernel + L, sizeof(b->last_kernel) - L, " tail=%zu/8", T);
      } else if (T && b->sK[i]) {
        const unsigned P = 2u << i;
        HIPOK(b, b->sring.reserve((T + 4 / P - 1) / (4 / P) * (4 / P) * (P - 1) * 256));
        sp.pairs = (unsigned)T;
        sp.P = P;
        sp.qtab = use_f16 ? b->stab16[i].p : b->stab[i].p;
        sp.words = (unsigned)(use_f16 ? b->sseg_words16[i] : b->sseg_words[i]);
        sp.PS = use_f16 && b->prof ? b->sPS16[i] : b->sPS[i];
        sp.fb_qtab = b->stab[i].p;
        sp.fb_words = (unsigned)b->sseg_words[i];
        sp.fb_PS = b->sPS[i];
        sp.ring = b->sring.p;
        const size_t L = strlen(b->last_kernel);
        snprintf(b->last_kernel + L, sizeof(b->last_kernel) - L, " split=%zu/%u", T, P);
      }
    }
    for (size_t p0 = 0; p0 < n; p0 += wspan) {
      const size_t np = std::min(wspan, n - p0);
      for (int sg = 0; sg < b->wsegs; ++sg) {
        const void* ein = sg > 0 ? b->edge[(sg - 1) & 1].p : nullptr;
        void* eout = sg + 1 < b->wsegs ? b->edge[sg & 1].p : nullptr;
        HIPOK(b, swk_launch_wave(
                     b->wK, b->col0, b->prof, gotoh ? 1 : 0, use_f16 ? 1 : 0, ein, eout, ecols,
                     sg > 0 ? 1 : 0, rec ? d_res + p0 * SWB_RECORD : d_res,
                     rec ? d_offs : d_offs + p0, rec ? d_lens : d_lens + p0, np,
                     use_f16 ? b->wtab16.p + sg * b->wseg_words16 : b->wtab.p + sg * b->wseg_words,
                     use_f16 ? b->nv16 : b->nv, b->S, b->O, b->E,
                     use_f16 && b->prof ? b->wPS16 : b->wPS, b->pad, d_scores + p0,
                     (int)packed, wave_fb ? b->wtab.p : nullptr, b->nv, b->wPS,
                     2048 - std::max(0, b->smax), &sp, ulen, ustride, half ? 1 : 0, st));
      }
    }
  } else {
    int R0 = b->R, W0 = b->segs[0].W;
    u16_gotoh_rows(b, use_f16, R0, W0);
    snprintf(b->last_kernel, sizeof(b->last_kernel), "tile %s%s R=%d W=%d segs=%zu", arith,
             b->prof ? "-profile" : use_pair ? " pair" : "", R0, W0, nseg);
  }
  const uint32_t* ident = nullptr;
  unsigned rbal_grid = 0;
  if (dsort && !sort_out && !b->no_handoff && !use_wave && !perm && use_f16 && use_pair && !gotoh && nseg == 1 &&
      wait_prev && (packed == SWK_PACK_BYTES || packed == SWK_PACK_NIBBLE) && min_len < max_len &&
      max_len < 2048 && !opt16 &&
      b->R == 32 && b->segs[0].W <= 4 && n <= 0xFFFFFFFFull && env_int("SWBANK_DSORT", 1) != 0 &&
      env_int("SWBANK_BAL", 1) != 0 && env_int("SWBANK_BAL_RAGGED", 1) != 0 &&
      !one_len_bin(min_len, max_len)) {
    const unsigned grid = swk_bal_slots(b->segs[0].W, b->pair_bytes, ragged_trim());
    const size_t kmin = std::max<uint32_t>(1u, (min_len + 7) / 8), kmax = (max_len + 7) / 8;
    if (grid && ntiles * kmin >= 2 * (size_t)grid * kmax && ntiles * kmax < (1ull << 31))
      rbal_grid = grid;
  }
  if (dsort && !use_wave && !perm && packed != SWK_PACK_RECORDS && ntiles > 1 &&
      n <= 0xFFFFFFFFull && !one_len_bin(min_len, max_len) && env_int("SWBANK_DSORT", 1) != 0) {
    uint32_t* order = sort_out;
    if (!order) {
      HIPOK(b, b->dperm.reserve(n + 2));
      order = b->dperm.p;
    }
    uint32_t* scr = sort_scr;
    if (!scr) {
      const size_t sw = swk_sort_scratch_bytes() / 4;
      if (b->dsort.cap < sw) {
        HIPOK(b, b->dsort.reserve(sw));
        HIPOK(b, hipMemsetAsync(b->dsort.p, 0, sw * 4, st));
      }
      scr = b->dsort.p;
    }
    if (rbal_grid) {
      HIPOK(b, b->bal_plan.reserve((size_t)(rbal_grid + 1) * 4));
      b->bal_key[0] = 0;
    }
    HIPOK(b, swk_sort_lens(d_lens, n, max_len, order, order + n, order + n + 1, scr, st,
                           rbal_grid ? b->bal_plan.p : nullptr, rbal_grid));
    ++b->ctr.device_sorts;
    if (!sort_out) {
      const size_t L = strlen(b->last_kernel);
      snprintf(b->last_kernel + L, sizeof(b->last_kernel) - L, " dsort");
    }
    perm = order;
    perm_n = order + n;
    ident = order + n + 1;
  }
  size_t span = n;
  if (nseg > 1) {
    const size_t budget = (size_t)std::max(1, env_int("SWBANK_EDGE_MB", 2048)) << 20;
    const size_t per_tile = (size_t)ecols * 64 * sizeof(uint2);
    span = std::max<size_t>(1, budget / std::max<size_t>(per_tile, 1)) * SWB_TILE;
    span = std::min(span, n);
    if (!use_wave || opt16) {
      const size_t words = std::max<size_t>(1, (span + SWB_TILE - 1) / SWB_TILE * ecols * 64);
      HIPOK(b, b->edge[0].reserve(words));
      HIPOK(b, b->edge[1].reserve(words));
    }
  }
  for (int pass = use_wave ? 1 : 0; pass < (opt16 && !wave_fb ? 2 : 1); ++pass) {
    const bool f16 = use_f16 && pass == 0;
    if (pass == 1) {
      HIPOK(b, b->fb_idx.reserve(n));
      HIPOK(b, b->fb_cnt.reserve(1));
      HIPOK(b, swk_flag_high(d_scores, n, 2048 - std::max(0, b->smax), b->fb_idx.p, b->fb_cnt.p,
                             st));
    }
    for (size_t p0 = 0; p0 < n; p0 += span) {
      const size_t np = std::min(span, n - p0);
      const uint8_t* res = d_res;
      const uint64_t* offs = d_offs;
      const uint32_t* lens = d_lens;
      int32_t* scores = d_scores;
      const uint32_t* idx = nullptr;
      const uint32_t* nidx = nullptr;
      if (pass == 0 && perm) {
        idx = perm + p0;
        nidx = perm_n;
      } else if (pass == 0 && rec) {
        res = d_res + p0 * SWB_RECORD;
        scores = d_scores + p0;
      } else if (pass == 0) {
        offs = d_offs + p0;
        lens = d_lens + p0;
        scores = d_scores + p0;
      } else {
        idx = b->fb_idx.p + p0;
        nidx = b->fb_cnt.p;
      }
      const bool rbal = pass == 0 && rbal_grid && perm && idx == perm && span == n;
      if (rbal || (pass == 0 && !b->no_handoff && f16 && use_pair && !gotoh && nseg == 1 && !idx && wait_prev &&
                   (packed == SWK_PACK_BYTES || packed == SWK_PACK_NIBBLE) && min_len == max_len &&
                   max_len > 0 && span == n &&
                   ntiles * ((max_len + 7) / 8) < (1ull << 31) && !opt16 && b->R == 32 &&
                   b->segs[0].W <= 4 && env_int("SWBANK_BAL", 1) != 0)) {
        const int Wl = b->segs[0].W;
        const unsigned grid = rbal ? rbal_grid : swk_bal_slots(Wl, b->pair_bytes, 0);
        uint32_t* fw = fault_word(b);
        if (!fw) return fail(b, SW_ERR_NOMEM, "fault word allocation failed");
        if (grid && (rbal || ntiles >= 2 * (size_t)grid)) {
          const size_t sw = (size_t)(grid + 1) * Wl * (2 * 32 + 2) * 64;
          HIPOK(b, b->bal_state.reserve(sw));
          if (b->bal_flag.cap < (size_t)(grid + 1) * Wl) {
            HIPOK(b, b->bal_flag.reserve((size_t)(grid + 1) * Wl));
            HIPOK(b, hipMemsetAsync(b->bal_flag.p, 0, b->bal_flag.cap * 4, st));
          }
          if (!rbal) {
            const size_t K = (max_len + 7) / 8;
            if (b->bal_key[0] != ntiles || b->bal_key[1] != K || b->bal_key[2] != grid) {
              HIPOK(b, b->bal_plan.reserve((size_t)(grid + 1) * 4));
              HIPOK(b, swk_bal_plan_uniform(b->bal_plan.p, (uint32_t)ntiles, (uint32_t)K, grid,
                                            st));
              b->bal_key[0] = ntiles;
              b->bal_key[1] = K;
              b->bal_key[2] = grid;
            }
          }
          const int gmode = rbal && ragged_trim() && packed == SWK_PACK_BYTES
                                ? env_int("SWBANK_RAGGED_GATHER", 0) : 0;
          const bool gat = gmode != 0;
          const bool gnib = gat && gmode == 2 && b->alpha <= 16;
          SwkDeal dl{};
          if (gat) {
            const size_t stride = ((gnib ? ((size_t)max_len + 7) / 8 * 4 : (size_t)max_len) + 15) &
                                  ~(size_t)15;
            HIPOK(b, b->gres.reserve(n * stride + 16));
            HIPOK(b, b->goffs.reserve(n));
            HIPOK(b, b->glens.reserve(n));
            dl.D = 1;
            dl.stride = (unsigned)stride;
            dl.codes[0] = b->gres.p;
            dl.offs[0] = reinterpret_cast<unsigned long long*>(b->goffs.p);
            dl.lens[0] = b->glens.p;
            dl.cnt[0] = n;
            dl.nib = gnib ? 1u : 0u;
            HIPOK(b, swk_deal_gather(res, offs, lens, idx, ident, n, &dl, st));
          }
          HIPOK(b, swk_launch_pair_bal(gat ? b->gres.p : res, gat ? b->goffs.p : offs,
                                       gat ? b->glens.p : lens, np, b->qpair.p, b->nv16, b->S, b->O,
                                       b->E, b->pair_bytes, b->pad, Wl,
                                       scores, b->pS1, b->pS2, ulen,
                                       ustride, b->bal_flag.p, b->bal_state.p, ++b->bal_gen, grid,
                                       gat ? nullptr : idx, gat ? nullptr : nidx,
                                       ident, b->bal_plan.p,
                                       fw + (b->host_call ? SWK_FAULT_WORDS : 0), poll_limit(1u << 23),
                                       (uint32_t)std::max(0, env_int("SWBANK_STALL", 0)),
                                       rbal && ragged_trim(),
                                       gnib ? (uint32_t)SWK_PACK_NIBBLE
                                            : gat ? (uint32_t)SWK_PACK_BYTES : packed,
                                       gat ? idx : nullptr, st));
          ++b->ctr.balanced_calls;
          const size_t L = strlen(b->last_kernel);
          snprintf(b->last_kernel + L, sizeof(b->last_kernel) - L, " balanced grid=%u%s", grid,
                   gnib ? " gather4" : gat ? " gather" : "");
          continue;
        }
      }
      for (size_t s = 0; s < nseg; ++s) {
        const void* ein = s > 0 ? b->edge[(s - 1) & 1].p : nullptr;
        void* eout = s + 1 < nseg ? b->edge[s & 1].p : nullptr;
        const bool pair = f16 && use_pair;
        int R = b->R, Wl = b->segs[s].W;
        u16_gotoh_rows(b, f16, R, Wl);
        HIPOK(b, swk_launch_score(R, b->RB, b->col0, b->prof, gotoh ? 1 : 0, f16 ? 1 : 0, res,
                                  offs, lens, np,
                                  pair ? b->qpair.p + s * (b->pair_bytes / 4)
                                  : f16 ? b->qtab16.p + b->segs[s].off16
                                        : b->qtab.p + b->segs[s].off,
                                  f16 ? b->nv16 : b->nv, b->S, b->O, b->E,
                                  pair ? b->pair_bytes : f16 && b->prof ? b->PS16 : b->PS,
                                  b->pad, Wl, scores, ein, eout, ecols, s > 0 ? 1 : 0,
                                  (int)packed, idx, nidx, (uint32_t)p0,
                                  pass == 0 ? ident : nullptr, pair ? 1 : 0, b->pS1, b->pS2,
                                  ulen, ustride, 1u, 0u, 0, st));
      }
    }
  }
  if (need32) {
    const uint32_t scols = std::max(max_len, 1u);
    const size_t budget = (size_t)std::max(1, env_int("SWBANK_EDGE_MB", 2048)) << 20;
    const size_t waves = swk_i32_waves(n, scols, budget);
    HIPOK(b, b->fb_idx.reserve(n));
    HIPOK(b, b->fb_cnt.reserve(1));
    HIPOK(b, b->i32scr.reserve(waves * 2 * scols));
    const int32_t thresh = bound > 65535u ? 65535 - std::max(0, b->smax) : -1;
    HIPOK(b, swk_flag_high(d_scores, n, thresh, b->fb_idx.p, b->fb_cnt.p, st));
    HIPOK(b, swk_launch_i32(gotoh ? 1 : 0, d_res, d_offs, d_lens, n, (int)packed, b->fb_idx.p,
                            b->fb_cnt.p, 0, b->i32prof.p, b->i32_strips,
                            (uint32_t)b->query.size(), b->pad, b->O, b->E, d_scores, b->i32scr.p,
                            scols, waves, st));
    const size_t L = strlen(b->last_kernel);
    snprintf(b->last_kernel + L, sizeof(b->last_kernel) - L, " +i32-rescore");
  }
  HIPOK(b, hipEventRecord(b->ev_used, st));
  if (b->timing) {
    HIPOK(b, hipEventRecord(ev.c, st));
    b->events.push_back(ev);
  }
  return SW_OK;
}

sw_status track_best_device(sw_bank* b, const int32_t* d_scores, const uint64_t* d_ids, size_t n,
                            hipStream_t st) {
  if (n > 0xFFFFFFFFull) return SW_OK;
  HIPOK(b, b->best_key.reserve(1));
  HIPOK(b, b->best_dev.reserve(3));
  HIPOK(b, swk_best_hit(d_scores, d_ids, n, b->best_key.p, b->best_dev.p, b->best_dev.p + 2, st));
  if (!b->best_ev) HIPOK(b, hipEventCreateWithFlags(&b->best_ev, hipEventDisableTiming));
  HIPOK(b, hipEventRecord(b->best_ev, st));
  b->best_kind = 2;
  return SW_OK;
}

sw_status launch_set(sw_bank* b, const uint8_t* d_res, const uint64_t* d_offs,
                     const uint32_t* d_lens, size_t n, uint32_t min_len, uint32_t max_len,
                     int32_t* d_scores, hipStream_t st, size_t sstride) {
  const size_t nq = b->qset.size();
  const uint64_t smax = (uint64_t)std::max(0, b->smax);
  const uint64_t top = std::min<uint64_t>(b->query.size(), max_len) * smax + smax;
  const bool f16_ok = b->f16 && b->f16_neg >= -2048 && env_int("SWBANK_F16", 1) != 0;
  const bool use_f16 = f16_ok && top <= 2048u;
  const bool exact = use_f16 || top <= 65535u;
  const size_t ntiles = (n + SWB_TILE - 1) / SWB_TILE;
  const char* kforce = std::getenv("SWBANK_KERNEL");
  const bool mq = env_int("SWBANK_MQ", 1) != 0 && !b->prof && !b->col0 && exact &&
                  env_int("SWBANK_I32", 0) == 0 && (b->R == 16 || b->R == 32) && b->RB == 4 &&
                  n <= 0xFFFFFFFFull &&
                  !(kforce && std::strcmp(kforce, "wave") == 0) && ntiles * nq <= 0x7FFFFFFFull;
  if (!mq) {
    const std::vector<uint8_t> longest = b->query;
    sw_status rs = SW_OK;
    for (size_t i = 0; i < nq && rs == SW_OK; ++i) {
      b->query = b->qset[i];
      b->dirty = true;
      rs = prepare(b);
      if (rs == SW_OK)
        rs = launch(b, d_res, d_offs, d_lens, n, max_len, d_scores + i * sstride, st, SWK_PACK_BYTES,
                    nullptr, nullptr, true, true, nullptr, nullptr, 0, 0, min_len);
    }
    b->query = longest;
    b->dirty = true;
    const size_t L = strlen(b->last_kernel);
    snprintf(b->last_kernel + L, sizeof(b->last_kernel) - L, " x%zu queries", nq);
    return rs;
  }
  sw_status rs = prepare_multi(b);
  if (rs != SW_OK) return rs;
  const bool gotoh = b->gotoh();
  const int prow = std::max(b->mq_pair_rows, 32);
  const size_t slots = (prow > 256 ? 1 : prow > 128 ? 2 : 4) * (size_t)std::max(b->cus, 1);
  const bool mpair = b->mq_pair_segs > 0 && use_f16 && nq <= slots &&
                     8 * (slots - slots / nq * nq) <= slots;
  const size_t nseg = mpair ? (size_t)b->mq_pair_segs : b->segs.size();
  snprintf(b->last_kernel, sizeof(b->last_kernel), "tile %s%s R=%d W=%d segs=%zu queries=%zu",
           use_f16 ? "f16" : "u16", mpair ? " pair" : "", b->R,
           mpair ? std::min(prow / 32, (int)(b->query.size() + 31) / 32) : b->segs[0].W, nseg,
           nq);
  HIPOK(b, hipStreamWaitEvent(st, b->ev_ready, 0));
  HIPOK(b, hipStreamWaitEvent(st, b->ev_used, 0));
  sw_bank::Ev ev{};
  if (b->timing) {
    HIPOK(b, hipEventCreate(&ev.a));
    HIPOK(b, hipEventCreate(&ev.c));
    HIPOK(b, hipEventRecord(ev.a, st));
    ev.b = ev.a;
  }
  const uint32_t ecols = (max_len + 7) / 8 * 8;
  const uint32_t *perm = nullptr, *perm_n = nullptr, *ident = nullptr;
  if (ntiles > 1 && !one_len_bin(min_len, max_len) && env_int("SWBANK_DSORT", 1) != 0) {
    HIPOK(b, b->dperm.reserve(n + 2));
    const size_t sw = swk_sort_scratch_bytes() / 4;
    if (b->dsort.cap < sw) {
      HIPOK(b, b->dsort.reserve(sw));
      HIPOK(b, hipMemsetAsync(b->dsort.p, 0, sw * 4, st));
    }
    HIPOK(b, swk_sort_lens(d_lens, n, max_len, b->dperm.p, b->dperm.p + n, b->dperm.p + n + 1,
                           b->dsort.p, st));
    ++b->ctr.device_sorts;
    perm = b->dperm.p;
    perm_n = b->dperm.p + n;
    ident = b->dperm.p + n + 1;
  }
  size_t span = n;
  if (nseg > 1) {
    const size_t budget = (size_t)std::max(1, env_int("SWBANK_EDGE_MB", 2048)) << 20;
    const size_t per_tile = (size_t)ecols * 64 * sizeof(uint2) * nq;
    span = std::min(n, std::max<size_t>(1, budget / per_tile) * SWB_TILE);
    const size_t words = (span + SWB_TILE - 1) / SWB_TILE * ecols * 64 * nq;
    HIPOK(b, b->edge[0].reserve(words));
    HIPOK(b, b->edge[1].reserve(words));
  }
  const uint32_t* tabs = use_f16 ? b->mqtab16.p : b->mqtab.p;
  for (size_t p0 = 0; p0 < n; p0 += span) {
    const size_t np = std::min(span, n - p0);
    const uint64_t* offs = perm ? d_offs : d_offs + p0;
    const uint32_t* lens = perm ? d_lens : d_lens + p0;
    int32_t* scores = perm ? d_scores : d_scores + p0;
    for (size_t sg = 0; sg < nseg; ++sg) {
      const void* ein = sg > 0 ? b->edge[(sg - 1) & 1].p : nullptr;
      void* eout = sg + 1 < nseg ? b->edge[sg & 1].p : nullptr;
      if (mpair) {
        const int rows = std::min(prow, (int)b->query.size() - (int)sg * prow);
        const int Wp = std::max(1, (rows + 31) / 32);
        HIPOK(b, swk_launch_score(32, 4, 0, 0, 0, 1, d_res, offs, lens, np,
                                  b->mqpair.p + sg * nq * b->mq_pair_words, b->nv16, b->S, b->O,
                                  b->E, (uint32_t)b->mq_pair_words * 4, b->pad, Wp, scores, ein,
                                  eout, ecols, sg > 0 ? 1 : 0, (int)SWK_PACK_BYTES,
                                  perm ? perm + p0 : nullptr, perm_n, (uint32_t)p0, ident, 1,
                                  b->mq_pS1, b->mq_pS2, 0, 0, (uint32_t)nq,
                                  (uint32_t)b->mq_pair_words, sstride, st));
        continue;
      }
      HIPOK(b, swk_launch_score(b->R, b->RB, 0, 0, gotoh ? 1 : 0, use_f16 ? 1 : 0, d_res, offs,
                                lens, np, tabs + b->segs[sg].off, use_f16 ? b->nv16 : b->nv,
                                b->S, b->O, b->E, 0, b->pad, b->segs[sg].W, scores, ein, eout,
                                ecols, sg > 0 ? 1 : 0, (int)SWK_PACK_BYTES,
                                perm ? perm + p0 : nullptr, perm_n, (uint32_t)p0, ident, 0, 0, 0,
                                0, 0, (uint32_t)nq, (uint32_t)b->mq_words, sstride, st));
    }
  }
  HIPOK(b, hipEventRecord(b->ev_used, st));
  if (b->timing) {
    HIPOK(b, hipEventRecord(ev.c, st));
    b->events.push_back(ev);
  }
  return SW_OK;
}

extern "C" sw_status sw_score_batch_device(sw_bank* b, const uint8_t* d_res,
                                           const uint64_t* d_offs, const uint32_t* d_lens,
                                           const uint64_t* d_ids, size_t n, uint32_t max_len,
                                           int32_t* d_scores, void* stream) {
  DevGuard dev_guard(b);
  return sw_score_batch_device_range(b, d_res, d_offs, d_lens, d_ids, n, 0, max_len, d_scores,
                                     stream);
}

extern "C" sw_status sw_score_batch_device_range(sw_bank* b, const uint8_t* d_res,
                                                 const uint64_t* d_offs, const uint32_t* d_lens,
                                                 const uint64_t* d_ids, size_t n,
                                                 uint32_t min_len, uint32_t max_len,
                                                 int32_t* d_scores, void* stream) {
  DevGuard dev_guard(b);
  if (!b) return SW_ERR_ARG;
  if (min_len > max_len) return fail(b, SW_ERR_ARG, "min_len %u > max_len %u", min_len, max_len);
  b->best_kind = 0;
  b->best_root = false;
  if (const sw_status fs = take_fault(b, 0); fs != SW_OK) return fs;
  if (n == 0) return SW_OK;
  if (!d_res || !d_offs || !d_lens || !d_scores) return fail(b, SW_ERR_ARG, "null device buffer");
  if (b->is_multi()) {
    if (b->qset.size() > 1 && d_ids) return fail(b, SW_ERR_UNSUPPORTED, "best hit over a query set");
    return multi_device(b, d_res, d_offs, d_lens, d_ids, n, min_len, max_len, d_scores,
                        reinterpret_cast<hipStream_t>(stream), false);
  }
  sw_status st = prepare(b);
  if (st != SW_OK) return st;
  HIPOK(b, hipSetDevice(b->device));
  hipStream_t hs = stream ? reinterpret_cast<hipStream_t>(stream) : b->stream;
  if (b->qset.size() > 1) {
    if (d_ids) return fail(b, SW_ERR_UNSUPPORTED, "best hit over a query set");
    return launch_set(b, d_res, d_offs, d_lens, n, min_len, max_len, d_scores, hs, n);
  }
  if ((st = launch(b, d_res, d_offs, d_lens, n, max_len, d_scores, hs, SWK_PACK_BYTES, nullptr,
                   nullptr, true, true, nullptr, nullptr, 0, 0, min_len)) != SW_OK)
    return st;
  return d_ids ? track_best_device(b, d_scores, d_ids, n, hs) : SW_OK;
}

extern "C" sw_status sw_batch_best(sw_bank* b, uint64_t* best_id, int32_t* best_score,
                                   uint64_t* best_index) {
  DevGuard dev_guard(b);
  if (!b) return SW_ERR_ARG;
  if (b->is_multi() && b->best_root) {
    const sw_status st = sw_batch_best(b->kids[0], best_id, best_score, best_index);
    if (st != SW_OK) return fail(b, st, "device %d: %s", b->kids[0]->device, b->kids[0]->err);
    if (const sw_status fs = take_fault(b, 0); fs != SW_OK) {
      b->kids[0]->best_kind = 0;
      return fs;
    }
    return SW_OK;
  }
  if (b->best_kind == 2) {
    uint64_t h[3];
    HIPOK(b, hipSetDevice(b->device));
    HIPOK(b, hipEventSynchronize(b->best_ev));
    if (const sw_status fs = take_fault(b, 0); fs != SW_OK) {
      b->best_kind = 0;
      return fs;
    }
    HIPOK(b, hipMemcpy(h, b->best_dev.p, sizeof(h), hipMemcpyDeviceToHost));
    b->best_id = h[0];
    b->best_score = (int32_t)(int64_t)h[1];
    b->best_index = h[2];
    b->best_kind = 1;
  }
  if (b->best_kind != 1)
    return fail(b, SW_ERR_STATE, "no best hit recorded (empty batch, or a device call without ids)");
  if (best_id) *best_id = b->best_id;
  if (best_score) *best_score = b->best_score;
  if (best_index) *best_index = b->best_index;
  return SW_OK;
}
```

Baseline: 12700.

## Precompute pair-profile LDS offsets in wave 0 via global code ring

In pair-mode score kernels, wave 0 now loads residue chunks ahead of time, converts them into 16-bit profile address offsets, and writes them into a per-block ring buffer in global memory. The other waves read precomputed offset rows instead of each running load_raw and pair_addr byte extraction in the inner loop. The goal is to remove redundant residue loads and address arithmetic from the critical DP path of every wave. In exchange it adds global-memory ring traffic, a dependency on __syncthreads ordering between the producer wave and its consumers, inline asm, and a new device allocation plumbed through all pair launch sites.

```diff
diff --git a/smith-waterman-fpga-module_amd/csrc/swbank_bank.h b/smith-waterman-fpga-module_amd/csrc/swbank_bank.h
--- a/smith-waterman-fpga-module_amd/csrc/swbank_bank.h
+++ b/smith-waterman-fpga-module_amd/csrc/swbank_bank.h
@@ -53,7 +53,9 @@
                                        const uint32_t* nidx, uint32_t idx_base,
                                        const uint32_t* ident, int pair, uint32_t pS1,
                                        uint32_t pS2, uint32_t ulen, uint32_t ustride, uint32_t nq,
-                                       uint32_t qwords, size_t sstride, hipStream_t st);
+                                       uint32_t qwords, size_t sstride, uint32_t* code_ring,
+                                       size_t ring_words, hipStream_t st);
+extern "C" size_t swk_code_ring_words(int W, uint32_t nq);
 extern "C" unsigned swk_bal_slots(int W, uint32_t PS, int trim);
 extern "C" unsigned swk_wave_half_grid(int gotoh, uint32_t prof_bytes, int W);
 extern "C" hipError_t swk_bal_plan_uniform(void* plan, uint32_t ntiles, uint32_t K, uint32_t G,
@@ -68,7 +70,8 @@
                                           const uint32_t* nidx, const uint32_t* ident,
                                           const void* plan, uint32_t* fault, uint32_t poll_limit,
                                           uint32_t stall, int trim, uint32_t packed,
-                                          const uint32_t* sidx, hipStream_t st);
+                                          const uint32_t* sidx, uint32_t* code_ring,
+                                          size_t ring_words, hipStream_t st);
 extern "C" hipError_t swk_best_hit(const int32_t* scores, const uint64_t* ids, size_t n,
                                    unsigned long long* key, uint64_t* out, uint64_t* out_index,
                                    hipStream_t st);
@@ -447,6 +450,7 @@
   DevBuf<int32_t> grecv;
   PinBuf hrecv;
   DevBuf<uint32_t> bal_state, bal_flag;
+  DevBuf<uint32_t> code_ring[2];
   DevBuf<uint32_t> wbal_state, wbal_flag;
   uint32_t wbal_gen = 0;
   DevBuf<uint32_t> bal_plan;
diff --git a/smith-waterman-fpga-module_amd/csrc/swbank_bank.hip b/smith-waterman-fpga-module_amd/csrc/swbank_bank.hip
--- a/smith-waterman-fpga-module_amd/csrc/swbank_bank.hip
+++ b/smith-waterman-fpga-module_amd/csrc/swbank_bank.hip
@@ -202,6 +202,8 @@
   b->dsort.release();
   b->bal_state.release();
   b->bal_flag.release();
+  b->code_ring[0].release();
+  b->code_ring[1].release();
   b->wbal_state.release();
   b->wbal_flag.release();
   b->bal_plan.release();
diff --git a/smith-waterman-fpga-module_amd/csrc/swbank_kcommon.h b/smith-waterman-fpga-module_amd/csrc/swbank_kcommon.h
--- a/smith-waterman-fpga-module_amd/csrc/swbank_kcommon.h
+++ b/smith-waterman-fpga-module_amd/csrc/swbank_kcommon.h
@@ -27,6 +27,12 @@
 #ifndef SWK_PRIO_END_FRAC
 #define SWK_PRIO_END_FRAC 4
 #endif
+
+#ifndef SWK_CODE_WAVE
+#define SWK_CODE_WAVE 1
+#endif
+#define SWK_CODE_ROW_WORDS 256
+__host__ __device__ inline int swk_code_ring_depth(int W) { return W <= 4 ? 4 : 16; }
 
 #ifndef SWK_STAMPS
 #define SWK_STAMPS 0
@@ -604,8 +610,9 @@
   uint32_t poll_limit, stall;
   uint32_t wbal_blocks, wbal_grid;
   const uint32_t* sidx;
+  uint32_t* code_ring;
 };
-static_assert(sizeof(ScoreArgs) == 376, "ScoreArgs layout (kernel argument block) changed");
+static_assert(sizeof(ScoreArgs) == 384, "ScoreArgs layout (kernel argument block) changed");
 
 __device__ __forceinline__ void report_fault(uint32_t* fault, uint32_t bit) {
   if (fault) __hip_atomic_store(fault + __builtin_ctz(bit), bit, __ATOMIC_RELAXED,
diff --git a/smith-waterman-fpga-module_amd/csrc/swbank_ktile.hip b/smith-waterman-fpga-module_amd/csrc/swbank_ktile.hip
--- a/smith-waterman-fpga-module_amd/csrc/swbank_ktile.hip
+++ b/smith-waterman-fpga-module_amd/csrc/swbank_ktile.hip
@@ -16,6 +16,7 @@
   static_assert(!PAIR || ((R == 32 || (R == 16 && GOTOH)) && F16 && !PROF && !COL0 &&
                           (!GOTOH || !MQ)),
                 "PAIR: f16, merged R = 32 or Gotoh R = 16 / 32 (one query)");
+  constexpr bool CW = PAIR && !STREAM && SWK_CODE_WAVE != 0;
   extern __shared__ __attribute__((aligned(16))) uint32_t smem[];
   const int lane = threadIdx.x & 63;
   const int wave = __builtin_amdgcn_readfirstlane(threadIdx.x >> 6);
@@ -49,7 +50,7 @@
     be = (int)__builtin_amdgcn_readfirstlane(p1.x), bf = (int)__builtin_amdgcn_readfirstlane(p1.y);
     total = (int)__builtin_amdgcn_readfirstlane(p1.z - p0.z);
   }
-  const auto bal_visit = [&](int v, int& t, int& c0, int& c1) {
+  const auto bal_visit_u = [&](int v, int& t, int& c0, int& c1) {
     const int bK = -1;
     const int bfirst = bo ? bs + 1 : bs;
     const int hh = bf > 0 ? 1 : 0;
@@ -62,10 +63,14 @@
     } else {
       t = nunits, c0 = 0, c1 = 1;
     }
+  };
+  const auto bal_visit = [&](int v, int& t, int& c0, int& c1) {
+    bal_visit_u(v, t, c0, c1);
     t = __builtin_amdgcn_readfirstlane(t);
     c0 = __builtin_amdgcn_readfirstlane(c0);
     c1 = __builtin_amdgcn_readfirstlane(c1);
   };
+  (void)bal_visit_u;
   if constexpr (BAL) {
   } else if constexpr (STREAM) {
     total = (int)blockIdx.x < ntiles ? (1 << 30) : 0;
@@ -198,9 +203,76 @@
   u16x2 best = {0, 0};
   u16x2 prevUpH = H0;
   uint2 rlo, rhi;
-  load_raw<C, !MQ>(cur, vc0, vc0 < nfull, a.pad, packed, rlo, rhi);
+  const u16x2 pS12 = {(unsigned short)a.pS1, (unsigned short)a.pS2};
+  const auto pair_addr = [&](uint32_t wl, uint32_t wh, int sh, uint32_t base) {
+    const uint32_t sel = (uint32_t)(sh >> 3) | 0x0C00u | ((uint32_t)(4 + (sh >> 3)) << 16) |
+                         0x0C000000u;
+    const u16x2 ab = __builtin_elementwise_min(as_u16x2(__builtin_amdgcn_perm(wh, wl, sel)),
+                                               (u16x2){4, 4});
+    return __builtin_amdgcn_udot2(ab, pS12, base, false);
+  };
+  typedef unsigned int crow_t __attribute__((ext_vector_type(C / 2)));
+  const int CD = __builtin_amdgcn_readfirstlane(swk_code_ring_depth(W));
+  uint8_t* const cring = reinterpret_cast<uint8_t*>(a.code_ring) +
+                         (size_t)blockIdx.x * CD * (SWK_CODE_ROW_WORDS * 4);
+  const uint32_t cvoff = (uint32_t)lane * (2 * C);
+  const auto row_ptr = [&](int r) {
+    return reinterpret_cast<crow_t*>(cring + (size_t)(uint32_t)((r & (CD - 1)) *
+                                                                (SWK_CODE_ROW_WORDS * 4)) +
+                                     (size_t)cvoff);
+  };
+  const auto store_row = [&](int r, const uint2& lo, const uint2& hi) {
+    crow_t v;
+#pragma unroll
+    for (int j = 0; j < C; j += 2) {
+      const uint32_t o0 = pair_addr(j < 4 ? lo.x : lo.y, j < 4 ? hi.x : hi.y, 8 * (j & 3), 0u);
+      const uint32_t o1 =
+          pair_addr(j + 1 < 4 ? lo.x : lo.y, j + 1 < 4 ? hi.x : hi.y, 8 * ((j + 1) & 3), 0u);
+      v[j >> 1] = o0 | (o1 << 16);
+    }
+    *row_ptr(r) = v;
+    asm volatile("" ::: "memory");
+  };
+  int ru = 0, rc = 0, rend = 0, rnfull = 0, rk = 0;
+  bool rmore = true;
+  const auto reader_step = [&]() {
+    if (rc + 1 < rend) {
+      ++rc;
+    } else if (rmore) {
+      int nu = ru + G, c0 = 0, ve = -1;
+      if constexpr (BAL) bal_visit_u(rk + 1, nu, c0, ve);
+      if (nu < nunits) {
+        ru = nu;
+        ++rk;
+        const int t = MQ ? nu / (int)a.nq : nu;
+        cur = lane_targets<!MQ>(a.res, a.offs, a.lens, n, t, lane, packed, idx, a.ulen,
+                                a.ustride);
+        int n_ch, n_cl;
+        tile_chunks<C>(cur, (size_t)t * SWB_TILE + lane, (size_t)t * SWB_TILE + lane + 64, n, n_ch,
+                       rnfull, n_cl);
+        rend = BAL && ve >= 0 ? ve : n_ch;
+        rc = c0;
+      } else {
+        rmore = false;
+      }
+    }
+    if (rmore) load_raw<C, !MQ>(cur, rc, rc < rnfull, a.pad, packed, rlo, rhi);
+  };
+  (void)store_row; (void)reader_step; (void)row_ptr; (void)cvoff; (void)cring;
+  crow_t nrow = {};
+  if constexpr (CW) {
+    if (wave == 0) {
+      load_raw<C, !MQ>(cur, vc0, vc0 < nfull, a.pad, packed, rlo, rhi);
+      store_row(0, rlo, rhi);
+      ru = unit, rc = vc0, rend = nch, rnfull = nfull;
+      reader_step();
+    }
+  } else {
+    load_raw<C, !MQ>(cur, vc0, vc0 < nfull, a.pad, packed, rlo, rhi);
+  }
   if (STREAM && threadIdx.x == 0) sq[W] = total;
   __syncthreads();
+  if constexpr (CW) nrow = *row_ptr(0);
 
   typedef unsigned int u32x4 __attribute__((ext_vector_type(4)));
   typedef __attribute__((address_space(3))) const u32x4 lds_u4;
@@ -210,18 +282,22 @@
     return __atomic_load_n((lds_u32*)(size_t)addr, __ATOMIC_RELAXED);
   };
   const uint32_t wofs = (uint32_t)wave * R * 4 + (uint32_t)(size_t)(lds_void_ptr)smem;
-  const u16x2 pS12 = {(unsigned short)a.pS1, (unsigned short)a.pS2};
-  const auto pair_addr = [&](uint32_t wl, uint32_t wh, int sh) {
-    const uint32_t sel = (uint32_t)(sh >> 3) | 0x0C00u | ((uint32_t)(4 + (sh >> 3)) << 16) |
-                         0x0C000000u;
-    const u16x2 ab = __builtin_elementwise_min(as_u16x2(__builtin_amdgcn_perm(wh, wl, sel)),
-                                               (u16x2){4, 4});
-    return __builtin_amdgcn_udot2(ab, pS12, wofs, false);
-  };
+  const auto row_addr = [&](const crow_t& v, int j) {
+    uint32_t r;
+    if (j & 1)
+      asm("v_add_u32_sdwa %0, %1, %2 dst_sel:DWORD dst_unused:UNUSED_PAD src0_sel:WORD_1 "
+          "src1_sel:DWORD" : "=v"(r) : "v"(v[j >> 1]), "s"(wofs));
+    else
+      asm("v_add_u32_sdwa %0, %1, %2 dst_sel:DWORD dst_unused:UNUSED_PAD src0_sel:WORD_0 "
+          "src1_sel:DWORD" : "=v"(r) : "v"(v[j >> 1]), "s"(wofs));
+    return r;
+  };
+  (void)row_addr;
   uint32_t acur = 0, pw = 0;
   uint4 pA0 = {0, 0, 0, 0}, pA1 = {0, 0, 0, 0};
   if constexpr (PAIR) {
-    acur = pair_addr(rlo.x, rhi.x, 0);
+    if constexpr (CW) acur = row_addr(nrow, 0);
+    else acur = pair_addr(rlo.x, rhi.x, 0, wofs);
     pA0 = ld4(acur + 16);
     pA1 = ld4(acur + 32);
     pw = ld1(acur + 12);
@@ -312,6 +388,14 @@
     const int g = ph - wave;
     if (g >= 0 && g < total) {
       const uint2 clo = rlo, chi = rhi;
+      const crow_t crow = nrow;
+      (void)crow;
+      if constexpr (CW) {
+        if (wave == 0) {
+          store_row(g + 1, rlo, rhi);
+          reader_step();
+        }
+      }
       const bool last = c + 1 == nch;
       int nunit = (MQ ? unit : tile) + G;
       int nc0 = 0, nvend = 0;
@@ -348,7 +432,16 @@
           }
         }
       }
-      if (!last) {
+      if constexpr (CW) {
+        if (last && nunit < nunits) {
+          const Lane2 t = lane_targets<!MQ>(a.res, a.offs, a.lens, n, ntile, lane, packed, idx,
+                                            a.ulen, a.ustride);
+          tile_chunks<C>(t, (size_t)ntile * SWB_TILE + lane, (size_t)ntile * SWB_TILE + lane + 64,
+                         n, nch_n, nfull_n, ncl_n);
+          if (BAL && nvend >= 0 && nvend < nch_n) ncl_n = C;
+          if (BAL && nvend < 0) nvend = nch_n;
+        }
+      } else if (!last) {
         load_raw<C, !MQ>(cur, c + 1, c + 1 < nfull, a.pad, packed, rlo, rhi);
       } else if (nunit < nunits) {
         if constexpr (STREAM) cur = stream_tile(ntile, packed_n);
@@ -446,6 +539,7 @@
           const uint32_t nwl = jj + 1 < C ? (jj + 1 < 4 ? clo.x : clo.y) : rlo.x;
           const uint32_t nwh = jj + 1 < C ? (jj + 1 < 4 ? chi.x : chi.y) : rhi.x;
           const int nsh = jj + 1 < C ? 8 * ((jj + 1) & 3) : 0;
+          (void)nwl; (void)nwh; (void)nsh;
           uint32_t Da, Db, X, DN, IN;
           const uint32_t noe = as_u32(as_u16x2(NOE2)), ne = as_u32(as_u16x2(NE2)),
                  no = as_u32(as_u16x2(NO2));
@@ -494,10 +588,14 @@
             __builtin_amdgcn_sched_barrier(0);
             SWK_PAIR_BLOCK(1, 16, pA0, pA1)
           }
-          acur = pair_addr(nwl, nwh, nsh);
+          if constexpr (CW) acur = jj + 1 < C ? row_addr(crow, jj + 1) : row_addr(nrow, 0);
+          else acur = pair_addr(nwl, nwh, nsh, wofs);
           pA0 = ld4(acur + 16);
           pA1 = ld4(acur + 32);
           pw = ld1(acur + 12);
+          if constexpr (CW) {
+            if (jj == C - 2) nrow = *row_ptr(g + 1);
+          }
           __builtin_amdgcn_sched_barrier(0);
           SWK_PAIR_BLOCK(2, R - 8, pB0, pB1)
 #undef SWK_PAIR_BLOCK
@@ -536,7 +634,12 @@
       }
       if constexpr (PAIR && TRIM) {
         if (trimmed) {
-          acur = pair_addr(rlo.x, rhi.x, 0);
+          if constexpr (CW) {
+            nrow = *row_ptr(g + 1);
+            acur = row_addr(nrow, 0);
+          } else {
+            acur = pair_addr(rlo.x, rhi.x, 0, wofs);
+          }
           pA0 = ld4(acur + 16);
           pA1 = ld4(acur + 32);
           pw = ld1(acur + 12);
@@ -553,13 +656,20 @@
           bal_store((int)blockIdx.x + 1);
         } else {
         uint32_t* bs = bestsh + (k % W) * SWB_TILE;
-        atomicMax(&bs[lane], (uint32_t)best.x);
-        atomicMax(&bs[lane + 64], (uint32_t)best.y);
+        if constexpr (CW) {
+          uint32_t ol = (uint32_t)lane;
+          asm volatile("" : "+v"(ol));
+          bs += ol;
+        } else {
+          bs += lane;
+        }
+        atomicMax(&bs[0], (uint32_t)best.x);
+        atomicMax(&bs[64], (uint32_t)best.y);
         if (wave == W - 1) {
           const size_t tlo = (size_t)tile * SWB_TILE + lane, thi = tlo + 64;
-          int32_t blo = (int32_t)bs[lane], bhi = (int32_t)bs[lane + 64];
-          bs[lane] = 0;
-          bs[lane + 64] = 0;
+          int32_t blo = (int32_t)bs[0], bhi = (int32_t)bs[64];
+          bs[0] = 0;
+          bs[64] = 0;
           if constexpr (F16) {
             blo = f16_unscore((uint32_t)blo);
             bhi = f16_unscore((uint32_t)bhi);
@@ -665,7 +775,7 @@
 template <int R, int RB, bool COL0, bool PROF, bool GOTOH, bool F16, bool PAIR = false,
           bool MQ = false, bool STREAM = false, int C = 8, bool BAL = false, bool TRIM = false>
 static hipError_t launch_score(const ScoreArgs& a, int W, uint32_t prof_bytes, hipStream_t st,
-                               unsigned bal_grid = 0) {
+                               unsigned bal_grid = 0, size_t ring_words = 0) {
   const size_t ntiles = (a.n + SWB_TILE - 1) / SWB_TILE * (MQ ? a.nq : 1);
   const size_t lds = (size_t)W * SWB_TILE * 4 + tile_ring_entries(W, C, a.edge_in != nullptr) * 8 +
                      (PROF ? prof_bytes : 0) + (PAIR ? a.PS : 0) + (STREAM ? 256 : 0);
@@ -690,6 +800,10 @@
 #endif
   if (MQ && PAIR) grid = std::max(a.nq, grid / a.nq * a.nq);
   if (BAL && (grid == 0 || ntiles < 2 * (size_t)grid)) return hipErrorInvalidConfiguration;
+  if (PAIR && !STREAM && SWK_CODE_WAVE != 0 &&
+      (!a.code_ring || a.PS > 65536u ||
+       (size_t)grid * swk_code_ring_depth(W) * SWK_CODE_ROW_WORDS > ring_words))
+    return hipErrorInvalidValue;
   hipLaunchKernelGGL(fn, dim3(grid), dim3(64 * W), (unsigned)lds, st, a);
   return hipGetLastError();
 }
@@ -727,6 +841,7 @@
                                        const uint32_t* ident, int pair, uint32_t pS1,
                                        uint32_t pS2, uint32_t ulen, uint32_t ustride,
                                        uint32_t nq, uint32_t qwords, size_t sstride,
+                                       uint32_t* code_ring, size_t ring_words,
                                        hipStream_t st) {
   if (n == 0) return hipSuccess;
   swk::ScoreArgs a{res,  offs, lens, n,  qtab, nv, S,
@@ -740,12 +855,15 @@
   a.nq = nq;
   a.qwords = qwords;
   a.sstride = sstride;
+  a.code_ring = code_ring;
   const uint32_t prof_bytes = (pad + 1) * PS;
   if (nq > 1 && pair) {
     if (R == 32 && f16 && !prof && !gotoh && !col0 && (W > 4 || a.edge_in || a.edge_out))
-      return swk::launch_score<32, 4, false, false, false, true, true, true, false, 4>(a, W, 0, st);
+      return swk::launch_score<32, 4, false, false, false, true, true, true, false, 4>(a, W, 0, st, 0,
+                                                                                       ring_words);
     if (R == 32 && f16 && !prof && !gotoh && !col0)
-      return swk::launch_score<32, 4, false, false, false, true, true, true>(a, W, 0, st);
+      return swk::launch_score<32, 4, false, false, false, true, true, true>(a, W, 0, st, 0,
+                                                                             ring_words);
     return hipErrorInvalidValue;
   }
   if (nq > 1) {
@@ -759,15 +877,16 @@
   }
   if (pair) {
     if (R == 32 && f16 && !prof && !gotoh && !col0)
-      return swk::launch_score<32, 4, false, false, false, true, true>(a, W, 0, st);
+      return swk::launch_score<32, 4, false, false, false, true, true>(a, W, 0, st, 0, ring_words);
 #define SWK_GPAIR(RR)                                                                         \
     if (R == RR && f16 && !prof && gotoh && !col0) {                                          \
       const hipError_t e = a.edge_in || a.edge_out                                            \
           ? hipErrorInvalidConfiguration                                                      \
-          : swk::launch_score<RR, 4, false, false, true, true, true>(a, W, 0, st);            \
+          : swk::launch_score<RR, 4, false, false, true, true, true>(a, W, 0, st, 0,          \
+                                                                     ring_words);             \
       if (e != hipErrorInvalidConfiguration) return e;                                        \
-      return swk::launch_score<RR, 4, false, false, true, true, true, false, false, 4>(a, W, 0, \
-                                                                                         st); \
+      return swk::launch_score<RR, 4, false, false, true, true, true, false, false, 4>(       \
+          a, W, 0, st, 0, ring_words);                                                        \
     }
     SWK_GPAIR(32) SWK_GPAIR(16)
 #undef SWK_GPAIR
@@ -802,6 +921,20 @@
   hipLaunchKernelGGL(swk::bal_plan_uniform, dim3(1), dim3(256), 0, st, static_cast<uint4*>(plan),
                      ntiles, K, G);
   return hipGetLastError();
+}
+
+extern "C" size_t swk_code_ring_words(int W, uint32_t nq) {
+#if SWK_CODE_WAVE
+  int dev = 0, cus = 0;
+  if (W < 1 || hipGetDevice(&dev) != hipSuccess ||
+      hipDeviceGetAttribute(&cus, hipDeviceAttributeMultiprocessorCount, dev) != hipSuccess)
+    return 0;
+  const size_t wgs = std::max<size_t>(nq, (size_t)cus * std::max(1, 32 / W));
+  return wgs * swk_code_ring_depth(W) * SWK_CODE_ROW_WORDS;
+#else
+  (void)W; (void)nq;
+  return 0;
+#endif
 }
 
 extern "C" unsigned swk_bal_slots(int W, uint32_t PS, int trim) {
@@ -831,7 +964,8 @@
                                           const uint32_t* nidx, const uint32_t* ident,
                                           const void* plan, uint32_t* fault, uint32_t poll_limit,
                                           uint32_t stall, int trim, uint32_t packed,
-                                          const uint32_t* sidx, hipStream_t st) {
+                                          const uint32_t* sidx, uint32_t* code_ring,
+                                          size_t ring_words, hipStream_t st) {
   if (n == 0) return hipSuccess;
   if (W > 4 || !flag || !state || !plan || !fault || poll_limit == 0 || (idx && !nidx) ||
       (packed != SWK_PACK_BYTES && packed != SWK_PACK_NIBBLE) || (sidx && (!trim || idx)))
@@ -852,11 +986,12 @@
   a.poll_limit = poll_limit;
   a.stall = stall;
   a.sidx = sidx;
+  a.code_ring = code_ring;
   if (trim)
     return swk::launch_score<32, 4, false, false, false, true, true, false, false, 8, true, true>(
-        a, W, 0, st, grid);
+        a, W, 0, st, grid, ring_words);
   return swk::launch_score<32, 4, false, false, false, true, true, false, false, 8, true>(
-      a, W, 0, st, grid);
+      a, W, 0, st, grid, ring_words);
 }
 
 extern "C" hipError_t swk_launch_stream(int R, int gotoh, int f16, int pair, const uint8_t* res,
diff --git a/smith-waterman-fpga-module_amd/csrc/swbank_launch.hip b/smith-waterman-fpga-module_amd/csrc/swbank_launch.hip
--- a/smith-waterman-fpga-module_amd/csrc/swbank_launch.hip
+++ b/smith-waterman-fpga-module_amd/csrc/swbank_launch.hip
@@ -46,6 +46,12 @@
 static uint32_t poll_limit(uint32_t dflt) {
   const int v = env_int("SWBANK_POLL_LIMIT", 0);
   return v > 0 ? (uint32_t)v : dflt;
+}
+
+static hipError_t code_ring_for(sw_bank* b, int W, uint32_t nq, hipStream_t st,
+                                DevBuf<uint32_t>*& ring) {
+  ring = &b->code_ring[st == b->stream2 ? 1 : 0];
+  return ring->reserve(swk_code_ring_words(W, nq));
 }
 
 static int ragged_trim() { return env_int("SWBANK_TRIM", 1) != 0 ? 1 : 0; }
@@ -348,6 +354,8 @@
             dl.nib = gnib ? 1u : 0u;
             HIPOK(b, swk_deal_gather(res, offs, lens, idx, ident, n, &dl, st));
           }
+          DevBuf<uint32_t>* cr = nullptr;
+          HIPOK(b, code_ring_for(b, Wl, 1u, st, cr));
           HIPOK(b, swk_launch_pair_bal(gat ? b->gres.p : res, gat ? b->goffs.p : offs,
                                        gat ? b->glens.p : lens, np, b->qpair.p, b->nv16, b->S, b->O,
                                        b->E, b->pair_bytes, b->pad, Wl,
@@ -360,7 +368,7 @@
                                        rbal && ragged_trim(),
                                        gnib ? (uint32_t)SWK_PACK_NIBBLE
                                             : gat ? (uint32_t)SWK_PACK_BYTES : packed,
-                                       gat ? idx : nullptr, st));
+                                       gat ? idx : nullptr, cr->p, cr->cap, st));
           ++b->ctr.balanced_calls;
           const size_t L = strlen(b->last_kernel);
           snprintf(b->last_kernel + L, sizeof(b->last_kernel) - L, " balanced grid=%u%s", grid,
@@ -374,6 +382,8 @@
         const bool pair = f16 && use_pair;
         int R = b->R, Wl = b->segs[s].W;
         u16_gotoh_rows(b, f16, R, Wl);
+        DevBuf<uint32_t>* cr = &b->code_ring[0];
+        if (pair) HIPOK(b, code_ring_for(b, Wl, 1u, st, cr));
         HIPOK(b, swk_launch_score(R, b->RB, b->col0, b->prof, gotoh ? 1 : 0, f16 ? 1 : 0, res,
                                   offs, lens, np,
                                   pair ? b->qpair.p + s * (b->pair_bytes / 4)
@@ -384,7 +394,7 @@
                                   b->pad, Wl, scores, ein, eout, ecols, s > 0 ? 1 : 0,
                                   (int)packed, idx, nidx, (uint32_t)p0,
                                   pass == 0 ? ident : nullptr, pair ? 1 : 0, b->pS1, b->pS2,
-                                  ulen, ustride, 1u, 0u, 0, st));
+                                  ulen, ustride, 1u, 0u, 0, cr->p, cr->cap, st));
       }
     }
   }
@@ -514,13 +524,15 @@
       if (mpair) {
         const int rows = std::min(prow, (int)b->query.size() - (int)sg * prow);
         const int Wp = std::max(1, (rows + 31) / 32);
+        DevBuf<uint32_t>* cr = nullptr;
+        HIPOK(b, code_ring_for(b, Wp, (uint32_t)nq, st, cr));
         HIPOK(b, swk_launch_score(32, 4, 0, 0, 0, 1, d_res, offs, lens, np,
                                   b->mqpair.p + sg * nq * b->mq_pair_words, b->nv16, b->S, b->O,
                                   b->E, (uint32_t)b->mq_pair_words * 4, b->pad, Wp, scores, ein,
                                   eout, ecols, sg > 0 ? 1 : 0, (int)SWK_PACK_BYTES,
                                   perm ? perm + p0 : nullptr, perm_n, (uint32_t)p0, ident, 1,
                                   b->mq_pS1, b->mq_pS2, 0, 0, (uint32_t)nq,
-                                  (uint32_t)b->mq_pair_words, sstride, st));
+                                  (uint32_t)b->mq_pair_words, sstride, cr->p, cr->cap, st));
         continue;
       }
       HIPOK(b, swk_launch_score(b->R, b->RB, 0, 0, gotoh ? 1 : 0, use_f16 ? 1 : 0, d_res, offs,
@@ -528,7 +540,7 @@
                                 b->S, b->O, b->E, 0, b->pad, b->segs[sg].W, scores, ein, eout,
                                 ecols, sg > 0 ? 1 : 0, (int)SWK_PACK_BYTES,
                                 perm ? perm + p0 : nullptr, perm_n, (uint32_t)p0, ident, 0, 0, 0,
-                                0, 0, (uint32_t)nq, (uint32_t)b->mq_words, sstride, st));
+                                0, 0, (uint32_t)nq, (uint32_t)b->mq_words, sstride, nullptr, 0, st));
     }
   }
   HIPOK(b, hipEventRecord(b->ev_used, st));
```

Result: no change. 12800, median of 6 (+0.8%).
